# urw7rs/diffusion-models-made-easy

Measured on AMD Instinct MI355X. Metric: denoising steps/sec + training images/sec, DDPM UNet CIFAR10 32×32 @1/2/4/8 GPU, higher is better.
Workload: dtype bf16; 1 GPU; DDPM T=1000 sampling, CIFAR10 32x32, default UNet (32,416,643 params, random init), batch 128 per GPU, t.shape=(1,); global_batch=128, parallelism=dp1 (independent chains per GPU, no data-path collective)

## Files before the change

### diffusion-models-made-easy_amd/_lib.py

```python

from __future__ import annotations

import ctypes as C
import os
import subprocess
import threading

_HERE = os.path.dirname(os.path.abspath(__file__))
LIB_PATH = os.environ.get("DMME_LIB_PATH") or os.path.join(_HERE, "libdmme_hip.so")
CSRC = os.path.join(_HERE, "csrc")

F16R32 = 4
F32, BF16, BF16X3, F16 = 0, 1, 2, 3
CHAIN_DDPM, CHAIN_DDIM, CHAIN_IDDPM, CHAIN_DDPM_GUIDED, CHAIN_DDIM_GUIDED, CHAIN_GDDIM = 0, 1, 2, 3, 4, 5
CHAIN_DDPM_CFG, CHAIN_GDDIM_CFG = 6, 7
CHAIN_DPMPP, CHAIN_DPMPP_CFG = 8, 9
CHAIN_REPAINT = 10
CHAIN_ILVR = 11
CHAIN_DDNM = 12
PRED_EPS, PRED_X0, PRED_V = 0, 1, 2
PREDICTIONS = {"eps": PRED_EPS, "x0": PRED_X0, "v": PRED_V}
CM_METRICS = {"pseudo-huber": 0, "l2": 1}
THRESHOLD_NONE, THRESHOLD_STATIC, THRESHOLD_DYNAMIC = 0, 1, 2
THRESHOLDS = {"none": THRESHOLD_NONE, "static": THRESHOLD_STATIC, "dynamic": THRESHOLD_DYNAMIC}
# ... 14 lines not shown
        ("dropout", C.c_float),
        ("num_depths", C.c_int),
        ("channels_per_depth", C.c_int * 8),
        ("num_blocks", C.c_int),
        ("num_attention_depths", C.c_int),
        ("attention_depths", C.c_int * 8),
        ("arch", C.c_int),
        ("num_heads", C.c_int),
        ("num_classes", C.c_int),
    ]


class ConvDesc(C.Structure):
    _fields_ = [(n, C.c_int) for n in (
        "dtype", "N", "Hin", "Win", "C1", "C2", "upsample", "stride", "taps", "Cout", "pro_silu", "out_silu",
        "nt", "tproj_ld", "in_nchw", "out_nchw", "force_generic")]


BUCKET_FN = C.CFUNCTYPE(None, C.c_void_p, C.c_int, C.c_int64, C.c_int64)


class DmmeError(RuntimeError):
    pass


def build(verbose: bool = False) -> str:
    cmd = ["make", "-C", CSRC, "-j", str(min(8, os.cpu_count() or 1))]
    res = subprocess.run(cmd, stdout=subprocess.PIPE, stderr=subprocess.STDOUT, text=True)
    if verbose or res.returncode != 0:
        print(res.stdout)
    if res.returncode != 0:
        raise DmmeError("building libdmme_hip.so failed")
    return LIB_PATH


_vp, _i, _i64, _f, _u64 = C.c_void_p, C.c_int, C.c_int64, C.c_float, C.c_uint64

PROTOTYPES = {
    "dmme_last_error": (C.c_char_p, []),
    "dmme_version": (_i, []),
    "dmme_device_count": (_i, []),
    "dmme_unet_plan_create": (_i, [C.POINTER(UNetCfg), _i, _i, _i, _i, _i, C.POINTER(_vp)]),
    "dmme_unet_plan_destroy": (None, [_vp]),
    "dmme_unet_plan_num_params": (_i, [_vp]),
    "dmme_unet_plan_param_info": (_i, [_vp, _i, C.c_char_p, _i, C.POINTER(_i), C.POINTER(_i64), C.POINTER(_i64), C.POINTER(_i)]),
    "dmme_unet_plan_ref_numel": (_i64, [_vp]),
    "dmme_unet_plan_packed_bytes": (_i64, [_vp]),
    "dmme_unet_plan_workspace_bytes": (_i64, [_vp]),
    "dmme_unet_plan_dropmask_numel": (_i64, [_vp]),
    "dmme_unet_plan_out_channels": (_i, [_vp]),
    "dmme_unet_plan_num_launches": (_i, [_vp]),
    "dmme_unet_plan_num_launches_nograd": (_i, [_vp]),
    "dmme_unet_plan_num_folded": (_i, [_vp]),
    "dmme_unet_pack_params": (_i, [_vp, _vp, _vp, _vp]),
    "dmme_unet_pack_folded": (_i, [_vp, _vp, _vp]),
    "dmme_unet_forward": (_i, [_vp, _vp, _vp, _vp, _i, _vp, _vp, _vp, _vp]),
    "dmme_unet_forward_nograd": (_i, [_vp, _vp, _vp, _vp, _i, _vp, _vp, _vp, _vp]),
    "dmme_unet_forward_cond": (_i, [_vp, _vp, _vp, _vp, _i, _vp, _vp, _vp, _vp, _i, _vp, _vp]),
    "dmme_unet_backward_cond": (_i, [_vp, _vp, _vp, _vp, _vp, _i, _vp, _vp, _vp, _vp, _vp, _vp, _vp, _vp, _vp, _vp]),
    "dmme_unet_backward_input_cond": (_i, [_vp, _vp, _vp, _vp, _vp, _i, _vp, _vp, _vp, _vp, _vp, _vp, _vp]),
    "dmme_label_dropout": (_i, [_vp, _i, _i, _f, _u64, _u64, _vp, _vp, _vp]),
    "dmme_cfg_step": (_i, [_i, _vp, _vp, _vp, _f, _f, _f, _f, _i, _i, _i64, _vp]),
    "dmme_chain_update_cfg": (_i, [_i, _vp, _vp, _vp, _vp, _vp, _vp, _i, _i64, _vp]),
    "dmme_cfg_chain_step": (_i, [_vp, _vp, _vp, _vp, _vp, _vp, _vp, _i, _vp, _vp, _vp, _vp]),
    "dmme_dpmpp_step": (_i, [_vp, _vp, _vp, C.POINTER(_f), _i, _i, _i64, _i, _vp]),
    "dmme_chain_update_dpmpp": (_i, [_vp, _vp, _vp, _vp, _vp, _vp, _i, _i64, _i, _vp]),
    "dmme_dpmpp_chain_step": (_i, [_vp, _vp, _vp, _vp, _vp, _vp, _vp, _vp, _vp, _vp]),
    "dmme_cfg_dpmpp_step": (_i, [_vp, _vp, _vp, C.POINTER(_f), _i, _i, _i64, _vp]),
    "dmme_chain_update_cfg_dpmpp": (_i, [_vp, _vp, _vp, _vp, _vp, _vp, _i, _i64, _vp]),
    "dmme_cfg_dpmpp_chain_step": (_i, [_vp, _vp, _vp, _vp, _vp, _vp, _vp, _vp, _vp, _vp, _vp, _vp]),
    "dmme_repaint_step": (_i, [_vp, _vp, _vp, _vp, _vp, C.POINTER(_f), _i, _i64, _i, _vp]),
    "dmme_chain_update_repaint": (_i, [_vp, _vp, _vp, _vp, _vp, _vp, _vp, _vp, _i, _i64, _i, _vp]),
    "dmme_repaint_chain_step": (_i, [_vp, _vp, _vp, _vp, _vp, _vp, _vp, _vp, _vp, _vp, _vp]),
    "dmme_lowpass": (_i, [_vp, _vp, _i, _i, _i, _vp, _vp, _vp, _i, _vp]),
    "dmme_lowpass_lds_capacity": (_i, []),
    "dmme_lowpass_scratch_bytes": (_i64, [_i, _i, _i]),
    "dmme_ilvr_step": (_i, [_vp, _vp, _vp, _vp, C.POINTER(_f), _vp, _vp, _vp, _i, _i, _i, _i, _i, _i, _vp]),
    "dmme_chain_update_ilvr": (_i, [_vp, _vp, _vp, _vp, _vp, _vp, _vp, _vp, _vp, _vp, _i, _i, _i, _i, _i, _i, _vp]),
    "dmme_ilvr_chain_step": (_i, [_vp, _vp, _vp, _vp, _vp, _vp, _vp, _vp, _vp, _vp, _vp, _vp, _vp]),
    "dmme_ddnm_band_capacity": (_i, []),
    "dmme_ddnm_measure": (_i, [_vp, _vp, _vp, _i, _i, _i, _i, _i, _i, _vp]),
    "dmme_ddnm_step": (_i, [_vp, _vp, _vp, _vp, _vp, C.POINTER(_f), _i, _i, _i, _i, _i, _i, _i, _vp]),
    "dmme_chain_update_ddnm": (_i, [_vp, _vp, _vp, _vp, _vp, _vp, _vp, _vp, _i, _i, _i, _i, _i, _i, _i, _vp]),
    "dmme_ddnm_chain_step": (_i, [_vp, _vp, _vp, _vp, _vp, _vp, _vp, _i, _i, _vp, _vp, _vp, _vp]),
    "dmme_distill_noise": (_i, [_vp, _vp, _vp, _vp, _vp, _vp, _i, _i, _i64, _vp, _vp, _vp, _vp, _vp]),
    "dmme_distill_mid": (_i, [_i, _i, _vp, _vp, _vp, _vp, _i, _i, _i64, _vp, _vp]),
    "dmme_distill_target": (_i, [_i, _i, _vp, _vp, _vp, _vp, _vp, _vp, _i, _i, _i64, _vp, _vp]),
    "dmme_cm_target": (_i, [_i, _vp, _vp, _vp, _vp, _i, _i, _i64, _vp, _vp]),
    "dmme_cm_loss": (_i, [_i, _vp, _vp, _vp, _vp, _vp, _i, _i, _i64, _f, _vp, _vp, _vp, _f, _vp, _vp]),
    "dmme_ema_lerp": (_i, [_vp, _vp, _i64, _f, _vp]),
    "dmme_unet_plan_num_ops": (_i, [_vp]),
    "dmme_unet_plan_level_info": (_i, [_vp, C.c_char_p, _i]),
    "dmme_unet_plan_check": (_i, [_vp]),
    "dmme_debug_level_stamps": (_i, [_vp, _i, _i]),
    "dmme_unet_plan_op_info": (_i, [_vp, _i, C.c_char_p, _i, C.POINTER(C.c_double), C.POINTER(C.c_double)]),
    "dmme_unet_forward_profiled": (_i, [_vp, _vp, _vp, _vp, _i, _vp, _vp, _vp, _vp, _vp]),
    "dmme_unet_plan_packed_bwd_bytes": (_i64, [_vp]),
    "dmme_unet_plan_bwd_workspace_bytes": (_i64, [_vp]),
    "dmme_unet_pack_params_bwd": (_i, [_vp, _vp, _vp, _vp]),
    "dmme_unet_backward": (_i, [_vp, _vp, _vp, _vp, _vp, _i, _vp, _vp, _vp, _vp, _vp, _vp, _vp]),
    "dmme_unet_backward_buckets": (_i, [_vp, _vp, _vp, _vp, _vp, _i, _vp, _vp, _vp, _vp, _vp, _vp, _vp, BUCKET_FN, _vp]),
    "dmme_unet_backward_input": (_i, [_vp, _vp, _vp, _vp, _vp, _i, _vp, _vp, _vp, _vp, _vp, _vp]),
    "dmme_unet_plan_grad_buckets": (_i, [_vp, C.POINTER(_i64), C.POINTER(_i64), C.POINTER(_i), _i]),
    "dmme_unet_plan_bwd_summary": (_i, [_vp, C.c_char_p, _i]),
    "dmme_grad_norm": (_i, [_vp, _i64, _vp, _vp, _vp]),
    "dmme_adam_step": (_i, [_vp, _vp, _vp, _vp, _vp, _i64, _f, _f, _f, _f, _i, _vp, _f, _f, _f, _vp]),
    "dmme_amp_init": (_i, [_vp, _f, _vp]),
    "dmme_amp_scale": (_i, [_vp, _i64, _vp, _vp]),
    "dmme_adam_step_amp": (_i, [_vp, _vp, _vp, _vp, _vp, _i64, _f, _f, _f, _f, _vp, _f, _f, _f, _vp, _f, _f, _i, _vp]),
    "dmme_grad_pack_bf16": (_i, [_vp, _i64, _vp, _i64, _vp]),
    "dmme_shard_reduce_bf16": (_i, [_vp, _i, _i64, _f, _vp, _vp]),
    "dmme_grad_unpack_bf16": (_i, [_vp, _i64, _vp, _vp]),
    "dmme_unet_debug_read": (_i, [_vp, _vp, C.c_char_p, _vp, _i64, C.POINTER(_i64), _vp]),
    "dmme_unet_debug_read_grad": (_i, [_vp, _vp, C.c_char_p, _vp, _i64, C.POINTER(_i64), _vp]),
    "dmme_unet_debug_read_norm_stats": (_i, [_vp, _vp, C.c_char_p, _vp, _i64, C.POINTER(_i64), _vp]),
    "dmme_dropout_masks": (_i, [_vp, _u64, _u64, _vp, _vp]),
    "dmme_randn": (_i, [_vp, _i64, _u64, _u64, _vp]),
    "dmme_q_sample": (_i, [_vp, _vp, _vp, _vp, _vp, _i, _i64, _vp, _vp, _vp]),
    "dmme_ddpm_step": (_i, [_vp, _vp, _vp, _f, _f, _f, _i, _i64, _vp]),
    "dmme_ddim_step": (_i, [_vp, _vp, _f, _f, _i64, _vp]),
    "dmme_gddim_step": (_i, [_vp, _vp, _vp, _f, _f, _f, _i64, _vp]),
    "dmme_slerp": (_i, [_vp, _vp, _vp, _i, _i, _i64, _vp, _vp]),
    "dmme_chain_set": (_i, [_vp, _i64, _vp, _u64, _u64, _vp]),
    "dmme_chain_update": (_i, [_i, _vp, _vp, _vp, _vp, _vp, _i, _i64, _vp]),
    "dmme_chain_step": (_i, [_vp, _vp, _vp, _vp, _vp, _i, _vp, _vp, _vp, _vp]),
    "dmme_chain_update_gddim": (_i, [_vp, _vp, _vp, _vp, _vp, _vp, _i, _i64, _vp]),
    "dmme_log_softmax_grad": (_i, [_vp, _vp, _i, _i, _i, _f, _vp, _vp, _vp, _vp]),
    "dmme_chain_update_guided": (_i, [_i, _vp, _vp, _vp, _vp, _vp, _vp, _vp, _i, _i64, _vp]),
    "dmme_guided_chain_step": (_i, [_vp, _vp, _vp, _vp, _vp, _vp, _vp, _vp, _vp, _vp, _vp, _vp, _vp, _vp, _vp, _i, _vp, _vp, _vp, _vp]),
    "dmme_mse_loss": (_i, [_vp, _vp, _i64, _vp, _vp, _f, _vp, _vp]),
    "dmme_pred_to_eps": (_i, [_i, _vp, _vp, _vp, _i, _vp, _i, _i, _i64, _vp]),
    "dmme_unet_plan_set_prediction": (_i, [_vp, _i, _vp, _i]),
    "dmme_x0_threshold": (_i, [_i, _vp, _vp, _vp, _i, _vp, _i, _i, _i64, _i, _i, _f, _i, _f, _vp, _vp]),
    "dmme_x0_threshold_scratch_bytes": (_i64, [_i, _i64]),
    "dmme_x0_threshold_lds_capacity": (_i, []),
    "dmme_unet_plan_set_threshold": (_i, [_vp, _i, _vp, _i, _i, _f, _vp]),
    "dmme_q_sample_pred": (_i, [_i, _vp, _vp, _vp, _vp, _vp, _i, _i64, _vp, _vp, _vp]),
    "dmme_mse_loss_rows": (_i, [_vp, _vp, _vp, _vp, _i, _i64, _vp, _vp, _f, _vp, _vp]),
    "dmme_image_batch": (_i, [_vp, _i64, _vp, _vp, _i, _i, _i, _i, _vp, _vp]),
    "dmme_grid_tile": (_i, [_vp, _i, _i, _i, _i, _i, _i, _i, _i, _i, _i, _i, _vp, _vp]),
    "dmme_iddpm_step": (_i, [_vp, _vp, _vp, _f, _f, _f, _f, _i, _i, _i64, _vp]),
    "dmme_iddpm_loss": (_i, [_vp, _vp, _vp, _vp, _vp, _vp, _i, _i64, _f, _f, _vp, _vp, _f, _vp, _vp]),
    "dmme_iddpm_loss_rows": (_i, [_vp, _vp, _vp, _vp, _vp, _vp, _i, _vp, _i, _i64, _f, _f, _vp, _vp, _vp, _f, _vp, _vp, _vp]),
    "dmme_iddpm_prior_rows": (_i, [_vp, _i, _i64, _f, _vp, _vp]),
    "dmme_tsampler_draw": (_i, [_vp, _vp, _i, _i, _f, _u64, _u64, _i, _vp, _vp, _vp, _vp]),
    "dmme_tsampler_update": (_i, [_vp, _vp, _i, _i, _vp, _vp, _i, _vp, _vp]),
    "dmme_conv2d": (_i, [C.POINTER(ConvDesc), _vp, _vp, _vp, _vp, _vp, _vp, _vp, _vp, _vp, _vp, _i, _vp, _vp]),
    "dmme_conv2d_res": (_i, [C.POINTER(ConvDesc), _vp, _vp, _vp, _vp, _vp, _vp, _vp, _vp, _vp, _i, _i, _vp, _vp, _vp, _vp]),
    "dmme_groupnorm_scale_shift": (_i, [_i, _vp, _vp, _i, _i, _i, _i, _i, _vp, _vp, _f, _vp, _vp, _vp, _i, _vp]),
    "dmme_attention": (_i, [_i, _vp, _i, _i, _i, _vp, _i, _vp]),
    "dmme_attention_proj": (_i, [_i, _vp, _i, _i, _i, _vp, _vp, _vp, _vp, _vp, _vp, _i, _vp]),
    "dmme_attention_fold": (_i, [_i, _i, _vp, _vp, _vp, _vp, _vp, _vp, _vp, _vp, _vp]),
    "dmme_attention_block": (_i, [_i, _vp, _i, _i, _i, _vp, _i, _i, _i, _vp, _vp, _f, _vp, _vp, _vp, _vp, _vp, _vp, _vp, _vp, _vp, _i, _vp]),
    "dmme_attention_heads": (_i, [_i, _vp, _i, _i, _i, _i, _vp, _i, _vp]),
    "dmme_nchw_to_nhwc": (_i, [_i, _vp, _i, _i, _i, _vp, _vp]),
    "dmme_nhwc_to_nchw": (_i, [_i, _vp, _i, _i, _i, _vp, _vp]),
    "dmme_pack_weight": (_i, [_i, _vp, _i, _i, _i, _vp, _vp]),
    "dmme_event_create": (_i, [C.POINTER(_vp)]),
    "dmme_event_record": (_i, [_vp, _vp]),
    "dmme_event_elapsed_ms": (_i, [_vp, _vp, C.POINTER(_f)]),
    "dmme_event_destroy": (_i, [_vp]),
    "dmme_debug_set_stamps": (_i, [_vp]),
    "dmme_debug_mfma_valu": (_i, [_i, _i, _i, _vp, _vp]),
    "dmme_debug_issue_probe": (_i, [_i, _i, _i, _i, _i, _vp, _vp, _vp]),
    "dmme_debug_l2_stream": (_i, [_vp, _i64, _i, _i, _i, _i, _vp, _vp]),
}


def lib():
    global _lib
    if _lib is not None:
        return _lib
    with _lock:
        if _lib is not None:
            return _lib
        if not os.path.exists(LIB_PATH):
            raise DmmeError(
                f"{LIB_PATH} is missing: the HIP extension is not built. Run `python -c 'import __graft_entry__ as g; g.build()'` "
                "(or `make -C diffusion-models-made-easy_amd/csrc`). There is no CPU fallback for the product path."
            )
        h = C.CDLL(LIB_PATH)
        for name, (res, args) in PROTOTYPES.items():
            fn = getattr(h, name)
            fn.restype = res
            fn.argtypes = args
        _lib = h
    return _lib


def check(rc: int, what: str = ""):
    if rc != 0:
        msg = lib().dmme_last_error().decode("utf-8", "replace")
        if rc == -2:
            raise NotImplementedError(f"{what}: {msg}")
        if rc == -1:
            raise ValueError(f"{what}: {msg}")
        raise DmmeError(f"{what} failed (status {rc}): {msg}")


def require_gpu():
    if lib().dmme_device_count() <= 0:
        raise DmmeError("libdmme_hip.so loaded but no HIP device is visible; the denoiser path only runs on an MI355X")


def dtype_code(precision) -> int:
# ... 29 lines not shown
```

### diffusion-models-made-easy_amd/csrc/common.h

```cpp
#pragma once

#include <hip/hip_runtime.h>
#include <stdint.h>

#include "dmme_hip.h"

namespace dmme {

void set_error(const char* fmt, ...) __attribute__((format(printf, 1, 2)));

int debug_route(const char* key, int dflt = 0);

#define DMME_CHECK_HIP(expr)                                                                          \
    do {                                                                                              \
        hipError_t e_ = (expr);                                                                       \
        if (e_ != hipSuccess) {                                                                       \
            ::dmme::set_error("%s failed: %s (%s:%d)", #expr, hipGetErrorString(e_), __FILE__, __LINE__); \
            return DMME_ERR_HIP;                                                                      \
        }                                                                                             \
    } while (0)

#define DMME_REQUIRE(cond, code, ...)        \
    do {                                     \
        if (!(cond)) {                       \
// ... 128 lines not shown
    const float* p2;
    int t1, cnt1, C1, t2, cnt2, C2, groups;
    const float* gamma;
    const float* beta;
    float eps;
    float* mean_rstd;
    const float* t_shift;
    const float* t_scale;
    int t_ld, nt;
};

struct ConvArgs {
    const void* src1;
    const void* src2;
    const void* w;
    const float* bias;
    const float* scale;
    const float* shift;
    const float* dmask;
    const float* tproj;
    const void* res1;
    const void* res2;
    void* dst;
    int N, Hin, Win, C1, C2;
    int up, stride, taps;
    int Hout, Wout, Cout;
    int pro_silu, out_silu;
    int nt, tproj_ld, R1;
    int in_nchw, out_nchw;
    float* gn_part;
    int gn_cg, gn_tiles;
    int gn_raw_moments;
    long long* stamps;
    float* splitk;
    int64_t splitk_cap;
    int x3;
    int mix;
    int mix2;
    int f16;
    int dma_b;
    GnOut gno[2];
    int n_gno;
    float gn_eps;
    void* act;
    int act_k, act_silu;
    const float* act_dmask;
    GnIn gni;
    int has_gni;
    const void* r_src1;
    const void* r_src2;
    const void* r_w;
    const float* r_bias;
    int r_C1, r_C2;
};

int launch_mfma_valu(int mode, int iters, int blocks, float* sink, hipStream_t s);
int launch_issue_probe(int kind, int n_inner, int iters, int flags, int blocks, long long* sink, const void* src, hipStream_t s);
int launch_l2_stream(const void* buf, int64_t bytes, int iters, int mode, int depth, int blocks, unsigned* sink, hipStream_t s);

struct ConvTile {
    int TW, TH, TN;
    int HH, HWd;
    int tiles_x, tiles_y;
    int tiles_m, tiles_n;
    int a_rows;
    unsigned magic_px, magic_w;
};
enum ConvFamily {
    CONV_GENERIC = 0,
    CONV_MFMA,
    CONV_THIN,
    CONV1X1_SPLIT,
    CONV1X1_AS,
    CONV1X1_TILED,
    CONV3X3_SPLIT,
    CONV3X3_WS,
    CONV3X3_KW,
    CONV3X3_PIPE,
};
struct ConvRoute {
    int family;
    ConvTile tile;
    int BM, BN;
    int cand;
    int GT, UA;
    int NI, ring;
    int ksplit;
    int rseg;
    int vec;
    int stat_bn;
    int stat_px;
    int stat_tiles;
};
inline ConvRoute make_route(int family, int BM = 0, int BN = 0, int vec = 0) {
    ConvRoute r{};
    r.family = family;
    r.BM = r.stat_px = BM;
    r.BN = r.stat_bn = BN;
    r.vec = vec;
    return r;
}
ConvRoute conv_route(int dtype, const ConvArgs& a);
bool conv_thin_route(int dtype, const ConvArgs& a, ConvRoute& r);
bool conv1x1_split_route(int dtype, const ConvArgs& a, ConvRoute& r);
bool conv1x1_domain(int dtype, const ConvArgs& a);
bool conv1x1_as_route(int dtype, const ConvArgs& a, ConvRoute& r);
bool conv1x1_tiled_route(int dtype, const ConvArgs& a, ConvRoute& r);
bool conv3x3_split_route(int dtype, const ConvArgs& a, ConvRoute& r);
bool conv3x3_pipe_route(int dtype, const ConvArgs& a, ConvRoute& r);
bool conv3x3_ws_route(int dtype, const ConvArgs& a, ConvRoute& r);
bool conv3x3_kw_route(int dtype, const ConvArgs& a, ConvRoute& r);
bool conv_mfma_route(int dtype, const ConvArgs& a, ConvRoute& r);
void conv_generic_route(const ConvArgs& a, ConvRoute& r);
bool conv_mfma_supported(int dtype, const ConvArgs& a);
int launch_conv_generic(int dtype, const ConvArgs& a, hipStream_t s);
const char* conv_generic_kernel_name(const ConvArgs& a);
int launch_conv_mfma(const ConvRoute& r, int dtype, const ConvArgs& a, hipStream_t s);
int launch_conv_out_thin(const ConvArgs& a, hipStream_t s);
int launch_conv1x1(const ConvRoute& r, int dtype, const ConvArgs& a, hipStream_t s);
int launch_conv1x1_as(const ConvArgs& a, hipStream_t s);
int launch_conv3x3(const ConvRoute& r, int dtype, const ConvArgs& a, hipStream_t s);
int launch_conv_kw(int dtype, const ConvArgs& a, const ConvTile& g, int NI, int ring, int BM, int ksplit, hipStream_t s);
int launch_conv(int dtype, const ConvArgs& a, hipStream_t s, int force = 0);
int launch_conv(const ConvRoute& r, int dtype, const ConvArgs& a, hipStream_t s);
void conv_label(const ConvRoute& r, int dtype, const ConvArgs& a, char* buf, int cap);
bool conv_stats_query(int dtype, const ConvArgs& a, int cg, int* tiles, int* px);
bool conv_gn_in_query(int dtype, const ConvArgs& a);
bool conv1x1_tiled_gn_in_ok(const ConvArgs& a, const ConvRoute& r);
bool conv3x3_pipe_gn_in_ok(int dtype, const ConvArgs& a, const ConvRoute& r);
int conv_gn_direct_query(int dtype, const ConvArgs& a, const int* cg, int n);
int launch_gn_finalize_parts(const float* part1, int tiles1, int cnt1, int C1, const float* part2, int tiles2, int cnt2, int C2, int N, int groups,
                             const float* gamma, const float* beta, float eps, float* scale, float* shift, float* mean_rstd, const float* t_shift,
                             const float* t_scale, int t_ld, int nt, hipStream_t s);

int launch_gn_generic(int dtype, const void* src1, const void* src2, int N, int HW, int C1, int C2, int groups,
                      const float* gamma, const float* beta, float eps, float* scale, float* shift, float* mean_rstd,
                      hipStream_t s);
bool gn_fast_supported(int dtype, int N, int HW, int C1, int C2, int groups);
size_t gn_fast_scratch_floats(int N, int HW, int C, int groups);
int launch_gn_fast(int dtype, const void* src1, const void* src2, int N, int HW, int C1, int C2, int groups,
                   const float* gamma, const float* beta, float eps, float* scale, float* shift, float* mean_rstd,
                   float* partial, hipStream_t s, void* act = nullptr, int act_silu = 0, const float* dmask = nullptr);
bool gn_small_act_supported(int dtype, int HW, int C1, int C2, int groups);

int launch_attn_generic(int dtype, const void* qkv, int N, int S, int C, void* out, hipStream_t s);
int launch_attn_heads(int dtype, const void* qkv, int N, int S, int C, int heads, void* out, hipStream_t s);
int launch_attn_heads_bwd(int dtype, const void* qkv, const void* dO, int N, int S, int C, int heads, float* P, float* dS, void* dqkv, hipStream_t s);
int launch_gn_modulate(float* scale, float* shift, const float* t_shift, const float* t_scale, int ld, int nt, int N, int C, hipStream_t s);
bool attn_x3_supported(int N, int S, int C, int heads);
int launch_attn_x3(const void* qkv, int N, int S, int C, int heads, void* out, hipStream_t s);
bool attn_mfma_supported(int dtype, int N, int S, int C);
bool attn_full_takes(int S, int D);
int launch_attn_mfma(int dtype, const void* qkv, int N, int S, int C, void* out, float* lse, hipStream_t s);
bool attn_proj_fusable(int dtype, int N, int S, int C, int gn_cg, int gn_tiles);
int launch_attn_proj(int dtype, const void* qkv, int N, int S, int C, void* ctx, float* lse, const void* w, const float* bias, const void* res, void* dst,
                     float* gn_part, int gn_tiles, int gn_cg, hipStream_t s, long long* stamps = nullptr);
struct AttnFoldJob {
    int64_t wq, bq, wp, bp;
    int64_t M, c, wpv, bias2;
    int32_t C, pad;
};
bool attn_fold_shape_ok(int dtype, int N, int S, int C, int gn_cg, int gn_tiles);
int launch_attn_fold(int dtype, const void* x, int N, int S, int C, const GnIn* gni, const float* scale, const float* shift, const void* M, const float* c,
                     const void* wpv, const float* bias2, const void* res, void* dst, float* gn_part, int gn_tiles, int gn_cg, hipStream_t s,
                     long long* stamps = nullptr);
int launch_attn_fold_weights(int dtype, const AttnFoldJob* jobs_dev, int n_jobs, int maxC, void* packed, hipStream_t s, const AttnFoldJob* one = nullptr);
bool attn_heads_mfma_supported(int dtype, int N, int S, int C, int heads);
int launch_attn_heads_mfma(int dtype, const void* qkv, int N, int S, int C, int heads, void* out, float* lse, hipStream_t s);
int launch_attn_heads_bwd_mfma(int dtype, const void* qkv, const void* O, const void* dO, const float* lse, int N, int S, int C, int heads, void* P,
                               void* dS, void* dqkv, hipStream_t s);
bool attn_bwd_mfma_supported(int dtype, int N, int S, int C);
int launch_attn_bwd_mfma(int dtype, const void* qkv, const void* O, const void* dO, const float* lse, int N, int S, int C, void* P, void* dS,
                         void* dqkv, hipStream_t s);

constexpr unsigned kFwdMarkKeep = 0x4B454550u, kFwdMarkNograd = 0x4E4F4752u;
constexpr unsigned kErrNogradBackward = 0x80000000u;
int launch_time_sinusoid(const int64_t* t, int nt, const float* freqs, int half, float* out, hipStream_t s, unsigned* mark = nullptr,
                         unsigned mark_val = 0);
int launch_linear_wave(int dtype, const float* in, int nt, int K, const void* W, const float* bias, int Nout,
                       int out_silu, float* out, hipStream_t s);
int launch_label_cond(const float* z2, int nt, const float* E, const int64_t* labels, int B, int K, int emb, float* temb, float* zsave, int* status,
                      hipStream_t s);
int launch_label_grad(const float* dz2, const int64_t* labels, int B, int K, int emb, float* dE, hipStream_t s);

int launch_nchw_to_nhwc(int dtype, const float* src, int N, int C, int HW, void* dst, hipStream_t s, const unsigned* mark = nullptr,
                        unsigned* err = nullptr);
int launch_nhwc_to_nchw(int dtype, const void* src, int N, int C, int HW, float* dst, hipStream_t s);
int launch_pack_weight(int dtype, const float* src, int Cout, int Cin, int taps, void* dst, hipStream_t s);
int launch_cast_f32_to_16(int dtype, const float* src, int64_t numel, void* dst, hipStream_t s);

struct PackItem {
    int64_t src_off;
    int64_t dst_off;
    int32_t cout, cin, taps;
    int32_t row0, rows;
    int32_t ci0, nci;
    int32_t as_f32;
};
int launch_pack_table(int dtype, const PackItem* items_dev, int n_items, const float* ref_flat, void* packed,
                      hipStream_t s);

int launch_randn(float* out, int64_t numel, uint64_t seed, uint64_t offset, hipStream_t s);
int launch_dropmask(float* out, int64_t numel, float p, uint64_t seed, uint64_t offset, hipStream_t s);
int launch_q_sample(const float* x0, const float* z, const float* sqrt_abar, const float* sqrt_1m_abar,
                    const int64_t* t, int B, int64_t chw, float* x_t, float* target, hipStream_t s);
int launch_pred_to_eps(int pred, float* model_out, const float* x, const float* ab, int T, const int64_t* t, int t_len, int B, int64_t chw,
                       hipStream_t s);
int launch_x0_threshold(int mode, float* out, const float* x, const float* table, int T, const int64_t* t, int t_len, int B, int64_t chw, int planes,
                        int halves, float sg, const float* sg_coef, int sg_row, int sg_col, const int64_t* sg_state, int k, float frac, void* scratch,
                        hipStream_t s);
int slerp_parts(int64_t chw);
int launch_slerp(const float* xa, const float* xb, const float* w, int n, int B, int64_t chw, float* out, float* scratch, hipStream_t s);
int launch_chain_set(void* state, int64_t i, const int64_t* t_table, uint64_t seed, uint64_t offset, hipStream_t s);

// ... 183 lines not shown
```

### diffusion-models-made-easy_amd/csrc/conv_pipe.hip

```cpp
#include <stdio.h>

#include "conv_common.h"

namespace dmme {



template <typename T, int BM, int BN, int GT, int PIPE_UA, bool ACC3 = false>
__global__ void __launch_bounds__(256, GT == 9 ? 1 : 2) conv3x3_pipe_kernel(ConvArgs a, ConvTile g, int shTW, int shTH, int ksplit) {
    constexpr int KC = Frag<T>::KC, EPV = Frag<T>::EPV;
    constexpr int MI = BM / 64, NI = BN / 64;
    constexpr int UB = BN / 32;
    extern __shared__ __attribute__((aligned(16))) char lds[];
#define PIPE_STAMP(K) do { if (a.stamps && blockIdx.x < 2 && blockIdx.y == 0 && threadIdx.x == 0) a.stamps[blockIdx.x * 8 + (K)] = (long long)wall_clock64(); } while (0)
    PIPE_STAMP(0);
    char* ldsA = lds;
    char* ldsB = lds + (size_t)g.a_rows * ROW_DATA;
    constexpr bool DMAB_OK = sizeof(T) == 2 && GT == 3 && BN == 64;
    constexpr int B_BYTES = GT * BN * ROW_DATA;
    const bool dmab = DMAB_OK && a.dma_b;
    int cur = 0;
    float* gni_par = reinterpret_cast<float*>(ldsB + (size_t)B_BYTES * (dmab ? 2 : 1));

    const int tid = threadIdx.x, lane = tid & 63, wave = tid >> 6;
// ... 269 lines not shown
        }
        float f[4] = {v.x, v.y, v.z, v.w};
        const int n = (int)(p / hw);
#pragma unroll
        for (int j = 0; j < 4; ++j) {
            float fold = a.bias ? a.bias[c + j] : 0.f;
            if (a.tproj) fold += a.tproj[(int64_t)(a.nt == 1 ? 0 : n) * a.tproj_ld + c + j];
            f[j] += fold;
            if (a.res1) f[j] += to_f(((const T*)a.res1)[p * a.Cout + c + j]);
            ((T*)a.dst)[p * a.Cout + c + j] = from_f<T>(f[j]);
        }
    }
}
static int pipe_ksplit(const ConvArgs& a, const ConvTile& g, int pick, int KC) {
    if (a.has_gni) return 1;
    const bool off = (debug_route("no_splitk") != 0);
    if (off || !a.splitk || pick != 3 || a.stride != 1 || a.gn_part || a.n_gno || a.out_silu || a.out_nchw || a.res2 || a.Cout % 4) return 1;
    const int64_t wgs = (int64_t)g.tiles_m * g.tiles_n;
    if (wgs > 128) return 1;
    int ks = (a.C1 + a.C2) / KC;
    const int room = (int)(256 / wgs);
    if (ks > room) ks = room;
    if (ks > 4) ks = 4;
    const int64_t out = (int64_t)a.N * a.Hout * a.Wout * a.Cout;
    while (ks > 1 && ks * out > a.splitk_cap) --ks;
    return ks < 1 ? 1 : ks;
}

#ifndef WS_CDMA
#define WS_CDMA 1
#endif
#ifndef WS_HYB
#define WS_HYB 0
#endif
#ifndef WS_SCHED2
#define WS_SCHED2 1
#endif
#ifndef WS_TP_UNROLL
#define WS_TP_UNROLL 9
#endif
template <typename T, int BN, int MI, int NI>
__device__ __forceinline__ void ws_stage16(const f32x16 (&acc)[MI][NI], T* row) {
    typedef T tx2 __attribute__((ext_vector_type(2)));
#pragma unroll
    for (int mi = 0; mi < MI; ++mi)
#pragma unroll
        for (int ni = 0; ni < NI; ++ni)
#pragma unroll
            for (int q = 0; q < 4; ++q) {
                const tx2 lo = {(T)acc[mi][ni][4 * q], (T)acc[mi][ni][4 * q + 1]}, hi = {(T)acc[mi][ni][4 * q + 2], (T)acc[mi][ni][4 * q + 3]};
                *reinterpret_cast<uint2*>(row + mi * 64 * (BN + kStage16Pad) + 32 * ni + 8 * q) = make_uint2(__builtin_bit_cast(unsigned, lo), __builtin_bit_cast(unsigned, hi));
            }
}
struct WsTile { int n0, oy0, ox0, co0, ts; };
__device__ __forceinline__ WsTile ws_tile_of(const ConvTile& g, int shTW, int shTH, int kt, int bn) {
    const int t = (int)blockIdx.x + kt * (int)gridDim.x;
    const int tile_n = t % g.tiles_n, tile_m = t / g.tiles_n;
    const int tiles_img = g.tiles_x * g.tiles_y;
    WsTile r;
    const int sp = tile_m % tiles_img;
    r.n0 = tile_m / tiles_img;
    r.oy0 = (sp / g.tiles_x) << shTH;
    r.ox0 = (sp % g.tiles_x) << shTW;
    r.co0 = tile_n * bn;
    r.ts = sp;
    return r;
}

__host__ __device__ inline int ws2_stage_pad(int a_bytes) { return a_bytes + 2 * 128 * ROW_DATA >= 64 * 1024 ? 0 : 64 * 1024 - 2 * 128 * ROW_DATA - a_bytes; }

__device__ __forceinline__ void ws_fill_par_gni(const ConvArgs& a, int n, bool writer, float* par, int Cin, int tid, int nthr) {
    for (int c = tid; c < Cin; c += nthr) {
        float sc, sh;
        const float dmk = a.dmask ? a.dmask[n * Cin + c] : 1.f;
        gn_in_scale_shift(a, n, c, Cin, writer, sc, sh);
        par[c] = sc * dmk;
        par[Cin + c] = sh * dmk;
        par[2 * Cin + c] = a.pro_silu ? -1.4426950408889634f * sc : 0.f;
        par[3 * Cin + c] = a.pro_silu ? -1.4426950408889634f * sh : -126.f;
    }
}

template <typename T, int SPLIT>
struct WsSplit {
    typedef T ts;
};
template <typename T>
struct WsSplit<T, 1> {
    typedef float ts;
};
template <typename T>
struct WsSplit<T, 2> {
    typedef float ts;
};
template <int PIPE_UA, typename T = bf16, int BM = 256, int SPLIT = 0, bool RSEG = false, bool E16 = false>
__global__ void __launch_bounds__(512, 1) conv3x3_ws2_kernel(ConvArgs a, ConvTile g, int shTW, int shTH, int ntiles) {
    constexpr int KC = 64, EPV = 8, BN = 128, MI = BM / 64, NI = 2, UB = BN / 32;
    constexpr bool CDMA = WS_CDMA != 0;
    constexpr bool SCHED2 = WS_SCHED2 != 0 && CDMA && SPLIT == 0;
    static_assert(!(SCHED2 && WS_HYB != 0), "the hybrid tap ownership counts the halo loads of the two-unit schedule");
    static_assert(!E16 || (SPLIT == 0 && BM == 256 && sizeof(T) == 2), "16-bit staging: 16-bit tensors, 256-pixel tiles");
    static_assert(!RSEG || (SPLIT == 0 && sizeof(T) == 2), "residual segment: 16-bit tensors");
    constexpr int KCR = SPLIT ? 32 : KC;
    constexpr int EPR = SPLIT ? 4 : EPV;
    typedef typename WsSplit<T, SPLIT>::ts TS;
    static_assert(SPLIT == 0 || (BM == 256 && dtype_of<T>::value == DMME_F16), "split passes: fp16 hi / lo on the 256-pixel tile");
    constexpr int R_BYTES = BN * ROW_DATA;
    constexpr int A_PITCH = ROW_DATA + 16;
    static_assert((BM == 256 && PIPE_UA == 11) || (BM == 128 && PIPE_UA == 7), "unit schedules below: 11 units over 9 stages, or 7 units over the first 7");
    typedef unsigned u32x4 __attribute__((ext_vector_type(4)));
    extern __shared__ __attribute__((aligned(16))) char lds[];
    const int a_bytes = g.a_rows * A_PITCH;
    const int Cin = a.C1 + a.C2;
    const int offA1 = a_bytes + 3 * R_BYTES, offR = a_bytes;
    float* par_base = reinterpret_cast<float*>(lds + 2 * a_bytes + 3 * R_BYTES + ws2_stage_pad(a_bytes));
    float* fold_base = par_base + 2 * 4 * Cin;
#define WS_FILL_FOLD(KT)                                                                              \
    if constexpr (E16) {                                                                              \
        if (tid < BN) {                                                                               \
            const TileXY ff_ = WS_TILE(KT);                                                           \
            const int co_ = ff_.co0 + tid;                                                            \
            float f_ = 0.f;                                                                           \
            if (co_ < a.Cout) {                                                                       \
                f_ = a.bias ? a.bias[co_] : 0.f;                                                      \
                if (a.r_bias) f_ += a.r_bias[co_];                                                    \
                if (a.tproj) f_ += a.tproj[(a.nt == 1 ? 0 : ff_.n0) * a.tproj_ld + co_];              \
            }                                                                                         \
            fold_base[((KT) & 1) * BN + tid] = f_;                                                    \
        }                                                                                             \
    }
#define WS_BUFA(p) (lds + (((p) & 1) ? offA1 : 0))
#define WS_RING(slot) (lds + offR + (slot) * R_BYTES)
#define WS_PAR(kt) (par_base + ((kt) & 1) * 4 * Cin)
#define WS_TILE(kt) ws_tile_of(g, shTW, shTH, (kt), BN)
    typedef WsTile TileXY;
    const int tid = threadIdx.x, lane = tid & 63, wave = tid >> 6;
    const bool producer = wave >= 4;
    const int nchunks = Cin / KCR;
    const int CinW = SPLIT ? 2 * Cin : Cin;
    const int Cres = RSEG ? a.r_C1 + a.r_C2 : 0;
    const int HS = Cres / 32;
    constexpr int RSL = 5;
    const int RT = HS + ((RSEG && (HS - 1) % RSL < 2) ? 1 : 0);
#define WS_RSA(k) ((k) < 2 ? lds + (k) * (BM * 64) : (k) == 2 ? lds + offR + 2 * R_BYTES : lds + offA1 + ((k) - 3) * (BM * 64))
#define WS_RSW(k) ((k) < 4 ? lds + offR + (k) * 8192 : lds + offA1 + 2 * (BM * 64))
    const int K = (ntiles - (int)blockIdx.x + (int)gridDim.x - 1) / (int)gridDim.x;
    const bool has_pro = a.scale || a.pro_silu || a.dmask;
#define WS_FILL_PAR_N(KT, NTHR)                                           \
    {                                                                     \
        float* par = WS_PAR(KT);                                          \
        const TileXY ft_ = WS_TILE(KT);                                   \
        if (a.has_gni) {                                                  \
            ws_fill_par_gni(a, ft_.n0, ft_.ts == 0 && ft_.co0 == 0, par, Cin, tid, NTHR); \
        } else {                                                          \
            const int pn0 = ft_.n0;                                       \
            for (int c = tid; c < Cin; c += (NTHR)) {                     \
                const int so = pn0 * Cin + c;                             \
                const float sc_ = a.scale ? a.scale[so] : 1.f, sh_ = a.scale ? a.shift[so] : 0.f, dm_ = a.dmask ? a.dmask[so] : 1.f; \
                par[c] = sc_ * dm_;                                       \
                par[Cin + c] = sh_ * dm_;                                 \
                par[2 * Cin + c] = a.pro_silu ? -1.4426950408889634f * sc_ : 0.f;    \
                par[3 * Cin + c] = a.pro_silu ? -1.4426950408889634f * sh_ : -126.f; \
            }                                                             \
        }                                                                 \
    }
#define WS_FILL_PAR(KT) WS_FILL_PAR_N(KT, 512)
    const int mTW = (1 << shTW) - 1, mTH = (1 << shTH) - 1;
    float gn_carry[2] = {0.f, 0.f};
    const bool estamp = tid == 0 && blockIdx.x == 0;
    int e_i = 0;
#define WS_ESTAMP() { if (estamp && a.stamps && e_i < 24) a.stamps[64 + e_i++] = (long long)clock64(); }
#define WS2_PASS(TT, P, STAGE_STMT)                                                                                                \
    {                                                                                                                              \
        constexpr int p = (P);                                                                                                     \
        auto pix_of = [&](int m) -> int {                                                                                          \
            const int mm = m + 128 * p;                                                                                            \
            const int tx = mm & mTW, ty = (mm >> shTW) & mTH;                                                                      \
            return ((TT).n0 * a.Hout + (TT).oy0 + ty) * a.Wout + (TT).ox0 + tx;                                                    \
        };                                                                                                                         \
        uint4 rpre[128 * (BN / (16 / (int)sizeof(TS))) / 512];                                                                     \
        if constexpr (!E16) conv_epilogue_res_prefetch<TS, 128, BN, 512>(a, (TT).co0, pix_of, rpre);  \
        WS_ESTAMP()                                                                                                                \
        STAGE_STMT                                                                                                                 \
        WS_ESTAMP()                                                                                                                \
        lds_barrier();                                                                                                             \
        WS_ESTAMP()                                                                                                                \
        conv_epilogue_store<TS, 128, BN, 512, E16>(a, (TT).co0, (TT).n0, pix_of, stage, (BM / 128) * (TT).ts + p, E16 ? nullptr : rpre, a.n_gno ? p : -1, gn_carry); \
        WS_ESTAMP()                                                                                                                \
        lds_barrier();                 \
    }
#define WS2_EPILOGUE(TT, KT, STAGE0, STAGE1)                                                                                       \
    {                                                                                                                              \
        float* stage = reinterpret_cast<float*>(WS_RING(1));                                                                       \
        WS2_PASS(TT, 0, STAGE0)                                                                                                    \
        if constexpr (BM == 256) { WS2_PASS(TT, 1, STAGE1) }                                                                       \
        if ((KT) + 2 < K) WS_FILL_PAR((KT) + 2)                                                                                    \
    }
#define WS2_EPILOGUE16(TT, KT, STAGE_ALL)                                                                                          \
    {                                                                                                                              \
        T* st16 = reinterpret_cast<T*>(WS_RING(1));                                                                                \
        if ((KT) + 1 < K) WS_FILL_FOLD((KT) + 1)                                                                                   \
        WS_ESTAMP()                                                                                                                \
        STAGE_ALL                                                                                                                  \
        WS_ESTAMP()                                                                                                                \
        lds_barrier();                                                                                                             \
        WS_ESTAMP()                                                                                                                \
        _Pragma("unroll") for (int p = 0; p < 2; ++p) {                                                                            \
            auto pix_of = [&](int m) -> int {                                                                                      \
                const int mm = m + 128 * p;                                                                                        \
                const int tx = mm & mTW, ty = (mm >> shTW) & mTH;                                                                  \
                return ((TT).n0 * a.Hout + (TT).oy0 + ty) * a.Wout + (TT).ox0 + tx;                                                \
            };                                                                                                                     \
            conv_epilogue_store<TS, 128, BN, 512, true>(a, (TT).co0, (TT).n0, pix_of, reinterpret_cast<float*>(st16 + p * 128 * (BN + kStage16Pad)), \
                                                        2 * (TT).ts + p, nullptr, a.n_gno ? p : -1, gn_carry);                     \
            WS_ESTAMP()                                                                                                            \
        }                                                                                                                          \
        lds_barrier();                                                                 \
        if ((KT) + 2 < K) WS_FILL_PAR((KT) + 2)                                                                                    \
    }
    if (producer) {
        const int ptid = tid & 255, cu = ptid & 7, urow = ptid >> 3, pw = ptid >> 6;
        const int Hv = a.up ? 2 * a.Hin : a.Hin, Wv = a.up ? 2 * a.Win : a.Win;
        int a_pix[PIPE_UA], a_sw[PIPE_UA];
        unsigned b_vo[UB];
#pragma unroll
        for (int i = 0; i < PIPE_UA; ++i) a_sw[i] = (urow + 32 * i) * A_PITCH + cu * (SPLIT ? 8 : 16);
#pragma unroll
        for (int k4 = 0; k4 < UB; ++k4) b_vo[k4] = (unsigned)(((urow + 32 * k4) * 9 * CinW + (cu ^ ((urow >> 1) & 7)) * EPV) * 2);
        auto pix_unit = [&](int i, const TileXY& t) __attribute__((always_inline)) -> int {
            const int row = urow + 32 * i;
            const int hy = (int)__umulhi((unsigned)row, g.magic_w), hx = row - hy * g.HWd;
            const int iy = t.oy0 - 1 + hy, ix = t.ox0 - 1 + hx;
            const bool in = iy >= 0 && iy < Hv && ix >= 0 && ix < Wv && !(a.up == 2 && ((iy | ix) & 1));
            const int sy = a.up ? (iy >> 1) : iy, sx = a.up ? (ix >> 1) : ix;
#ifdef WS_SAME_IMAGE
            return row >= g.a_rows ? -2 : in ? ((t.n0 & 7) * a.Hin + sy) * a.Win + sx : -1;
#else
            return row >= g.a_rows ? -2 : in ? (t.n0 * a.Hin + sy) * a.Win + sx : -1;
#endif
        };
        auto set_pix = [&](int i, const TileXY& t) __attribute__((always_inline)) { a_pix[i] = pix_unit(i, t); };
        const char* wbase = (const char*)a.w;
        u32x4 areg[PIPE_UA];
        f32x2 pS[4], pH[4], pS2[4], pH2[4];
        auto load_par = [&](const float* par, int c0) __attribute__((always_inline)) {
            const float* p = par + c0 + cu * EPR;
#pragma unroll
            for (int d = 0; d < EPR / 2; ++d) {
                pS[d] = *reinterpret_cast<const f32x2*>(p + 2 * d);
                pH[d] = *reinterpret_cast<const f32x2*>(p + Cin + 2 * d);
                pS2[d] = *reinterpret_cast<const f32x2*>(p + 2 * Cin + 2 * d);
                pH2[d] = *reinterpret_cast<const f32x2*>(p + 3 * Cin + 2 * d);
            }
        };
        auto load_A = [&](int i, int ch) __attribute__((always_inline)) {
            constexpr int SB = SPLIT == 1 ? 4 : 2;
            const int c0 = ch * KCR;
            const bool second = c0 >= a.C1;
            const char* sbase = (const char*)(second ? a.src2 : a.src1) + (size_t)((second ? c0 - a.C1 : c0) * SB);
            const int Cs = second ? a.C2 : a.C1;
            const int px = a_pix[i] < 0 ? 0 : a_pix[i];
            const char* gp = sbase + (size_t)((unsigned)(px * Cs + cu * EPR) * (unsigned)SB);
            if constexpr (SPLIT == 2) {
                const uint2 v2 = *reinterpret_cast<const uint2*>(gp);
                areg[i] = u32x4{v2.x, v2.y, 0u, 0u};
            } else {
                areg[i] = *reinterpret_cast<const u32x4*>(gp);
            }
        };
        auto store_A = [&](int i, char* dstA, int mode = 0) __attribute__((always_inline)) {
            const int pix = a_pix[i], sw = a_sw[i];
            u32x4 val = areg[i];
            if constexpr (SPLIT != 0) {
                f32x2 y[2];
                if constexpr (SPLIT == 1) {
                    y[0] = f32x2{__uint_as_float(val[0]), __uint_as_float(val[1])};
                    y[1] = f32x2{__uint_as_float(val[2]), __uint_as_float(val[3])};
                } else {
                    typedef T tx4 __attribute__((ext_vector_type(4)));
                    const tx4 x = __builtin_bit_cast(tx4, make_uint2(val[0], val[1]));
                    y[0] = f32x2{(float)x[0], (float)x[1]};
// ... 12 lines not shown
#pragma unroll
                for (int d = 0; d < 2; ++d)
#pragma unroll
                    for (int k = 0; k < 2; ++k) {
                        const f16 hv = (f16)y[d][k];
                        hi[2 * d + k] = hv;
                        lo[2 * d + k] = (f16)sub_plain(y[d][k], (float)hv);
                    }
                uint2 hw = __builtin_bit_cast(uint2, hi), lw = __builtin_bit_cast(uint2, lo);
                if (pix < 0) hw = lw = make_uint2(0u, 0u);
                if (pix != -2) {
                    *reinterpret_cast<uint2*>(dstA + sw) = hw;
                    *reinterpret_cast<uint2*>(dstA + sw + 64) = lw;
                }
                return;
            }
            if (has_pro && mode != 2) {
                typedef typename Vec8<T>::type tx8;
                const tx8 x = __builtin_bit_cast(tx8, val);
                tx8 o;
#pragma unroll
                for (int d = 0; d < 4; ++d) {
                    float xv[2], yv[2];
                    if constexpr (sizeof(T) == 2 && dtype_of<T>::value == DMME_BF16) {
                        xv[0] = __uint_as_float(val[d] << 16);
                        xv[1] = __uint_as_float(val[d] & 0xffff0000u);
                    } else {
                        xv[0] = (float)x[2 * d];
                        xv[1] = (float)x[2 * d + 1];
                    }
                    pro_pair_plain(xv[0], xv[1], pS[d], pH[d], pS2[d], pH2[d], yv[0], yv[1]);
                    o[2 * d] = (T)yv[0];
                    o[2 * d + 1] = (T)yv[1];
                }
                val = __builtin_bit_cast(u32x4, o);
            }
            if (mode == 1) {
                areg[i] = val;
                return;
            }
            const u32x4 zero = {0u, 0u, 0u, 0u};
            if (pix < 0) val = zero;
            if (pix != -2) *reinterpret_cast<u32x4*>(dstA + sw) = val;
        };
        auto dma_tap = [&](char* dstR, int co0, int c, int t) __attribute__((always_inline)) {
#if defined(WS_X_NO_DMA)
            {
                const char* ub1 = wbase + ((size_t)co0 * 9 * CinW + (size_t)t * CinW + (size_t)c * KC) * 2;
                _Pragma("unroll") for (int k4 = 0; k4 < UB; ++k4) glds16_hidden(ub1 + (lane & 7) * 16, (unsigned)__builtin_amdgcn_readfirstlane((int)((unsigned)(size_t)(lds_c*)dstR + (unsigned)(pw * 8 * ROW_DATA) + (unsigned)(32 * k4 * ROW_DATA))));
                return;
            }
#endif
            const unsigned lbase = (unsigned)(size_t)(lds_c*)dstR + (unsigned)(pw * 8 * ROW_DATA);
            const char* ub = wbase + ((size_t)co0 * 9 * CinW + (size_t)t * CinW + (size_t)c * KC) * 2;
#pragma unroll
            for (int k4 = 0; k4 < UB; ++k4) {
                const unsigned l = (unsigned)__builtin_amdgcn_readfirstlane((int)(lbase + (unsigned)(32 * k4 * ROW_DATA)));
                glds16_hidden(ub + b_vo[k4], l);
            }
        };
        constexpr int RA = BM / 64, RD = RA + 2;
        auto dma_rseg_A = [&](int k, const TileXY& t, int j) __attribute__((always_inline)) {
            int ln = lane;
            asm volatile("" : "+v"(ln));
            const int c0 = j * 32;
            const bool second = c0 >= a.r_C1;
            const int Cs = second ? a.r_C2 : a.r_C1;
            const int tile_pix0 = (t.n0 * a.Hin + t.oy0) * a.Win + t.ox0;
            const char* sb = (const char*)(second ? a.r_src2 : a.r_src1) + ((size_t)tile_pix0 * Cs + (second ? c0 - a.r_C1 : c0)) * 2;
            const unsigned la = (unsigned)(size_t)(lds_c*)WS_RSA(k) + (unsigned)(pw * (BM / 4) * 64);
            const int piece = ((ln & 3) ^ ((ln >> 4) & 3)) * 16;
#pragma unroll
            for (int q = 0; q < RA; ++q) {
                const int m = (BM / 4) * pw + 16 * q + (ln >> 2);
                const int rel = (m >> shTW) * a.Win + (m & mTW);
                const unsigned l = (unsigned)__builtin_amdgcn_readfirstlane((int)(la + (unsigned)(q * 1024)));
                glds16_hidden_s(sb, (unsigned)(rel * Cs * 2 + piece), l);
            }
        };
        auto dma_rseg_W = [&](int k, const TileXY& t, int j) __attribute__((always_inline)) {
            int ln = lane;
            asm volatile("" : "+v"(ln));
            const char* wb = (const char*)a.r_w + ((size_t)t.co0 * Cres + j * 32) * 2;
            const unsigned lw = (unsigned)(size_t)(lds_c*)WS_RSW(k) + (unsigned)(pw * 2048);
            const int piece = ((ln & 3) ^ ((ln >> 4) & 3)) * 16;
#pragma unroll
            for (int q = 0; q < 2; ++q) {
                const unsigned l = (unsigned)__builtin_amdgcn_readfirstlane((int)(lw + (unsigned)(q * 1024)));
                glds16_hidden_s(wb, (unsigned)((32 * pw + 16 * q + (ln >> 2)) * Cres * 2 + piece), l);
            }
        };
        TileXY tcur = WS_TILE(0), tnext = WS_TILE(K > 1 ? 1 : 0);
        {
#pragma unroll
            for (int i = 0; i < PIPE_UA; ++i) {
                set_pix(i, tcur);
                load_A(i, 0);
            }
            dma_tap(WS_RING(0), tcur.co0, 0, 0);
            dma_tap(WS_RING(1), tcur.co0, 0, 1);
            WS_FILL_PAR(0)
            __syncthreads();
            load_par(WS_PAR(0), 0);
#pragma unroll
            for (int i = 0; i < PIPE_UA; ++i) store_A(i, WS_BUFA(0));
#pragma unroll
            for (int i = 0; i < PIPE_UA; ++i) load_A(i, 1);
            wait_vm_keep<PIPE_UA>();
        }
        __syncthreads();
        int kt = 0, cc = 0, cg = 0;
        int p_i = 0;
        (void)p_i;
#define WS_A_UNIT(i)                                                        \
    {                                                                       \
        if (RSEG && last_c) {  \
            if (do_store) store_A((i), dstA, 1);                            \
        } else {                                                            \
            if (do_store) store_A((i), dstA);                               \
            WS_PSTT(1)                                                      \
            if (new_tile) set_pix((i), tnn);                                \
            WS_PSTT(2)                                                      \
            load_A((i), lc);                                                \
            WS_PSTT(3)                                                      \
        }                                                                   \
    }
#define WS_A_MATH(i) { if (do_store) store_A((i), dstA, 1); }
#define WS_A_WRITE(i)                                                        \
    {                                                                       \
        if (RSEG && last_c) {  } \
        else {                                                              \
            if (do_store) store_A((i), dstA, 2);                            \
            WS_PSTT(1)                                                      \
            if (new_tile) set_pix((i), tnn);                                \
            load_A((i), lc);                                                \
        }                                                                   \
    }
#define WS_A_ARRIVED(i) { asm volatile("" : "+v"(areg[i][0]), "+v"(areg[i][1]), "+v"(areg[i][2]), "+v"(areg[i][3])); }
#ifdef WS_PSTAMPS
        long long* pst_lds = reinterpret_cast<long long*>(reinterpret_cast<char*>(par_base) + 2 * 4 * Cin * 4 + 1024);
#define WS_PSTT(TAG) { if (a.stamps && ptid == 0 && blockIdx.x == 0 && p_i < 500) pst_lds[p_i++] = (long long)clock64() | ((long long)(TAG) << 56); }
#else
#define WS_PSTT(TAG)
#endif
#define WS_PST() WS_PSTT(0)
#define WS_L(TP) (PIPE_UA == 11 ? (((TP) == 0 || (TP) == 8) ? 2 : 1) : ((TP) < 7 ? 1 : 0))
#define WS_RD(TP) ((TP) <= 4 ? UB : (TP) <= 6 ? UB + RA : 0)
#define WS_RX(TP) (((TP) == 5 || (TP) == 6) ? RA : 0)
#define WS_PSTAGE(TP)                                                                                                   \
    {                                                                                                                   \
        WS_PST()                                                                                                        \
        const bool last_c = cc + 1 == nchunks;                                                                          \
        const bool have_n = !(last_c && kt + 1 == K);                                                                   \
// ... 77 lines not shown
            else wait_lgkm_all();                                                                                       \
        }                                                                                                               \
        else if (RSEG && last_c) {                                                                                      \
             \
            if ((TP) == 0) wait_vm_keep<WS_L(8) + UB>();                                                                \
            else if ((TP) <= 6) wait_vm_keep<WS_RX(((TP) + 8) % 9) + WS_RD(TP)>();                                      \
            else if ((TP) == 7) wait_vm_keep<WS_RX(6) + 4>();   \
            else wait_vm_keep<2>();                                                                                     \
        }                                                                                                               \
        else if (sent_next) wait_vm_keep<UB + WS_L(TP)>();                                                              \
        else if (sent) wait_vm_keep<WS_L(((TP) + 8) % 9) + UB + WS_L(TP)>();                                            \
        else wait_vm_keep<WS_L(((TP) + 8) % 9) + WS_L(TP)>();                                                           \
        WS_PST()                                                                                                        \
        __builtin_amdgcn_s_barrier();                                                                                   \
        if ((TP) == 8) {                                                                                                \
            ++cg;                                                                                                       \
            if (++cc == nchunks) {         \
                if constexpr (RSEG) {                                                                                   \
                     \
                    int sl = 2;                                                                                         \
                    for (int j = 0; j < RT; ++j) {                                                                      \
                        const bool fin = j + 1 == RT && kt + 1 < K;                                                     \
                        for (int h_ = (j == 0 ? 2 : j + 4); h_ <= j + 4 && h_ < HS; ++h_) {                             \
                            dma_rseg_A(sl, tcur, h_);                                                                   \
                            dma_rseg_W(sl, tcur, h_);                                                                   \
                            sl = sl == RSL - 1 ? 0 : sl + 1;                                                            \
                        }                                                                                               \
                        if (fin) {  \
                            _Pragma("unroll") for (int i = 0; i < PIPE_UA; ++i) store_A(i, WS_BUFA(cg), 2);             \
                            dma_tap(WS_RING(0), tnext.co0, 0, 0);                                                       \
                            _Pragma("unroll") for (int i = 0; i < PIPE_UA; ++i) load_A(i, 1);                           \
                        }                                                                                               \
                        __builtin_amdgcn_sched_barrier(0);                                                              \
                        const int hmax = j + 4 < HS - 1 ? j + 4 : HS - 1;     \
                        const int ahead = hmax - (j + 1);                    \
                        if (fin) wait_vm_keep<UB + PIPE_UA>();                                                          \
                        else if (ahead >= 3) wait_vm_keep<3 * RD>();                                                    \
                        else if (ahead == 2) wait_vm_keep<2 * RD>();                                                    \
                        else if (ahead == 1) wait_vm_keep<RD>();                                                        \
                        else wait_vm_keep<0>();                                                                         \
                        __builtin_amdgcn_s_barrier();                                                                   \
                    }                                                                                                   \
                }                                                                                                       \
                if constexpr (E16) { WS2_EPILOGUE16(tcur, kt, ;) } else { WS2_EPILOGUE(tcur, kt, ;, ;) }                         \
                                       \
                        \
                cc = 0;                                                                                                 \
                ++kt;                                                                                                   \
                tcur = tnext;                                                                                           \
                tnext = WS_TILE(kt + 1 < K ? kt + 1 : kt);                                                              \
            }                                                                                                           \
        }                                                                                                               \
    }
        const int GCH = K * nchunks;
        for (int ch = 0; ch < GCH; ++ch) {
            WS_PSTAGE(0) WS_PSTAGE(1) WS_PSTAGE(2) WS_PSTAGE(3) WS_PSTAGE(4) WS_PSTAGE(5) WS_PSTAGE(6) WS_PSTAGE(7) WS_PSTAGE(8)
        }
#ifdef WS_PSTAMPS
        if (a.stamps && ptid == 0 && blockIdx.x == 0)
            for (int i = 0; i < p_i; ++i) a.stamps[128 + i] = pst_lds[i];
#endif
#undef WS_PSTAGE
#undef WS_RD
#undef WS_RX
#undef WS_L
#undef WS_PST
#undef WS_PSTT
#undef WS_A_UNIT
#undef WS_A_MATH
#undef WS_A_WRITE
#undef WS_A_ARRIVED
        return;
    }

    WS_FILL_PAR(0)
    WS_FILL_FOLD(0)
    __syncthreads();
    if (K > 1) WS_FILL_PAR_N(1, 256)
    __builtin_amdgcn_s_setprio(3);
    const int wrow = wave >> 1, wn0 = (wave & 1) * 64;
    const int r = lane & 31, h = lane >> 5;
    int a_row[MI];
#pragma unroll
    for (int mi = 0; mi < MI; ++mi) {
        const int m = (2 * mi + wrow) * 32 + r;
        const int tx = m & mTW, ty = (m >> shTW) & mTH;
        a_row[mi] = (ty * g.HWd + tx) * A_PITCH + h * 16;
    }
    int b_off[NI][4];
#pragma unroll
    for (int ni = 0; ni < NI; ++ni) {
        const int row = wn0 + ni * 32 + r;
#pragma unroll
        for (int kg = 0; kg < 4; ++kg) b_off[ni][kg] = row * ROW_DATA + (((kg * 2 + h) ^ ((row >> 1) & 7)) << 4);
    }
    unsigned cb_vo[UB];
#pragma unroll
    for (int k4 = 0; k4 < UB; ++k4) {
        const int urow_ = wave * 8 + (lane >> 3);
        cb_vo[k4] = (unsigned)(((urow_ + 32 * k4) * 9 * CinW + ((lane & 7) ^ ((urow_ >> 1) & 7)) * EPV) * 2);
    }
    auto cdma = [&](int slot, int co0, int c, int t) __attribute__((always_inline)) {
        const char* ub = (const char*)a.w + ((size_t)co0 * 9 * CinW + (size_t)t * CinW + (size_t)c * KC) * 2;
        const unsigned lbase = (unsigned)(size_t)(lds_c*)WS_RING(slot) + (unsigned)(wave * 8 * ROW_DATA);
#pragma unroll
        for (int k4 = 0; k4 < UB; ++k4)
            glds16_hidden_s(ub, cb_vo[k4], (unsigned)__builtin_amdgcn_readfirstlane((int)(lbase + (unsigned)(32 * k4 * ROW_DATA))));
    };
    int stamp_i = 0;
    const bool stamping = a.stamps && tid == 0 && blockIdx.x == 0;
#define WS_STAMP() { if (stamping && stamp_i < 64) a.stamps[stamp_i++] = (long long)clock64(); }
    WS_STAMP()
    __syncthreads();
    WS_STAMP()
    int cg = 0;
    for (int kt = 0; kt < K; ++kt) {
        const TileXY t = WS_TILE(kt);
        f32x16 acc[MI][NI];
        if constexpr (E16) {
            const float* fb = fold_base + (kt & 1) * BN + wn0 + 4 * h;
#pragma unroll
            for (int ni = 0; ni < NI; ++ni)
#pragma unroll
                for (int q = 0; q < 4; ++q) {
                    const f32x4 f4 = *reinterpret_cast<const f32x4*>(fb + 32 * ni + 8 * q);
#pragma unroll
                    for (int mi = 0; mi < MI; ++mi)
#pragma unroll
                        for (int k = 0; k < 4; ++k) acc[mi][ni][4 * q + k] = f4[k];
                }
        } else {
#pragma unroll
        for (int mi = 0; mi < MI; ++mi)
#pragma unroll
            for (int ni = 0; ni < NI; ++ni)
#pragma unroll
                for (int j = 0; j < 16; ++j) acc[mi][ni][j] = 0.f;
        }
#if defined(WS_X_NO_FRAGS)
#define WS_FRAGS(SET, KG)                                                                                                         \
    {                                                                                                                             \
        _Pragma("unroll") for (int mi = 0; mi < MI; ++mi) { u32x4 t_; asm volatile("" : "=v"(t_)); af[SET][mi] = __builtin_bit_cast(uint4, t_); }   \
        _Pragma("unroll") for (int ni = 0; ni < NI; ++ni) { u32x4 t_; asm volatile("" : "=v"(t_)); bfr[SET][ni] = __builtin_bit_cast(uint4, t_); }  \
        __builtin_amdgcn_sched_barrier(0);                                                                                        \
    }
#else
#define WS_FRAGS(SET, KG)                                                                                                         \
    {                                                                                                                             \
        _Pragma("unroll") for (int mi = 0; mi < MI; ++mi) af[SET][mi] = *reinterpret_cast<const uint4*>(pa[mi] + (KG) * 32);      \
        _Pragma("unroll") for (int ni = 0; ni < NI; ++ni) bfr[SET][ni] = *reinterpret_cast<const uint4*>(ldsR + b_off[ni][KG]);   \
        __builtin_amdgcn_sched_barrier(0);                                                                                        \
    }
#endif
#if defined(WS_X_NO_MFMA)
#define WS_MMAS(SET)                                                                                  \
    {                                                                                                 \
        _Pragma("unroll") for (int mi = 0; mi < MI; ++mi) asm volatile("" ::"v"(__builtin_bit_cast(u32x4, af[SET][mi])));   \
        _Pragma("unroll") for (int ni = 0; ni < NI; ++ni) asm volatile("" ::"v"(__builtin_bit_cast(u32x4, bfr[SET][ni])));  \
        __builtin_amdgcn_sched_barrier(0);                                                            \
    }
#else
#define WS_MMAS(SET)                                                                                  \
    {                                                                                                 \
        _Pragma("unroll") for (int mi = 0; mi < MI; ++mi)                                             \
            _Pragma("unroll") for (int ni = 0; ni < NI; ++ni) {                                       \
                if constexpr (E16) mma_group(bfr[SET][ni], af[SET][mi], acc[mi][ni], (T*)nullptr);    \
                else mma_group(af[SET][mi], bfr[SET][ni], acc[mi][ni], (T*)nullptr);                  \
            }                                                                                         \
        __builtin_amdgcn_sched_barrier(0);                                                            \
    }
#endif
#define WS_FA(SET, KG) { _Pragma("unroll") for (int mi = 0; mi < MI; ++mi) af[SET][mi] = *reinterpret_cast<const uint4*>(pa[mi] + (KG) * 32); }
#define WS_FB(SET, KG) { _Pragma("unroll") for (int ni = 0; ni < NI; ++ni) bfr[SET][ni] = *reinterpret_cast<const uint4*>(ldsR + b_off[ni][KG]); }
#define WS_SB() __builtin_amdgcn_sched_barrier(0);
#define WS_MM(SA, SB_)                                                                                \
    {                                                                                                 \
        _Pragma("unroll") for (int mi = 0; mi < MI; ++mi)                                             \
            _Pragma("unroll") for (int ni = 0; ni < NI; ++ni) mma_group(af[SA][mi], bfr[SB_][ni], acc[mi][ni], (T*)nullptr); \
        __builtin_amdgcn_sched_barrier(0);                                                            \
    }
        const TileXY tn = WS_TILE(kt + 1 < K ? kt + 1 : kt);
        const bool three = !a.mix2;
        for (int c = 0; c < nchunks; ++c, ++cg) {
            const char* ldsA = WS_BUFA(cg);
            const bool last_c = c + 1 == nchunks;
#pragma unroll WS_TP_UNROLL
            for (int tp = 0; tp < 9; ++tp) {
                const char* ldsR = WS_RING(tp % 3);
                const int tap_b = ((tp / 3) * g.HWd + (tp % 3)) * A_PITCH;
                const char* pa[MI];
#pragma unroll
                for (int mi = 0; mi < MI; ++mi) pa[mi] = ldsA + a_row[mi] + tap_b;
                uint4 af[2][MI], bfr[2][NI];
                bool sent = false;
#define WS_CDMA_ISSUE()                                                                                               \
    if constexpr (CDMA) {                                                                                             \
        if (tp == 0 && c == 0 && kt > 0) cdma(1, t.co0, 0, 1);                                                        \
        if (tp <= 6) { if (WS_HYB == 0 || tp == 0 || tp == 6) { cdma((tp + 2) % 3, t.co0, c, tp + 2); sent = true; } } \
        else if (RSEG && last_c) { }                                                                                  \
        else if (tp == 7) { if (!(last_c && kt + 1 == K)) { cdma(0, last_c ? tn.co0 : t.co0, last_c ? 0 : c + 1, 0); sent = true; } } \
        else if (!last_c) { cdma(1, t.co0, c + 1, 1); sent = true; }                                                  \
        __builtin_amdgcn_sched_barrier(0);                                                                            \
    }
                if constexpr (SPLIT != 0) {
                    WS_FA(0, 0) WS_FB(0, 0) WS_FB(1, 2) WS_SB()
                    WS_CDMA_ISSUE()
                    WS_MM(0, 0)
                    WS_FA(1, 2) WS_SB()
                    if (three) { WS_MM(0, 1) }
                    WS_FA(0, 1) WS_FB(1, 1) WS_SB()
                    WS_MM(1, 0)
                    WS_FB(0, 3) WS_FA(1, 3) WS_SB()
                    WS_MM(0, 1)
                    if (three) { WS_MM(0, 0) }
                    WS_MM(1, 1)
                } else {
                    WS_FRAGS(0, 0) WS_FRAGS(1, 1) WS_CDMA_ISSUE() WS_MMAS(0) WS_FRAGS(0, 2) WS_MMAS(1) WS_FRAGS(1, 3) WS_MMAS(0) WS_MMAS(1)
                }
#undef WS_CDMA_ISSUE
                WS_STAMP()
                if constexpr (CDMA) {
                    if (sent) wait_vm_keep<UB>();
                    else wait_vm_keep<0>();
                }
                __syncthreads();
                WS_STAMP()
            }
        }
        if constexpr (RSEG) {
            const int rsw = (r >> 2) & 3;
            const int rA = (wrow * 32 + r) * 64, rB = (wn0 + r) * 64;
            const int pk0 = (h ^ rsw) << 4, pk1 = ((2 + h) ^ rsw) << 4;
            int slot = 0;
            for (int j = 0; j < HS; ++j) {
                const char* sa = WS_RSA(slot) + rA;
                const char* sw = WS_RSW(slot) + rB;
                slot = slot == RSL - 1 ? 0 : slot + 1;
                uint4 af[2][MI], bfr[2][NI];
#pragma unroll
                for (int mi = 0; mi < MI; ++mi) af[0][mi] = *reinterpret_cast<const uint4*>(sa + mi * 4096 + pk0);
#pragma unroll
                for (int ni = 0; ni < NI; ++ni) bfr[0][ni] = *reinterpret_cast<const uint4*>(sw + ni * 2048 + pk0);
                __builtin_amdgcn_sched_barrier(0);
#pragma unroll
                for (int mi = 0; mi < MI; ++mi) af[1][mi] = *reinterpret_cast<const uint4*>(sa + mi * 4096 + pk1);
#pragma unroll
                for (int ni = 0; ni < NI; ++ni) bfr[1][ni] = *reinterpret_cast<const uint4*>(sw + ni * 2048 + pk1);
                __builtin_amdgcn_sched_barrier(0);
                WS_MMAS(0) WS_MMAS(1)
                WS_STAMP()
                __syncthreads();
                WS_STAMP()
            }
            for (int j = HS; j < RT; ++j) __syncthreads();
        }
#undef WS_FA
#undef WS_FB
#undef WS_SB
#undef WS_MM
#undef WS_FRAGS
#undef WS_MMAS
        if constexpr (E16) {
            WS2_EPILOGUE16(t, kt, (ws_stage16<T, BN, MI, NI>(acc, st16 + (wrow * 32 + r) * (BN + kStage16Pad) + wn0 + 4 * h));)
        } else {
        WS2_EPILOGUE(t, kt, (conv_epilogue_stage<T, BN, 2, NI, 64>(a, reinterpret_cast<f32x16(&)[2][NI]>(acc[0]), t.co0, wn0, r, h, wrow * 32, t.n0, stage));,
                     (conv_epilogue_stage<T, BN, 2, NI, 64>(a, reinterpret_cast<f32x16(&)[2][NI]>(acc[2]), t.co0, wn0, r, h, wrow * 32, t.n0, stage));)
        }
        WS_STAMP()
    }
#undef WS_STAMP
#undef WS2_EPILOGUE
#undef WS2_EPILOGUE16
#undef WS_FILL_FOLD
#undef WS2_PASS
#undef WS_FILL_PAR
#undef WS_FILL_PAR_N
#undef WS_ESTAMP
#undef WS_BUFA
#undef WS_RING
#undef WS_RSA
#undef WS_RSW
#undef WS_PAR
#undef WS_TILE
}

static size_t ws2_lds(const ConvArgs& a, const ConvTile& g) {
    const size_t a_bytes = (size_t)g.a_rows * (ROW_DATA + 16);
    size_t extra = 0;
#ifdef WS_PSTAMPS
    extra = 4096;
#endif
    return 2 * a_bytes + 3 * (size_t)128 * ROW_DATA + (size_t)ws2_stage_pad((int)a_bytes) + (size_t)2 * 4 * (a.C1 + a.C2) * 4 + 1024  + extra;
}

static int ws_pick(const ConvArgs& a, ConvTile& g) {
    constexpr int ws_min_tiles = 256;
    const int Cin = a.C1 + a.C2, nch = Cin / 64;
    if (a.taps != 9 || a.stride != 1 || Cin % 64 || a.C1 % 64 || nch < 2 || nch % 2 || Cin > 512 || a.out_silu || a.out_nchw || a.in_nchw || a.Cout % 128) return 0;
    ConvTile t;
    if (make_tile(a, 256, 128, t) && t.TN == 1 && t.a_rows <= 352 && ws2_lds(a, t) <= 160 * 1024 && (size_t)t.a_rows * ROW_DATA + 2 * 128 * ROW_DATA >= 64 * 1024 &&
        t.tiles_m * t.tiles_n >= ws_min_tiles) {
        g = t;
        return 3;
    }
    ConvTile u;
    if (!debug_route("no_ws128") && make_tile(a, 128, 128, u) && u.TN == 1 && u.a_rows <= 224 && ws2_lds(a, u) <= 160 * 1024 && u.tiles_m * u.tiles_n >= ws_min_tiles) {
        g = u;
        return 4;
    }
    return 0;
}

static bool ws2s_pick(const ConvArgs& a, ConvTile& g) {
    const int Cin = a.C1 + a.C2;
    if ((a.mix != 1 && a.mix != 2) || a.taps != 9 || a.stride != 1 || a.up == 2 || Cin % 64 || a.C1 % 32 || Cin < 64 || Cin > 512 || a.out_silu || a.out_nchw || a.in_nchw ||
        a.Cout % 128 || a.res2 || a.n_gno || (a.tproj && a.nt != 1 && a.nt != a.N))
// ... 49 lines not shown
        if (pipe_fits(a, 4, t) && (int64_t)t.tiles_m * t.tiles_n >= 2 * 256) {
            pick = 4;
            g = t;
        }
    }
    return pick;
}

static bool rseg_shape_ok(const ConvArgs& a) {
    const int Cres = a.r_C1 + a.r_C2;
    return a.r_src1 && a.r_bias && a.r_C1 > 0 && a.r_C1 % 64 == 0 && a.r_C2 >= 0 && (a.r_C2 == 0 || a.r_src2) && Cres % 128 == 0 && Cres <= 512 && !a.up && !a.res1 &&
           !a.res2 && (int64_t)a.Cout * Cres < (1ll << 30) && (int64_t)a.N * a.Hin * a.Win * Cres < (1ll << 30);
}

bool conv3x3_split_route(int dtype, const ConvArgs& a, ConvRoute& r) {
    ConvTile g{};
    if (dtype != DMME_F16 || a.taps != 9 || !ws2s_pick(a, g)) return false;
    r = make_route(CONV3X3_SPLIT, 256, 128, 4);
    r.tile = g;
    r.stat_px = 128;
    r.stat_tiles = g.tiles_x * g.tiles_y * 2;
    return true;
}

bool conv3x3_pipe_route(int dtype, const ConvArgs& a, ConvRoute& r) {
    if (!conv_mfma_supported(dtype, a)) return false;
    if (a.taps != 9 || (a.stride != 1 && a.stride != 2)) return false;
    if ((int64_t)a.Cout * 9 * (a.C1 + a.C2) >= (1ll << 31)) return false;
    if ((int64_t)a.N * a.Hin * a.Win >= (1ll << 31)) return false;
    ConvTile g{};
    const int pick = pipe_pick(a, g);
    if (pick < 0) return false;
    r = make_route(CONV3X3_PIPE, kPipeCand[pick][0], kPipeCand[pick][1], is16(dtype) ? 8 : 4);
    r.tile = g;
    r.cand = pick;
    r.GT = kPipeCand[pick][2];
    r.UA = kPipeUA[pick];
    r.ksplit = pipe_ksplit(a, g, pick, is16(dtype) ? 64 : 32);
    r.stat_tiles = g.TN == 1 ? g.tiles_x * g.tiles_y : 0;
    return true;
}

bool conv3x3_ws_route(int dtype, const ConvArgs& a, ConvRoute& r) {
    ConvTile g{};
    if (!is16(dtype) || getenv("DMME_NO_WS") || !ws_pick(a, g)) return false;
    r = make_route(CONV3X3_WS, g.TH * g.TW, 128, 8);
    r.tile = g;
    r.rseg = a.r_w && rseg_shape_ok(a);
    r.stat_px = 128;
    r.stat_tiles = g.tiles_x * g.tiles_y * (r.BM / 128);
    return true;
}

static size_t pipe_launch_lds(int dtype, const ConvArgs& a, const ConvRoute& r, bool* dma) {
    size_t lds = pipe_lds(r.tile, r.BN, r.GT);
    *dma = pipe_dma_ok(dtype, r.tile, r.BN, r.GT);
    if (*dma) lds += (size_t)r.GT * r.BN * ROW_DATA;
    if (a.has_gni) lds += (size_t)2 * (a.C1 + a.C2) * 4;
    if (a.n_gno && lds < (size_t)kDirectLds) lds = kDirectLds;
    return lds;
}

bool conv3x3_pipe_gn_in_ok(int dtype, const ConvArgs& a, const ConvRoute& r) {
    if (debug_route("no_gn_in_pipe") || r.tile.TN != 1) return false;
    ConvArgs b = a;
    b.has_gni = 1;
    bool dma = false;
    return pipe_launch_lds(dtype, b, r, &dma) <= (size_t)(r.GT == 9 ? 128 : 80) * 1024;
}

template <typename K>
static int set_lds_limit(K kernel, size_t bytes) {
    DMME_CHECK_HIP(hipFuncSetAttribute(reinterpret_cast<const void*>(kernel), hipFuncAttributeMaxDynamicSharedMemorySize, (int)bytes));
    return DMME_OK;
}

static int launch_ws2_split(const ConvRoute& r, const ConvArgs& a, hipStream_t s) {
    const ConvTile& gw = r.tile;
    static bool attr = false;
    if (!attr) {
        int rc0 = set_lds_limit(conv3x3_ws2_kernel<11, f16, 256, 1>, 160 * 1024);
        if (rc0 == DMME_OK) rc0 = set_lds_limit(conv3x3_ws2_kernel<11, f16, 256, 2>, 160 * 1024);
        if (rc0 != DMME_OK) return rc0;
        attr = true;
    }
    const int ntiles = gw.tiles_m * gw.tiles_n;
    const dim3 wgrid((unsigned)(ntiles < 256 ? ntiles : 256));
    if (a.mix == 2)
        hipLaunchKernelGGL((conv3x3_ws2_kernel<11, f16, 256, 2>), wgrid, dim3(512), ws2_lds(a, gw), s, a, gw, ilog2(gw.TW), ilog2(gw.TH), ntiles);
    else
        hipLaunchKernelGGL((conv3x3_ws2_kernel<11, f16, 256, 1>), wgrid, dim3(512), ws2_lds(a, gw), s, a, gw, ilog2(gw.TW), ilog2(gw.TH), ntiles);
    DMME_CHECK_LAUNCH();
    return DMME_OK;
}

template <typename T>
static int launch_ws_t(const ConvRoute& r, const ConvArgs& a, hipStream_t s) {
    const ConvTile& gw = r.tile;
    static bool ws_attr = false;
    if (!ws_attr) {
        int rc0 = set_lds_limit(conv3x3_ws2_kernel<11, T, 256>, 160 * 1024);
        if (rc0 == DMME_OK) rc0 = set_lds_limit(conv3x3_ws2_kernel<7, T, 128>, 160 * 1024);
        if (rc0 == DMME_OK) rc0 = set_lds_limit(conv3x3_ws2_kernel<11, T, 256, 0, true>, 160 * 1024);
        if (rc0 == DMME_OK) rc0 = set_lds_limit(conv3x3_ws2_kernel<7, T, 128, 0, true>, 160 * 1024);
        if (rc0 == DMME_OK) rc0 = set_lds_limit(conv3x3_ws2_kernel<11, T, 256, 0, false, true>, 160 * 1024);
        if (rc0 == DMME_OK) rc0 = set_lds_limit(conv3x3_ws2_kernel<11, T, 256, 0, true, true>, 160 * 1024);
        if (rc0 != DMME_OK) return rc0;
        ws_attr = true;
    }
    const int ntiles = gw.tiles_m * gw.tiles_n;
    const dim3 wgrid((unsigned)(ntiles < 256 ? ntiles : 256));
    const bool e16 = !a.res1 && !a.res2 && !debug_route("no_ws_e16");
    if (a.r_w) {
        if (r.BM == 128)
            hipLaunchKernelGGL((conv3x3_ws2_kernel<7, T, 128, 0, true>), wgrid, dim3(512), ws2_lds(a, gw), s, a, gw, ilog2(gw.TW), ilog2(gw.TH), ntiles);
        else if (e16)
            hipLaunchKernelGGL((conv3x3_ws2_kernel<11, T, 256, 0, true, true>), wgrid, dim3(512), ws2_lds(a, gw), s, a, gw, ilog2(gw.TW), ilog2(gw.TH), ntiles);
        else
            hipLaunchKernelGGL((conv3x3_ws2_kernel<11, T, 256, 0, true>), wgrid, dim3(512), ws2_lds(a, gw), s, a, gw, ilog2(gw.TW), ilog2(gw.TH), ntiles);
    } else if (r.BM == 128)
        hipLaunchKernelGGL((conv3x3_ws2_kernel<7, T, 128>), wgrid, dim3(512), ws2_lds(a, gw), s, a, gw, ilog2(gw.TW), ilog2(gw.TH), ntiles);
    else if (e16)
        hipLaunchKernelGGL((conv3x3_ws2_kernel<11, T, 256, 0, false, true>), wgrid, dim3(512), ws2_lds(a, gw), s, a, gw, ilog2(gw.TW), ilog2(gw.TH), ntiles);
    else
        hipLaunchKernelGGL((conv3x3_ws2_kernel<11, T, 256>), wgrid, dim3(512), ws2_lds(a, gw), s, a, gw, ilog2(gw.TW), ilog2(gw.TH), ntiles);
    DMME_CHECK_LAUNCH();
    return DMME_OK;
}

template <typename T, bool ACC3 = false>
static int launch_pipe_t(const ConvRoute& r, int dtype, const ConvArgs& a, hipStream_t s) {
    const ConvTile& g = r.tile;
    const int ksplit = r.ksplit;
    const dim3 grid((unsigned)(g.tiles_m * g.tiles_n), (unsigned)ksplit);
    ConvArgs ad = a;
    bool dma = false;
    const size_t lds = pipe_launch_lds(dtype, a, r, &dma);
    ad.dma_b = dma ? 1 : 0;
    const int shTW = ilog2(g.TW), shTH = ilog2(g.TH);
    static bool attr_done[5] = {false, false, false, false, false};
    int rc = DMME_OK;
#define DMME_PIPE_CASE(IDX, BM_, BN_, GT_, UA_, LIM)                                                                          \
    case IDX:                                                                                                                 \
        if (!attr_done[IDX]) {                                                                                                \
            rc = set_lds_limit(conv3x3_pipe_kernel<T, BM_, BN_, GT_, UA_, ACC3>, (LIM) * 1024);                               \
            attr_done[IDX] = rc == DMME_OK;                                                                                   \
        }                                                                                                                     \
        if (rc == DMME_OK) hipLaunchKernelGGL((conv3x3_pipe_kernel<T, BM_, BN_, GT_, UA_, ACC3>), grid, dim3(256), lds, s, ad, g, shTW, shTH, ksplit); \
        break;
    switch (r.cand) {
        DMME_PIPE_CASE(0, 128, 128, 3, 8, 80)
        DMME_PIPE_CASE(1, 128, 64, 3, 8, 80)
        DMME_PIPE_CASE(2, 64, 64, 3, 8, 80)
        DMME_PIPE_CASE(3, 64, 64, 9, 11, 128)
        DMME_PIPE_CASE(4, 64, 64, 3, 10, 80)
    }
#undef DMME_PIPE_CASE
    if (rc != DMME_OK) return rc;
    DMME_CHECK_LAUNCH();
    if (ksplit > 1) {
        const int64_t total4 = (int64_t)a.N * a.Hout * a.Wout * (a.Cout / 4);
        hipLaunchKernelGGL(conv_splitk_finish_kernel<T>, dim3((unsigned)((total4 + 255) / 256)), dim3(256), 0, s, a, ksplit, total4);
        DMME_CHECK_LAUNCH();
    }
    return DMME_OK;
}

int launch_conv3x3(const ConvRoute& r, int dtype, const ConvArgs& a, hipStream_t s) {
    switch (r.family) {
        case CONV3X3_SPLIT: return launch_ws2_split(r, a, s);
        case CONV3X3_WS: return dtype == DMME_F16 ? launch_ws_t<f16>(r, a, s) : launch_ws_t<bf16>(r, a, s);
        case CONV3X3_KW: return launch_conv_kw(dtype, a, r.tile, r.NI, r.ring, r.BM, r.ksplit, s);
        default: break;
    }
    if (dtype == DMME_BF16) return launch_pipe_t<bf16>(r, dtype, a, s);
    if (dtype == DMME_F16) return launch_pipe_t<f16>(r, dtype, a, s);
    return a.x3 ? launch_pipe_t<float, true>(r, dtype, a, s) : launch_pipe_t<float>(r, dtype, a, s);
}

}
```

### diffusion-models-made-easy_amd/csrc/conv_route.hip

```cpp
#include <stdio.h>
#include <stdlib.h>

#include "conv_common.h"

namespace dmme {

ConvRoute conv_route(int dtype, const ConvArgs& a) {
    ConvRoute r{};
    if (conv_thin_route(dtype, a, r)) return r;
    if (conv1x1_split_route(dtype, a, r)) return r;
    if (conv1x1_domain(dtype, a) && (conv1x1_as_route(dtype, a, r) || conv1x1_tiled_route(dtype, a, r))) return r;
    if (conv3x3_split_route(dtype, a, r)) return r;
    if (conv3x3_pipe_route(dtype, a, r)) {
        if (!conv3x3_ws_route(dtype, a, r)) conv3x3_kw_route(dtype, a, r);
        return r;
    }
    if (conv_mfma_route(dtype, a, r)) return r;
    conv_generic_route(a, r);
    return r;
}

int launch_conv(const ConvRoute& r, int dtype, const ConvArgs& a, hipStream_t s) {
    DMME_REQUIRE(!a.r_w || r.rseg, DMME_ERR_UNSUPPORTED,
                 "conv with a residual segment: only the wave-specialised 3x3 kernel takes it, with raw channel counts inside its domain");
    switch (r.family) {
        case CONV_THIN: return launch_conv_out_thin(a, s);
        case CONV1X1_AS: return launch_conv1x1_as(a, s);
        case CONV1X1_SPLIT:
        case CONV1X1_TILED: return launch_conv1x1(r, dtype, a, s);
        case CONV3X3_SPLIT:
        case CONV3X3_WS:
        case CONV3X3_KW:
        case CONV3X3_PIPE: return launch_conv3x3(r, dtype, a, s);
        case CONV_MFMA: return launch_conv_mfma(r, dtype, a, s);
        default: return launch_conv_generic(dtype, a, s);
    }
}

int launch_conv(int dtype, const ConvArgs& a, hipStream_t s, int force) {
    ConvRoute r{};
    if (force == 0)
        r = conv_route(dtype, a);
    else if (force == 2)
        conv_mfma_route(dtype, a, r);
    return launch_conv(r, dtype, a, s);
}

void conv_label(const ConvRoute& r, int dtype, const ConvArgs& a, char* buf, int cap) {
    const char* tn = dtype == DMME_BF16 ? "bf16" : dtype == DMME_F16 ? "f16" : a.x3 ? "float:bf16x3" : "float";
    switch (r.family) {
        case CONV_THIN: snprintf(buf, (size_t)cap, a.mix == 3 ? "conv_out_thin_kernel<%d,f16x3>" : "conv_out_thin_kernel<%d>", a.Cout * 9 <= 32 ? 1 : 2); break;
        case CONV1X1_SPLIT: snprintf(buf, (size_t)cap, "conv1x1_split_kernel<128,128>"); break;
        case CONV1X1_AS: snprintf(buf, (size_t)cap, "conv1x1_as_kernel<%d>", (a.C1 + a.C2) / 64); break;
        case CONV1X1_TILED: snprintf(buf, (size_t)cap, "conv1x1_pipe_kernel<%s,%d,%d>", tn, r.BM, r.BN); break;
        case CONV3X3_SPLIT: snprintf(buf, (size_t)cap, a.mix == 2 ? "conv3x3_ws2_kernel<11,f16x3,src16>" : "conv3x3_ws2_kernel<11,f16x3>"); break;
        case CONV3X3_WS: snprintf(buf, (size_t)cap, r.BM == 128 ? (a.r_w ? "conv3x3_ws2_kernel<7,128,res>" : "conv3x3_ws2_kernel<7,128>") : a.r_w ? "conv3x3_ws2_kernel<11,res>" : "conv3x3_ws2_kernel<11>"); break;
        case CONV3X3_KW: snprintf(buf, (size_t)cap, "conv3x3_kw_kernel<%d,%d,%d>", r.NI, r.ring, r.BM); break;
        case CONV3X3_PIPE: snprintf(buf, (size_t)cap, "conv3x3_pipe_kernel<%s,%d,%d,%d,%d>", tn, r.BM, r.BN, r.GT, r.UA); break;
        case CONV_MFMA: snprintf(buf, (size_t)cap, "conv_mfma_kernel<%s,%d,%d,%d>", tn, a.taps, r.BM, r.BN); break;
        default: snprintf(buf, (size_t)cap, "%s<%s>", conv_generic_kernel_name(a), dtype == DMME_BF16 ? "bf16" : dtype == DMME_F16 ? "f16" : "float"); break;
    }
}

bool conv_stats_query(int dtype, const ConvArgs& a, int cg, int* tiles, int* px) {
    ConvArgs b = a;
    b.gn_part = nullptr;
    const ConvRoute r = conv_route(dtype, b);
    if (!r.stat_tiles || !stats_cols_ok(a, r.stat_bn, cg, r.vec)) return false;
    *tiles = r.stat_tiles;
    *px = r.stat_px;
    return true;
}

bool conv_gn_in_query(int dtype, const ConvArgs& a) {
    if (getenv("DMME_NO_GN_IN") || !is16(dtype)) return false;
    const ConvRoute r = conv_route(dtype, a);
    switch (r.family) {
        case CONV_THIN: return true;
        case CONV3X3_SPLIT:
        case CONV3X3_WS: return true;
        case CONV1X1_AS: return true;
        case CONV1X1_TILED: return conv1x1_tiled_gn_in_ok(a, r);
        case CONV3X3_KW: return !debug_route("no_gn_in_kw") && r.tile.TN == 1;
        case CONV3X3_PIPE: return conv3x3_pipe_gn_in_ok(dtype, a, r);
        default: return false;
    }
}

int conv_gn_direct_query(int dtype, const ConvArgs& a, const int* cg, int n) {
    if (a.mix || n < 1 || n > 2) return 0;
    const ConvRoute r = conv_route(dtype, a);
    const ConvTile& g = r.tile;
    if (r.family == CONV3X3_WS) {
        if (debug_route("no_gn_direct_ws") || g.TH != a.Hout || g.TW != a.Wout || r.BM != 256) return 0;
        const int cgs = a.gn_cg;
        if (cgs < 8 || cgs % 8 || 128 % cgs || !stats_cols_ok(a, 128, cgs, 8)) return 0;
        for (int k = 0; k < n; ++k) {
            const int f = cg[k] / cgs;
            if (cg[k] % cgs || (f != 1 && f != 2 && f != 4) || 128 % cg[k]) return 0;
        }
        return 2;
    }
    if (r.family != CONV3X3_KW && r.family != CONV3X3_PIPE) return 0;
    const int HW = a.Hout * a.Wout;
    if (a.out_silu || a.out_nchw || a.res2 || a.Cout % r.vec || HW > 64 || (HW & (HW - 1))) return 0;
    if (r.family == CONV3X3_KW) {
        if (a.up) return 0;
    } else {
        ConvArgs b = a;
// ... 15 lines not shown
```

### diffusion-models-made-easy_amd/csrc/kernels_generic.hip

```cpp
#include <stdlib.h>

#include <algorithm>

#include "common.h"

namespace dmme {

template <typename T>
__global__ void __launch_bounds__(256) conv_generic_kernel(ConvArgs a) {
    const int64_t total = (int64_t)a.N * a.Hout * a.Wout * a.Cout;
    const int Cin = a.C1 + a.C2;
    const int Hv = a.up ? 2 * a.Hin : a.Hin, Wv = a.up ? 2 * a.Win : a.Win;
    const int k = a.taps == 9 ? 3 : 1, pad = a.taps == 9 ? 1 : 0;
    for (int64_t idx = blockIdx.x * (int64_t)blockDim.x + threadIdx.x; idx < total;
         idx += (int64_t)gridDim.x * blockDim.x) {
        const int co = (int)(idx % a.Cout);
        int64_t p = idx / a.Cout;
        const int ow = (int)(p % a.Wout);
        p /= a.Wout;
        const int oh = (int)(p % a.Hout);
        const int n = (int)(p / a.Hout);
        const T* w = (const T*)a.w + (int64_t)co * a.taps * Cin;
        const float* sc = a.scale ? a.scale + (int64_t)n * Cin : nullptr;
        const float* sh = a.scale ? a.shift + (int64_t)n * Cin : nullptr;
// ... 809 lines not shown
        hipLaunchKernelGGL(pack_table_kernel<bf16>, dim3(n_items), dim3(256), 0, s, items_dev, ref_flat, (char*)packed);
    else if (dtype == DMME_F16)
        hipLaunchKernelGGL(pack_table_kernel<f16>, dim3(n_items), dim3(256), 0, s, items_dev, ref_flat, (char*)packed);
    else
        hipLaunchKernelGGL(pack_table_kernel<float>, dim3(n_items), dim3(256), 0, s, items_dev, ref_flat, (char*)packed);
    DMME_CHECK_LAUNCH();
    return DMME_OK;
}

template <typename T>
__global__ void __launch_bounds__(256) attn_fold_weights_kernel(const AttnFoldJob* __restrict__ jobs, AttnFoldJob one, char* __restrict__ packed) {
    const AttnFoldJob jb = jobs ? jobs[blockIdx.x] : one;
    const int C = jb.C, i = blockIdx.y, j = threadIdx.x;
    if (i >= C) return;
    const T* wq = (const T*)(packed + jb.wq);
    const T* wk = wq + (int64_t)C * C;
    const T* wv = wk + (int64_t)C * C;
    const T* wp = (const T*)(packed + jb.wp);
    const float* bq = (const float*)(packed + jb.bq);
    const float* bv = bq + 2 * C;
    const float s = 1.0f / sqrtf((float)C);
    if (j < C) {
        float m = 0.f, pv = 0.f;
        for (int o = 0; o < C; ++o) {
            m = fmaf((float)wk[(int64_t)o * C + i], (float)wq[(int64_t)o * C + j], m);
            pv = fmaf((float)wp[(int64_t)i * C + o], (float)wv[(int64_t)o * C + j], pv);
        }
        ((T*)(packed + jb.M))[(int64_t)i * C + j] = from_f<T>(m * s);
        ((T*)(packed + jb.wpv))[(int64_t)i * C + j] = from_f<T>(pv);
    }
    if (j == 0) {
        float c = 0.f, b2 = 0.f;
        for (int o = 0; o < C; ++o) {
            c = fmaf((float)wk[(int64_t)o * C + i], bq[o], c);
            b2 = fmaf((float)wp[(int64_t)i * C + o], bv[o], b2);
        }
        ((float*)(packed + jb.c))[i] = c * s;
        ((float*)(packed + jb.bias2))[i] = b2 + ((const float*)(packed + jb.bp))[i];
    }
}
int launch_attn_fold_weights(int dtype, const AttnFoldJob* jobs_dev, int n_jobs, int maxC, void* packed, hipStream_t s, const AttnFoldJob* one) {
    if (n_jobs == 0) return DMME_OK;
    DMME_REQUIRE((jobs_dev != nullptr) != (one != nullptr) && (!one || n_jobs == 1), DMME_ERR_INVALID, "attn_fold_weights: a device table, or one job by value");
    const AttnFoldJob j1 = one ? *one : AttnFoldJob{};
    DMME_REQUIRE(is16(dtype) && maxC >= 1 && maxC <= 256, DMME_ERR_UNSUPPORTED, "attn_fold_weights: 16-bit plans, blocks of at most 256 channels (got %d)", maxC);
    if (dtype == DMME_F16)
        hipLaunchKernelGGL(attn_fold_weights_kernel<f16>, dim3((unsigned)n_jobs, (unsigned)maxC), dim3(256), 0, s, jobs_dev, j1, (char*)packed);
    else
        hipLaunchKernelGGL(attn_fold_weights_kernel<bf16>, dim3((unsigned)n_jobs, (unsigned)maxC), dim3(256), 0, s, jobs_dev, j1, (char*)packed);
    DMME_CHECK_LAUNCH();
    return DMME_OK;
}

template <int DEPTH>
__global__ void __launch_bounds__(256) l2_stream_kernel(const uint4* __restrict__ buf, int nvec, int iters, unsigned* __restrict__ sink) {
    unsigned acc = 0;
    const int tid = threadIdx.x;
    for (int it = 0; it < iters; ++it) {
        for (int base = 0; base + DEPTH * 256 <= nvec; base += DEPTH * 256) {
            uint4 v[DEPTH];
#pragma unroll
            for (int d = 0; d < DEPTH; ++d) v[d] = buf[base + d * 256 + tid];
#pragma unroll
            for (int d = 0; d < DEPTH; ++d) acc ^= v[d].x ^ v[d].y ^ v[d].z ^ v[d].w;
        }
    }
    if (acc == 0x12345u) sink[blockIdx.x] = acc;
}
typedef __attribute__((address_space(3))) char l2s_lds_c;
template <int DEPTH>
__global__ void __launch_bounds__(256) l2_stream_dma_kernel(const uint4* __restrict__ buf, int nvec, int iters, unsigned* __restrict__ sink, int row_stride) {
    extern __shared__ __attribute__((aligned(16))) char lds[];
    const int tid = threadIdx.x, wave = tid >> 6;
    (void)wave;
    unsigned acc = 0;
    for (int it = 0; it < iters; ++it) {
        int gbase = 0;
        for (int base = 0; base + DEPTH * 256 <= nvec; base += DEPTH * 256) {
            if (row_stride) {
                gbase += DEPTH * 32 * row_stride;
                if (gbase + (DEPTH * 32 + 32) * row_stride >= nvec) gbase = 0;
            }
#pragma unroll
            for (int d = 0; d < DEPTH; ++d) {
#if defined(__HIP_DEVICE_COMPILE__)
                const unsigned l = (unsigned)__builtin_amdgcn_readfirstlane((int)((unsigned)(size_t)(l2s_lds_c*)lds + (unsigned)((d * 4 + wave) * 1024)));
                const int idx = row_stride ? gbase + (d * 32 + (tid >> 3)) * row_stride + (tid & 7) : base + d * 256 + tid;
                __builtin_amdgcn_global_load_lds(buf + idx, (l2s_lds_c*)(size_t)l, 16, 0, 0);
#endif
            }
#if defined(__HIP_DEVICE_COMPILE__)
            asm volatile("s_waitcnt vmcnt(0)" ::: "memory");
#endif
        }
        acc ^= reinterpret_cast<unsigned*>(lds)[tid];
    }
    if (acc == 0x12345u) sink[blockIdx.x] = acc;
}
typedef float f32x16_d __attribute__((ext_vector_type(16)));
typedef __bf16 bf16x8_d __attribute__((ext_vector_type(8)));
__global__ void __launch_bounds__(512, 1) mfma_valu_kernel(int mode, int iters, float* __restrict__ sink) {
    const int wave = threadIdx.x >> 6;
    float out = 0.f;
    if (wave < 4) {
        if (!(mode & 1)) return;
        bf16x8_d a, b;
// ... 215 lines not shown
```

### diffusion-models-made-easy_amd/csrc/plan.h

```cpp
#pragma once
#include <stdarg.h>
#include <stdlib.h>
#include <stdio.h>
#include <string.h>

#include <algorithm>
#include <memory>
#include <string>
#include <unordered_map>
#include <vector>

#include "common.h"
#include "lvl.h"

namespace dmme {

static inline int64_t align_up(int64_t v, int64_t a) { return (v + a - 1) / a * a; }

template <typename T>
class DevTable {
    T* p_ = nullptr;

public:
    DevTable() = default;
// ... 47 lines not shown
    int cout = 1, cin = 1, taps = 1;
    int64_t numel() const { return shape[0] * shape[1] * shape[2] * shape[3]; }
};

struct Tensor {
    int64_t off = 0;
    int C = 0, H = 0, W = 0;
    int f32 = 0;
    int64_t stats_off = -1;
    int stats_tiles = 0, stats_cnt = 0;
};

enum OpKind { OP_SINUS, OP_LINEAR, OP_GN, OP_CONV, OP_ATTN, OP_CAST, OP_LABEL };

struct Op {
    OpKind kind;
    int64_t lin_in = 0, lin_out = 0;
    int lin_K = 0, lin_N = 0, lin_w = -1, lin_b = -1, lin_silu = 0;
    int64_t lin_pre = -1;
    int gn_src1 = -1, gn_src2 = -1, gn_gamma = -1, gn_beta = -1;
    int64_t b_rowsum = 0, b_ab = 0;
    int64_t b_gnrows = -1;
    int gn_rows_deferred = 0;
    int64_t gn_scale = 0, gn_shift = 0, gn_mr = 0;
    int gn_mod_col = -1, gn_mod_C = 0;
    int64_t gn_act = -1;
    int gn_force_small = 0;
    int gn_consumer = -1;
    int gn_direct = 0;
    int gn_in_consumer = 0;
    int src1 = -1, src2 = -1;
    int w = -1, b = -1;
    int gn = -1;
    int pro_silu = 0, out_silu = 0;
    int64_t dmask_off = -1;
    int tproj_col = -1;
    int res1 = -1, res2 = -1;
    int dst = -1;
    int up = 0, stride = 1, taps = 9;
    int use_act = 0;
    int gd_n = 0, gd_gn[2] = {-1, -1}, gd_coff[2] = {0, 0};
    int gd_act = -1;
    int res_alias = 0;
    int rseg = -1, fused_away = 0;
    int wg_layer = -1;
    int64_t wg_act = -1;
    int bias_deferred = 0;
    int at_qkv = -1, at_out = -1, at_heads = 1;
    int64_t at_lse = 0;
    int at_proj = -1;
    int at_fold_qkv = -1;
    int folded_into = -1;
    int64_t fold_M = -1, fold_c = -1, fold_wpv = -1, fold_b2 = -1;
    int mix = 0, route_f32 = 0;
    int mix2 = 0;
    int cast_src = -1, cast_dst = -1;
    int lvl = -1, lvl_first = 0;
};

struct LvlRun {
    int op_first = 0, op_last = 0;
    int sh = 0, NG = 0, NGS = 0, GB = 1, NJ = 1;
    std::vector<LvlOp> ops;
    std::vector<std::pair<int, int>> made;
    DevTable<LvlOp> ops_dev;
    std::vector<LvlOp> ops_nograd;
    DevTable<LvlOp> ops_nograd_dev;
    int raw_skipped = 0;
    DevTable<unsigned> sync_dev;
    double flops = 0, bytes = 0;
};

}

using namespace dmme;

struct dmme_plan {
    dmme_unet_cfg cfg;
    int B, H, W, dtype, device;
    int x3 = 0;
    int mix = 0;
    int out_channels = 0;
    int head_src = -1, p_hgw = -1, p_hgb = -1, p_hw = -1, p_hb = -1;
    int64_t bws_hpool = 0, bws_hrows = 0;
    int cond = 0, p_lemb = -1, label_op = -1;
    std::vector<Param> params;
    std::vector<Tensor> tensors;
    std::vector<Op> ops;
    std::unordered_map<std::string, int> named;
    int64_t ref_numel = 0, packed_bytes = 0, ws_bytes = 0, dropmask_numel = 0;
    int64_t ws_tsin = 0, ws_th1 = 0, ws_temb = 0, ws_tproj = 0, ws_gnpart = 0;
    int64_t ws_mark = 0;
    int64_t ws_tz1 = -1, ws_tz2 = -1;
    int64_t ws_splitk = 0, splitk_floats = 0;
    int tproj_cols = 0;
    int64_t tproj_w_off = 0, tproj_b_off = 0;
    int freqs_param = -1;
    DevTable<PackItem> items_dev;
    int n_items = 0;
    int n_launches = 0;
    struct TBlock { int tw, tb, col, cout; };
    std::vector<TBlock> tblocks;
    int p_l1w = -1, p_l1b = -1, p_l2w = -1, p_l2b = -1;
    int64_t packed_bwd_bytes = 0, bws_bytes = 0;
    std::vector<int64_t> gt_off;
    int64_t bws_zero = 0, bws_zero_bytes = 0, bws_wimage = 0, bws_gnS = 0, bws_zpage = 0;
    DevTable<PackItem> items_unpack_dev;
    int n_items_unpack = 0;
    int64_t bws_sink = 0, sink_half = 0;
    int64_t bws_tmp = 0, bws_dy = 0, bws_rowsum = 0, bws_dtproj = 0, bws_dtemb = 0, bws_dh1 = 0, bws_z = 0, bws_wT = 0, bws_attP = 0,
            bws_attdS = 0;
    DevTable<PackItem> items_bwd_dev;
    int n_items_bwd = 0;
    struct WgGroup {
        int taps = 0;
        std::vector<WgLayer> layers;
        std::vector<WgJob> jobs;
        DevTable<WgLayer> layers_dev;
        DevTable<WgJob> jobs_dev;
        int dma = 0;
        int stride = 1;
    } wg[3];
    struct GradBucket {
        int op_lo = 0, op_hi = 0;
        WgGroup wg[3];
        int col0 = 0, col1 = 0, bias0 = 0, bias1 = 0;
        std::vector<std::pair<int, int>> unpack, tcols;
        std::vector<std::pair<int64_t, int64_t>> ranges;
    };
    std::vector<GradBucket> gb;
    std::vector<int64_t> tp_tiles;
    DevTable<int64_t> tp_tiles_dev;
    int tp_n64 = 0;
    std::vector<BiasJob> bias_jobs;
    DevTable<BiasJob> bias_jobs_dev;
    std::vector<ColJob> col_jobs;
    DevTable<ColJob> col_jobs_dev;
    std::vector<LvlRun> lvl_runs;
    int lvl_max_wg = LVL_MAX_WG;
    PinnedWord err_host;
    mutable const void* nograd_ws = nullptr;
    std::vector<AttnFoldJob> fold_jobs;
    DevTable<AttnFoldJob> fold_jobs_dev;
    int fold_maxC = 0, n_launches_nograd = 0;
    mutable const void* fold_packed = nullptr;
    int pred = DMME_PRED_EPS, pred_T = 0;
    const float* pred_ab = nullptr;
    int thr_mode = DMME_THRESHOLD_NONE, thr_T = 0, thr_k = 0;
    float thr_frac = 0.f;
    const float* thr_table = nullptr;
    void* thr_scratch = nullptr;
};

namespace dmme {

constexpr int kR32TwoPassDefault = 0;
static inline int conv_dt(const dmme_plan* P, const Op& o) { return o.route_f32 ? DMME_F32 : P->dtype; }
static inline int wg_index(const Op& o) { return o.taps == 1 ? 1 : o.stride == 2 ? 2 : 0; }

void fill_conv(const dmme_plan* P, const Op& o, const char* packed, const float* x, float* y, char* ws, const float* drop_masks, int nt, ConvArgs& a,
               bool fwd = false);
bool gn_from_parts(const dmme_plan* P, const Op& o);
void assign_levels(dmme_plan* P);
void assign_rseg(dmme_plan* P);
int run_level(const dmme_plan* P, const LvlRun& R, const char* pk, char* ws, int nt, const float* drop_masks, hipStream_t s, bool keep_ctx = true);
void assign_lvl_nograd(dmme_plan* P);
void assign_attn_fold(dmme_plan* P);
int lvl_check(const dmme_plan* P, const char* where, hipStream_t stream = nullptr, bool have_stream = false);
void build_unpack_items(const dmme_plan* P, std::vector<PackItem>& items);
void plan_backward(dmme_plan* P);

}
```

### diffusion-models-made-easy_amd/csrc/plan.hip

```cpp
#include "plan.h"

#include <functional>
#include <map>
#include <mutex>

namespace dmme {

static thread_local char g_err[512] = "";
void set_error(const char* fmt, ...) {
    va_list ap;
    va_start(ap, fmt);
    vsnprintf(g_err, sizeof(g_err), fmt, ap);
    va_end(ap);
}

int debug_route(const char* key, int dflt) {
    const char* e = getenv("DMME_DEBUG_ROUTE");
    if (!e || !*e) return dflt;
    const size_t kl = strlen(key);
    for (const char* p = e; *p;) {
        const char* end = strchr(p, ',');
        const size_t len = end ? (size_t)(end - p) : strlen(p);
        if (len >= kl && !strncmp(p, key, kl) && (len == kl || p[kl] == '=')) return len == kl ? 1 : atoi(p + kl + 1);
        if (!end) break;
// ... 921 lines not shown
    for (int ai = 1; ai < (int)P->ops.size(); ++ai) {
        Op& at = P->ops[ai];
        if (at.kind != OP_ATTN || at.at_proj < 0 || at.at_heads != 1 || at.lvl >= 0) continue;
        Op& qc = P->ops[ai - 1];
        const Op& pr = P->ops[at.at_proj];
        if (qc.kind != OP_CONV || qc.dst != at.at_qkv || qc.taps != 1 || qc.src1 < 0 || qc.src2 >= 0 || qc.gn < 0 || qc.pro_silu || qc.out_silu || qc.dmask_off >= 0 ||
            qc.tproj_col >= 0 || qc.res1 >= 0 || qc.res2 >= 0 || qc.up || qc.stride != 1 || qc.gd_n > 0 || qc.mix || qc.route_f32 || qc.fused_away || qc.rseg >= 0 ||
            qc.use_act || qc.lvl >= 0 || pr.res1 != qc.src1)
            continue;
        const Op& gn = P->ops[qc.gn];
        const Tensor& tx = P->tensors[qc.src1];
        const int C = tx.C, groups = P->cfg.num_groups;
        if (gn.kind != OP_GN || gn.gn_src1 != qc.src1 || gn.gn_src2 >= 0 || gn.gn_mod_col >= 0 || gn.gn_act >= 0 || tx.f32 ||
            (gn.gn_in_consumer && (tx.stats_off < 0 || tx.stats_tiles > 32)) || P->tensors[at.at_qkv].C != 3 * C || P->params[qc.w].pack_code >= 0 || P->params[pr.w].pack_code >= 0)
            continue;
        bool only_here = true;
        for (int oi = 0; oi < (int)P->ops.size() && only_here; ++oi) {
            const Op& o = P->ops[oi];
            if (oi == ai) continue;
            if (o.kind == OP_CONV && (o.src1 == at.at_qkv || o.src2 == at.at_qkv || o.res1 == at.at_qkv || o.res2 == at.at_qkv)) only_here = false;
            if (o.kind == OP_GN && (o.gn_src1 == at.at_qkv || o.gn_src2 == at.at_qkv)) only_here = false;
            if (o.kind == OP_ATTN && o.at_qkv == at.at_qkv) only_here = false;
            if (o.kind == OP_CAST && o.cast_src == at.at_qkv) only_here = false;
        }
        const Tensor& td = P->tensors[pr.dst];
        const bool stats = td.stats_off >= 0;
        if (!only_here || !attn_fold_shape_ok(P->dtype, P->B, tx.H * tx.W, C, stats ? C / groups : 0, stats ? td.stats_tiles : 0)) continue;
        at.at_fold_qkv = ai - 1;
        qc.folded_into = ai;
        at.fold_M = cur;
        cur = align_up(cur + (int64_t)C * C * es, 256);
        at.fold_wpv = cur;
        cur = align_up(cur + (int64_t)C * C * es, 256);
        at.fold_c = cur;
        cur = align_up(cur + (int64_t)C * 4, 256);
        at.fold_b2 = cur;
        cur = align_up(cur + (int64_t)C * 4, 256);
        AttnFoldJob jb{};
        jb.wq = P->params[qc.w].packed_off;
        jb.bq = P->params[qc.b].packed_off;
        jb.wp = P->params[pr.w].packed_off;
        jb.bp = P->params[pr.b].packed_off;
        jb.M = at.fold_M;
        jb.c = at.fold_c;
        jb.wpv = at.fold_wpv;
        jb.bias2 = at.fold_b2;
        jb.C = C;
        P->fold_jobs.push_back(jb);
        if (C > P->fold_maxC) P->fold_maxC = C;
    }
    P->packed_bytes = cur;
}

int run_gn(const dmme_plan* P, const Op& o, const char* pk, char* ws, int nt, const float* drop_masks, hipStream_t s) {
    if (o.gn_direct || o.gn_in_consumer) return DMME_OK;
    const float* tsh = o.gn_mod_col >= 0 ? (const float*)(ws + P->ws_tproj) + o.gn_mod_col : nullptr;
    const float* tsc = tsh ? tsh + o.gn_mod_C : nullptr;
    int rc;
    const Tensor& t1 = P->tensors[o.gn_src1];
    const void* s1 = ws + t1.off;
    const void* s2 = o.gn_src2 >= 0 ? ws + P->tensors[o.gn_src2].off : nullptr;
    const int C2 = o.gn_src2 >= 0 ? P->tensors[o.gn_src2].C : 0;
    const float* gam = (const float*)(pk + P->params[o.gn_gamma].packed_off);
    const float* bet = (const float*)(pk + P->params[o.gn_beta].packed_off);
    float* sc = (float*)(ws + o.gn_scale);
    float* sh = (float*)(ws + o.gn_shift);
    if (gn_from_parts(P, o)) {
        const Tensor* t2 = o.gn_src2 >= 0 ? &P->tensors[o.gn_src2] : nullptr;
        return launch_gn_finalize_parts((const float*)(ws + t1.stats_off), t1.stats_tiles, t1.stats_cnt, t1.C,
                                        t2 ? (const float*)(ws + t2->stats_off) : nullptr, t2 ? t2->stats_tiles : 0,
                                        t2 ? t2->stats_cnt : 0, C2, P->B, P->cfg.num_groups, gam, bet, 1e-5f, sc, sh,
                                        (float*)(ws + o.gn_mr), tsh, tsc, P->tproj_cols, nt, s);
    }
    const int gdt = t1.f32 ? DMME_F32 : P->dtype;
    if (gn_fast_supported(gdt, P->B, t1.H * t1.W, t1.C, C2, P->cfg.num_groups)) {
        void* act = nullptr;
        int act_silu = 0;
        const float* dm = nullptr;
        if (o.gn_act >= 0) {
            const Op& cv = P->ops[o.gn_consumer];
            act = ws + o.gn_act;
            act_silu = cv.pro_silu;
            if (cv.dmask_off >= 0 && drop_masks) dm = drop_masks + cv.dmask_off;
        }
        rc = launch_gn_fast(gdt, s1, s2, P->B, t1.H * t1.W, t1.C, C2, P->cfg.num_groups, gam, bet, 1e-5f, sc, sh,
                            (float*)(ws + o.gn_mr), (float*)(ws + P->ws_gnpart), s, act, act_silu, dm);
    }
    else
        rc = launch_gn_generic(gdt, s1, s2, P->B, t1.H * t1.W, t1.C, C2, P->cfg.num_groups, gam, bet, 1e-5f, sc, sh,
                               (float*)(ws + o.gn_mr), s);
    if (rc != DMME_OK || !tsh) return rc;
    return launch_gn_modulate(sc, sh, tsh, tsc, P->tproj_cols, nt, P->B, o.gn_mod_C, s);
}

int run_op(const dmme_plan* P, const Op& o, const char* pk, const float* x, const int64_t* t, int nt, float* y,
           char* ws, const float* drop_masks, hipStream_t s, bool keep_ctx, const int64_t* labels = nullptr, int* status = nullptr) {
    if (o.lvl >= 0) return o.lvl_first ? run_level(P, P->lvl_runs[o.lvl], pk, ws, nt, drop_masks, s, keep_ctx) : DMME_OK;
    if (o.fused_away) return DMME_OK;
    const bool fold = !keep_ctx && P->fold_packed == (const void*)pk;
    if (fold && o.kind == OP_CONV && o.folded_into >= 0) return DMME_OK;
    switch (o.kind) {
        case OP_SINUS:
            return launch_time_sinusoid(t, nt, (const float*)(pk + P->params[P->freqs_param].packed_off),
                                        P->cfg.pos_dim / 2, (float*)(ws + P->ws_tsin), s, (unsigned*)(ws + P->ws_mark),
                                        keep_ctx ? kFwdMarkKeep : kFwdMarkNograd);
        case OP_LINEAR: {
            const char* w = o.lin_w >= 0 ? pk + P->params[o.lin_w].packed_off : pk + P->tproj_w_off;
            const float* b = (const float*)(o.lin_b >= 0 ? pk + P->params[o.lin_b].packed_off : pk + P->tproj_b_off);
            if (nt > 4)
                return launch_small_gemm(P->dtype, 0, (const float*)(ws + o.lin_in), o.lin_K, w, o.lin_K, nt, o.lin_N, o.lin_K, b, o.lin_silu,
                                         (float*)(ws + o.lin_out), o.lin_N, s, o.lin_pre >= 0 ? (float*)(ws + o.lin_pre) : nullptr);
            return launch_linear_wave(P->dtype, (const float*)(ws + o.lin_in), nt, o.lin_K, w, b, o.lin_N, o.lin_silu,
                                      (float*)(ws + o.lin_out), s);
        }
        case OP_LABEL: {
            float* z2 = (float*)(ws + P->ws_tz2);
            return launch_label_cond(z2, nt, (const float*)(pk + P->params[P->p_lemb].packed_off), labels, P->B, P->cfg.num_classes, P->cfg.emb_dim,
                                     (float*)(ws + P->ws_temb), nt == P->B ? z2 : nullptr, status, s);
        }
        case OP_GN:
            return run_gn(P, o, pk, ws, nt, drop_masks, s);
        case OP_CONV: {
            ConvArgs a{};
            fill_conv(P, o, pk, x, y, ws, drop_masks, nt, a, true);
            return launch_conv(conv_dt(P, o), a, s);
        }
        case OP_CAST: {
            const Tensor& ts = P->tensors[o.cast_src];
            return launch_cast_f32_to_16(P->dtype, (const float*)(ws + ts.off), (int64_t)P->B * ts.H * ts.W * ts.C, ws + P->tensors[o.cast_dst].off, s);
        }
        case OP_ATTN: {
            const Tensor& q = P->tensors[o.at_qkv];
            const int S = q.H * q.W, C = q.C / 3;
            if (fold && o.at_fold_qkv >= 0) {
                ConvArgs a{}, qa{};
                fill_conv(P, P->ops[o.at_proj], pk, x, y, ws, drop_masks, nt, a, true);
                fill_conv(P, P->ops[o.at_fold_qkv], pk, x, y, ws, drop_masks, nt, qa, true);
                return launch_attn_fold(P->dtype, qa.src1, P->B, S, C, qa.has_gni ? &qa.gni : nullptr, qa.scale, qa.shift, pk + o.fold_M, (const float*)(pk + o.fold_c), pk + o.fold_wpv,
                                        (const float*)(pk + o.fold_b2), a.res1, a.dst, a.gn_part, a.gn_tiles, a.gn_cg, s);
            }
            if (o.at_proj >= 0) {
                ConvArgs a{};
                fill_conv(P, P->ops[o.at_proj], pk, x, y, ws, drop_masks, nt, a, true);
                return launch_attn_proj(P->dtype, ws + q.off, P->B, S, C, keep_ctx ? ws + P->tensors[o.at_out].off : nullptr, (float*)(ws + o.at_lse), a.w, a.bias,
                                        a.res1, a.dst, a.gn_part, a.gn_tiles, a.gn_cg, s);
            }
            if (P->x3 && attn_x3_supported(P->B, S, C, o.at_heads))
                return launch_attn_x3(ws + q.off, P->B, S, C, o.at_heads, ws + P->tensors[o.at_out].off, s);
            if (o.at_heads > 1) {
                if (attn_heads_mfma_supported(P->dtype, P->B, S, C, o.at_heads))
                    return launch_attn_heads_mfma(P->dtype, ws + q.off, P->B, S, C, o.at_heads, ws + P->tensors[o.at_out].off, (float*)(ws + o.at_lse), s);
                return launch_attn_heads(P->dtype, ws + q.off, P->B, S, C, o.at_heads, ws + P->tensors[o.at_out].off, s);
            }
            if (attn_mfma_supported(P->dtype, P->B, S, C))
                return launch_attn_mfma(P->dtype, ws + q.off, P->B, S, C, ws + P->tensors[o.at_out].off, (float*)(ws + o.at_lse), s);
            return launch_attn_generic(P->dtype, ws + q.off, P->B, S, C, ws + P->tensors[o.at_out].off, s);
        }
    }
    return DMME_OK;
}
void op_account(const dmme_plan* P, const Op& o, char* label, int cap, double* flops, double* bytes) {
    const double es = (double)dtype_size(P->dtype);
    const char* tn = P->dtype == DMME_BF16 ? "bf16" : P->dtype == DMME_F16 ? "f16" : "float";
    const double B = P->B;
    *flops = 0;
    *bytes = 0;
    if (o.lvl >= 0) {
        const LvlRun& R = P->lvl_runs[o.lvl];
        if (o.lvl_first) {
            snprintf(label, cap, "lvl_engine_kernel<%dx%d>", 1 << R.sh, 1 << R.sh);
            *flops = R.flops;
            *bytes = R.bytes;
        } else {
            snprintf(label, cap, "(level engine)");
        }
        return;
    }
// ... 103 lines not shown
                     DMME_ERR_INVALID, "channels_per_depth[%d]=%d not divisible by num_groups=%d", d,
                     cfg->channels_per_depth[d], cfg->num_groups);
    return DMME_OK;
}

static int check_mix_kernels(const dmme_plan* P) {
    if (!P->mix) return DMME_OK;
    for (const Op& o : P->ops) {
        if (o.kind != OP_CONV || !(o.mix || o.route_f32)) continue;
        ConvArgs a{};
        fill_conv(P, o, (const char*)4096, (const float*)4096, (float*)4096, (char*)4096, nullptr, 1, a);
        const bool ok = !o.mix || conv_route(P->dtype, a).family == (o.mix == 3 ? CONV_THIN : o.mix == 4 ? CONV1X1_SPLIT : CONV3X3_SPLIT);
        DMME_REQUIRE(ok, DMME_ERR_UNSUPPORTED, "plan_create: precision fp16r32 has no kernel for the %dx%d conv %d+%d -> %d channels on the %dx%d level (B = %d)",
                     o.taps == 9 ? 3 : 1, o.taps == 9 ? 3 : 1, a.C1, a.C2, a.Cout, a.Hout, a.Wout, P->B);
    }
    return DMME_OK;
}

static int count_launches(const dmme_plan* P, bool nograd = false) {
    int n = 0;
    for (const Op& o : P->ops) {
        if (o.fused_away || (nograd && o.folded_into >= 0)) continue;
        if (o.lvl >= 0)
            n += o.lvl_first;
        else if (o.kind == OP_GN)
            n += !(o.gn_direct || o.gn_in_consumer);
        else
            ++n;
    }
    return n;
}

#define DMME_TRY(expr)                 \
    do {                               \
        if (int rc_ = (expr)) return rc_; \
    } while (0)

static int upload_tables(dmme_plan* P) {
    DMME_CHECK_HIP(hipSetDevice(P->device));
    std::vector<PackItem> items, bitems, uitems;
    build_pack_items(P, items);
    build_pack_items_bwd(P, bitems);
    build_unpack_items(P, uitems);
    P->n_items = (int)items.size();
    P->n_items_bwd = (int)bitems.size();
    P->n_items_unpack = (int)uitems.size();
    DMME_TRY(P->items_dev.upload(items));
    DMME_TRY(P->items_bwd_dev.upload(bitems));
    DMME_TRY(P->items_unpack_dev.upload(uitems));
    DMME_TRY(P->tp_tiles_dev.upload(P->tp_tiles));
    DMME_TRY(P->col_jobs_dev.upload(P->col_jobs));
    DMME_TRY(P->bias_jobs_dev.upload(P->bias_jobs));
    if (!P->fold_jobs.empty()) DMME_TRY(P->fold_jobs_dev.upload(P->fold_jobs));
    std::vector<dmme_plan::WgGroup*> all_groups{&P->wg[0], &P->wg[1], &P->wg[2]};
    for (auto& B_ : P->gb)
        for (int k = 0; k < 3; ++k) all_groups.push_back(&B_.wg[k]);
    for (dmme_plan::WgGroup* G : all_groups) {
        if (G->jobs.empty()) continue;
        DMME_TRY(G->layers_dev.upload(G->layers));
        DMME_TRY(G->jobs_dev.upload(G->jobs));
    }
    DMME_TRY(P->err_host.alloc());
    for (LvlRun& R : P->lvl_runs) {
        DMME_TRY(R.ops_dev.upload(R.ops));
        if (R.raw_skipped > 0) DMME_TRY(R.ops_nograd_dev.upload(R.ops_nograd));
        DMME_TRY(R.sync_dev.zeroed(16 + R.ops.size() * 2 * (size_t)R.NG * LVL_NS));
    }
    return DMME_OK;
}

}

extern "C" {

DMME_API const char* dmme_last_error(void) { return g_err; }
DMME_API int dmme_version(void) { return 119; }
DMME_API int dmme_device_count(void) {
    int n = 0;
    if (hipGetDeviceCount(&n) != hipSuccess) return 0;
    return n;
}

DMME_API int dmme_unet_plan_create(const dmme_unet_cfg* cfg, int B, int H, int W, int dtype, int device, dmme_plan** out) {
    DMME_REQUIRE(cfg && out, DMME_ERR_INVALID, "plan_create: null argument");
    DMME_TRY(check_cfg(cfg, B, H, W, dtype));
    std::unique_ptr<dmme_plan> owned(new dmme_plan());
    dmme_plan* P = owned.get();
    P->cfg = *cfg;
    if (cfg->arch == DMME_ARCH_DDPM_COND) {
        P->cond = 1;
        P->cfg.arch = DMME_ARCH_DDPM;
    }
    P->B = B;
    P->H = H;
    P->W = W;
    P->x3 = dtype == DMME_BF16X3;
    P->mix = dtype == DMME_F16R32;
    P->dtype = P->x3 ? DMME_F32 : P->mix ? DMME_F16 : dtype;
    P->device = device;
    DMME_TRY(build_plan(P));
    DMME_TRY(check_mix_kernels(P));
    assign_levels(P);
    const bool fused_gn = !getenv("DMME_NO_FUSED_GN");
    if (fused_gn) assign_stats(P);
    if (fused_gn && !getenv("DMME_NO_GN_DIRECT")) assign_direct(P);
    if (!getenv("DMME_NO_PREACT")) assign_preact(P);
    if (fused_gn) assign_gn_in(P);
    assign_rseg(P);
    assign_attn_proj(P);
    assign_lvl_nograd(P);
    assign_attn_fold(P);
    P->n_launches = count_launches(P);
    P->n_launches_nograd = count_launches(P, true);
    plan_backward(P);
    if (device >= 0) DMME_TRY(upload_tables(P));
    *out = owned.release();
    return DMME_OK;
}

DMME_API void dmme_unet_plan_destroy(dmme_plan* plan) { delete plan; }

DMME_API int dmme_unet_plan_num_params(const dmme_plan* plan) { return plan ? (int)plan->params.size() : 0; }

DMME_API int dmme_unet_plan_param_info(const dmme_plan* plan, int index, char* name, int name_cap, int* ndim,
                              int64_t shape[4], int64_t* ref_offset, int* is_buffer) {
    DMME_REQUIRE(plan && index >= 0 && index < (int)plan->params.size(), DMME_ERR_INVALID, "param_info: bad index %d", index);
    const Param& p = plan->params[index];
    if (name && name_cap > 0) {
        strncpy(name, p.name.c_str(), (size_t)name_cap - 1);
        name[name_cap - 1] = 0;
    }
    if (ndim) *ndim = p.ndim;
    if (shape)
        for (int i = 0; i < 4; ++i) shape[i] = p.shape[i];
    if (ref_offset) *ref_offset = p.ref_off;
    if (is_buffer) *is_buffer = p.is_buffer ? 1 : 0;
    return DMME_OK;
}

DMME_API int64_t dmme_unet_plan_ref_numel(const dmme_plan* plan) { return plan ? plan->ref_numel : 0; }
DMME_API int64_t dmme_unet_plan_packed_bytes(const dmme_plan* plan) { return plan ? plan->packed_bytes : 0; }
DMME_API int64_t dmme_unet_plan_workspace_bytes(const dmme_plan* plan) { return plan ? plan->ws_bytes : 0; }
DMME_API int64_t dmme_unet_plan_dropmask_numel(const dmme_plan* plan) { return plan ? plan->dropmask_numel : 0; }
DMME_API int dmme_unet_plan_out_channels(const dmme_plan* plan) { return plan ? plan->out_channels : 0; }
DMME_API int dmme_unet_plan_num_launches(const dmme_plan* plan) { return plan ? plan->n_launches : 0; }
DMME_API int dmme_unet_plan_num_launches_nograd(const dmme_plan* plan) { return plan ? plan->n_launches_nograd : 0; }
DMME_API int dmme_unet_plan_num_folded(const dmme_plan* plan) { return plan ? (int)plan->fold_jobs.size() : 0; }

DMME_API int dmme_unet_pack_params(const dmme_plan* plan, const float* ref_flat, void* packed, void* stream) {
    DMME_REQUIRE(plan && ref_flat && packed, DMME_ERR_INVALID, "pack_params: null argument");
    DMME_REQUIRE(plan->items_dev, DMME_ERR_INVALID, "pack_params: plan was created without a device");
    if (plan->fold_packed == packed) plan->fold_packed = nullptr;
    return launch_pack_table(plan->dtype, plan->items_dev.get(), plan->n_items, ref_flat, packed, (hipStream_t)stream);
}

DMME_API int dmme_unet_pack_folded(const dmme_plan* plan, void* packed, void* stream) {
    DMME_REQUIRE(plan && packed, DMME_ERR_INVALID, "pack_folded: null argument");
    DMME_REQUIRE(plan->items_dev, DMME_ERR_INVALID, "pack_folded: plan was created without a device");
    if (plan->fold_jobs.empty()) return DMME_OK;
    const int rc = launch_attn_fold_weights(plan->dtype, plan->fold_jobs_dev.get(), (int)plan->fold_jobs.size(), plan->fold_maxC, packed, (hipStream_t)stream);
    if (rc == DMME_OK) plan->fold_packed = packed;
    return rc;
}

static int unet_forward_impl(const dmme_plan* plan, const void* packed, const float* x, const int64_t* t, int t_len,
                      float* y, void* workspace, const float* drop_masks, void* stream, bool keep_ctx, const int64_t* labels = nullptr,
                      int* status = nullptr) {
    DMME_REQUIRE(plan && packed && x && t && y && workspace, DMME_ERR_INVALID, "unet_forward: null argument");
    DMME_REQUIRE((plan->cond != 0) == (labels != nullptr), DMME_ERR_INVALID,
                 plan->cond ? "unet_forward: a class-conditional plan (DMME_ARCH_DDPM_COND) takes labels: call dmme_unet_forward_cond / dmme_cfg_chain_step"
                            : "unet_forward_cond: the plan is not class-conditional (DMME_ARCH_DDPM_COND)");
    DMME_REQUIRE(t_len == 1 || t_len == plan->B, DMME_ERR_INVALID,
                 "unet_forward: timestep tensor of length %d does not broadcast against batch %d", t_len, plan->B);
    {
        const int rc = lvl_check(plan, "unet_forward", (hipStream_t)stream, true);
        if (rc != DMME_OK) return rc;
    }
    hipStream_t s = (hipStream_t)stream;
    const dmme_plan* P = plan;
    const char* pk = (const char*)packed;
    char* ws = (char*)workspace;
    const int nt = t_len;
    if (keep_ctx) {
        if (plan->nograd_ws == workspace) plan->nograd_ws = nullptr;
    } else {
        plan->nograd_ws = workspace;
    }
    for (int oi = 0; oi < (int)P->ops.size(); ++oi) {
        const int rc = run_op(P, P->ops[oi], pk, x, t, P->cond && oi > P->label_op ? P->B : nt, y, ws, drop_masks, s, keep_ctx, labels, status);
        if (rc != DMME_OK) return rc;
    }
    if (P->head_src >= 0) {
        const Tensor& tt = P->tensors[P->head_src];
        return launch_cls_head_fwd(P->dtype, ws + tt.off, P->B, tt.H * tt.W, tt.C, P->cfg.num_groups, (const float*)(pk + P->params[P->p_hgw].packed_off),
                                   (const float*)(pk + P->params[P->p_hgb].packed_off), (const float*)(pk + P->params[P->p_hw].packed_off),
                                   (const float*)(pk + P->params[P->p_hb].packed_off), P->out_channels, y, s);
    }
    return DMME_OK;
}
DMME_API int dmme_unet_forward(const dmme_plan* plan, const void* packed, const float* x, const int64_t* t, int t_len,
                      float* y, void* workspace, const float* drop_masks, void* stream) {
    return unet_forward_impl(plan, packed, x, t, t_len, y, workspace, drop_masks, stream, true);
}
DMME_API int dmme_unet_forward_nograd(const dmme_plan* plan, const void* packed, const float* x, const int64_t* t, int t_len,
                      float* y, void* workspace, const float* drop_masks, void* stream) {
    return unet_forward_impl(plan, packed, x, t, t_len, y, workspace, drop_masks, stream, false);
}

DMME_API int dmme_unet_forward_cond(const dmme_plan* plan, const void* packed, const float* x, const int64_t* t, int t_len, const int64_t* labels,
                                    float* y, void* workspace, const float* drop_masks, int keep_ctx, int* status, void* stream) {
    DMME_REQUIRE(labels, DMME_ERR_INVALID, "unet_forward_cond: null argument (labels)");
    return unet_forward_impl(plan, packed, x, t, t_len, y, workspace, drop_masks, stream, keep_ctx != 0, labels, status);
}
// ... 552 lines not shown
                             (hipStream_t)stream);
}

DMME_API int dmme_attention(int dtype, const void* qkv, int N, int S, int C, void* out, int force_generic, void* stream) {
    DMME_REQUIRE(qkv && out && N > 0 && S > 0 && C > 0, DMME_ERR_INVALID, "attention: bad argument");
    if (dtype == DMME_BF16X3) {
        if (!force_generic && attn_x3_supported(N, S, C, 1)) return launch_attn_x3(qkv, N, S, C, 1, out, (hipStream_t)stream);
        dtype = DMME_F32;
    }
    if (!force_generic && attn_mfma_supported(dtype, N, S, C)) return launch_attn_mfma(dtype, qkv, N, S, C, out, nullptr, (hipStream_t)stream);
    return launch_attn_generic(dtype, qkv, N, S, C, out, (hipStream_t)stream);
}

DMME_API int dmme_attention_proj(int dtype, const void* qkv, int N, int S, int C, const void* w, const float* bias, const void* res, void* dst, void* ctx,
                                 float* gn_part, int gn_cg, void* stream) {
    DMME_REQUIRE(qkv && w && bias && res && dst && N > 0 && S > 0 && C > 0, DMME_ERR_INVALID, "attention_proj: bad argument");
    return launch_attn_proj(dtype, qkv, N, S, C, ctx, nullptr, w, bias, res, dst, gn_part, S / 32, gn_cg, (hipStream_t)stream, g_stamps);
}

DMME_API int dmme_attention_fold(int dtype, int C, const void* wqkv, const float* bqkv, const void* wp, const float* bp, void* M, float* c, void* wpv, float* bias2,
                                 void* stream) {
    DMME_REQUIRE(wqkv && bqkv && wp && bp && M && c && wpv && bias2 && C > 0, DMME_ERR_INVALID, "attention_fold: bad argument");
    AttnFoldJob jb{};
    jb.wq = (int64_t)(intptr_t)wqkv;
    jb.bq = (int64_t)(intptr_t)bqkv;
    jb.wp = (int64_t)(intptr_t)wp;
    jb.bp = (int64_t)(intptr_t)bp;
    jb.M = (int64_t)(intptr_t)M;
    jb.c = (int64_t)(intptr_t)c;
    jb.wpv = (int64_t)(intptr_t)wpv;
    jb.bias2 = (int64_t)(intptr_t)bias2;
    jb.C = C;
    return launch_attn_fold_weights(dtype, nullptr, 1, C, nullptr, (hipStream_t)stream, &jb);
}
DMME_API int dmme_attention_block(int dtype, const void* x, int N, int S, int C, const float* parts, int part_tiles, int part_cnt, int groups, const float* gamma,
                                  const float* beta, float eps, float* scale, float* shift, const void* M, const float* c, const void* wpv, const float* bias2,
                                  const void* res, void* dst, float* gn_part, int gn_cg, void* stream) {
    DMME_REQUIRE(x && M && c && wpv && bias2 && res && dst && N > 0 && S > 0 && C > 0, DMME_ERR_INVALID, "attention_block: bad argument");
    GnIn gni{};
    if (parts) {
        DMME_REQUIRE(gamma && beta && groups > 0 && part_tiles > 0 && part_cnt > 0, DMME_ERR_INVALID, "attention_block: partials without gamma / beta / geometry");
        gni.p1 = parts;
        gni.t1 = part_tiles;
        gni.cnt1 = part_cnt;
        gni.C1 = C;
        gni.groups = groups;
        gni.gamma = gamma;
        gni.beta = beta;
        gni.eps = eps;
    }
    return launch_attn_fold(dtype, x, N, S, C, parts ? &gni : nullptr, scale, shift, M, c, wpv, bias2, res, dst, gn_part, S / 32, gn_cg, (hipStream_t)stream, g_stamps);
}

DMME_API int dmme_attention_heads(int dtype, const void* qkv, int N, int S, int C, int heads, void* out, int force_generic, void* stream) {
    DMME_REQUIRE(qkv && out && N > 0 && S > 0 && C > 0 && heads > 0 && C % heads == 0, DMME_ERR_INVALID, "attention_heads: bad argument");
    if (dtype == DMME_BF16X3) {
        if (!force_generic && attn_x3_supported(N, S, C, heads)) return launch_attn_x3(qkv, N, S, C, heads, out, (hipStream_t)stream);
        dtype = DMME_F32;
    }
    if (!force_generic && attn_heads_mfma_supported(dtype, N, S, C, heads))
        return launch_attn_heads_mfma(dtype, qkv, N, S, C, heads, out, nullptr, (hipStream_t)stream);
    return launch_attn_heads(dtype, qkv, N, S, C, heads, out, (hipStream_t)stream);
}

DMME_API int dmme_nchw_to_nhwc(int dtype, const float* src, int N, int C, int HW, void* dst, void* stream) {
    DMME_REQUIRE(src && dst, DMME_ERR_INVALID, "nchw_to_nhwc: null argument");
    return launch_nchw_to_nhwc(dtype, src, N, C, HW, dst, (hipStream_t)stream);
}
DMME_API int dmme_nhwc_to_nchw(int dtype, const void* src, int N, int C, int HW, float* dst, void* stream) {
    DMME_REQUIRE(src && dst, DMME_ERR_INVALID, "nhwc_to_nchw: null argument");
    return launch_nhwc_to_nchw(dtype, src, N, C, HW, dst, (hipStream_t)stream);
}
DMME_API int dmme_pack_weight(int dtype, const float* src, int Cout, int Cin, int taps, void* dst, void* stream) {
    DMME_REQUIRE(src && dst, DMME_ERR_INVALID, "pack_weight: null argument");
    return launch_pack_weight(dtype, src, Cout, Cin, taps, dst, (hipStream_t)stream);
}

DMME_API int dmme_event_create(void** ev) {
    DMME_REQUIRE(ev, DMME_ERR_INVALID, "event_create: null");
    hipEvent_t e;
    DMME_CHECK_HIP(hipEventCreate(&e));
    *ev = (void*)e;
    return DMME_OK;
}
DMME_API int dmme_event_record(void* ev, void* stream) {
    DMME_CHECK_HIP(hipEventRecord((hipEvent_t)ev, (hipStream_t)stream));
    return DMME_OK;
}
DMME_API int dmme_event_elapsed_ms(void* start, void* stop, float* ms) {
    DMME_CHECK_HIP(hipEventSynchronize((hipEvent_t)stop));
    DMME_CHECK_HIP(hipEventElapsedTime(ms, (hipEvent_t)start, (hipEvent_t)stop));
    return DMME_OK;
}
DMME_API int dmme_event_destroy(void* ev) {
    DMME_CHECK_HIP(hipEventDestroy((hipEvent_t)ev));
    return DMME_OK;
}

}
```

### include/dmme_hip.h

```cpp
#ifndef DMME_HIP_H
#define DMME_HIP_H

#include <stddef.h>
#include <stdint.h>

#if defined(DMME_BUILD)
#define DMME_API __attribute__((visibility("default")))
#else
#define DMME_API
#endif

#ifdef __cplusplus
extern "C" {
#endif

typedef enum {
    DMME_OK = 0,
    DMME_ERR_INVALID = -1,
    DMME_ERR_UNSUPPORTED = -2,
    DMME_ERR_HIP = -3,
    DMME_ERR_NOMEM = -4
} dmme_status;

typedef enum { DMME_F32 = 0, DMME_BF16 = 1, DMME_BF16X3 = 2, DMME_F16 = 3, DMME_F16R32 = 4 } dmme_dtype;

typedef enum {
    DMME_ARCH_DDPM = 0,
    DMME_ARCH_IDDPM = 1,
    DMME_ARCH_CLASSIFIER = 2,
    DMME_ARCH_DDPM_COND = 3
} dmme_unet_arch;

typedef struct {
    int in_channels;
    int pos_dim;
    int emb_dim;
    int num_groups;
    float dropout;
    int num_depths;
    int channels_per_depth[8];
    int num_blocks;
    int num_attention_depths;
    int attention_depths[8];
    int arch;
    int num_heads;
    int num_classes;
} dmme_unet_cfg;

typedef struct dmme_plan dmme_plan;

DMME_API const char* dmme_last_error(void);
DMME_API int dmme_version(void);
DMME_API int dmme_device_count(void);

DMME_API int dmme_unet_plan_create(const dmme_unet_cfg* cfg, int B, int H, int W, int dtype, int device, dmme_plan** out);
DMME_API void dmme_unet_plan_destroy(dmme_plan* plan);

DMME_API int dmme_unet_plan_num_params(const dmme_plan* plan);
DMME_API int dmme_unet_plan_param_info(const dmme_plan* plan, int index, char* name, int name_cap, int* ndim,
                              int64_t shape[4], int64_t* ref_offset, int* is_buffer);
DMME_API int64_t dmme_unet_plan_ref_numel(const dmme_plan* plan);
DMME_API int64_t dmme_unet_plan_packed_bytes(const dmme_plan* plan);
DMME_API int64_t dmme_unet_plan_workspace_bytes(const dmme_plan* plan);
DMME_API int64_t dmme_unet_plan_dropmask_numel(const dmme_plan* plan);
DMME_API int dmme_unet_plan_out_channels(const dmme_plan* plan);
DMME_API int dmme_unet_plan_num_launches(const dmme_plan* plan);
DMME_API int dmme_unet_plan_num_launches_nograd(const dmme_plan* plan);
DMME_API int dmme_unet_plan_num_folded(const dmme_plan* plan);

DMME_API int dmme_unet_pack_params(const dmme_plan* plan, const float* ref_flat, void* packed, void* stream);
DMME_API int dmme_unet_pack_folded(const dmme_plan* plan, void* packed, void* stream);

DMME_API int dmme_unet_forward(const dmme_plan* plan, const void* packed, const float* x, const int64_t* t, int t_len,
                      float* y, void* workspace, const float* drop_masks, void* stream);
DMME_API int dmme_unet_forward_nograd(const dmme_plan* plan, const void* packed, const float* x, const int64_t* t, int t_len,
                      float* y, void* workspace, const float* drop_masks, void* stream);

DMME_API int dmme_unet_forward_cond(const dmme_plan* plan, const void* packed, const float* x, const int64_t* t, int t_len, const int64_t* labels,
                                    float* y, void* workspace, const float* drop_masks, int keep_ctx, int* status, void* stream);

DMME_API int dmme_unet_plan_num_ops(const dmme_plan* plan);
DMME_API int dmme_unet_plan_level_info(const dmme_plan* plan, char* buf, int cap);
DMME_API int dmme_unet_plan_check(const dmme_plan* plan);
DMME_API int dmme_unet_plan_op_info(const dmme_plan* plan, int index, char* label, int label_cap, double* flops,
                           double* bytes);
DMME_API int dmme_unet_forward_profiled(const dmme_plan* plan, const void* packed, const float* x, const int64_t* t,
                               int t_len, float* y, void* workspace, const float* drop_masks, void* stream,
                               float* op_ms);

DMME_API int64_t dmme_unet_plan_packed_bwd_bytes(const dmme_plan* plan);
DMME_API int64_t dmme_unet_plan_bwd_workspace_bytes(const dmme_plan* plan);
DMME_API int dmme_unet_pack_params_bwd(const dmme_plan* plan, const float* ref_flat, void* packed_bwd, void* stream);
DMME_API int dmme_unet_backward(const dmme_plan* plan, const void* packed, const void* packed_bwd, const float* x,
                       const int64_t* t, int t_len, const float* d_y, void* workspace, void* bwd_workspace,
                       const float* drop_masks, float* grad_flat, float* d_x, void* stream);
typedef void (*dmme_bucket_fn)(void* user, int bucket, int64_t offset, int64_t numel);
DMME_API int dmme_unet_backward_buckets(const dmme_plan* plan, const void* packed, const void* packed_bwd, const float* x,
                               const int64_t* t, int t_len, const float* d_y, void* workspace, void* bwd_workspace,
                               const float* drop_masks, float* grad_flat, float* d_x, void* stream, dmme_bucket_fn ready, void* user);
DMME_API int dmme_unet_backward_input(const dmme_plan* plan, const void* packed, const void* packed_bwd, const float* x, const int64_t* t,
                                      int t_len, const float* d_y, void* workspace, void* bwd_workspace, const float* drop_masks, float* d_x,
                                      void* stream);
DMME_API int dmme_unet_plan_grad_buckets(const dmme_plan* plan, int64_t* offsets, int64_t* numels, int* bucket_of, int cap);
DMME_API int dmme_unet_backward_cond(const dmme_plan* plan, const void* packed, const void* packed_bwd, const float* x, const int64_t* t, int t_len,
                                     const int64_t* labels, const float* d_y, void* workspace, void* bwd_workspace, const float* drop_masks,
                                     float* grad_flat, float* d_x, void* stream, dmme_bucket_fn ready, void* user);
DMME_API int dmme_unet_backward_input_cond(const dmme_plan* plan, const void* packed, const void* packed_bwd, const float* x, const int64_t* t,
                                           int t_len, const int64_t* labels, const float* d_y, void* workspace, void* bwd_workspace,
                                           const float* drop_masks, float* d_x, void* stream);
DMME_API int dmme_unet_plan_bwd_summary(const dmme_plan* plan, char* buf, int cap);
DMME_API int dmme_debug_level_stamps(void* buf, int run, int workgroup);
DMME_API int dmme_debug_mfma_valu(int mode, int iters, int blocks, void* sink, void* stream);
DMME_API int dmme_debug_issue_probe(int kind, int n_inner, int iters, int flags, int blocks, void* sink, const void* src, void* stream);
DMME_API int dmme_debug_l2_stream(const void* buf, int64_t bytes, int iters, int mode, int depth, int blocks, void* sink, void* stream);
DMME_API int dmme_grad_norm(const float* grad, int64_t numel, float* norm_out, float* scratch, void* stream);
DMME_API int dmme_adam_step(float* param, const float* grad, float* exp_avg, float* exp_avg_sq, float* ema, int64_t numel,
                            float lr, float beta1, float beta2, float eps, int step, const float* grad_norm, float max_norm,
                            float ema_decay, float grad_scale, void* stream);
DMME_API int dmme_amp_init(float* amp_state, float init_scale, void* stream);
DMME_API int dmme_amp_scale(float* grad, int64_t numel, const float* amp_state, void* stream);
DMME_API int dmme_adam_step_amp(float* param, const float* grad, float* exp_avg, float* exp_avg_sq, float* ema, int64_t numel, float lr, float beta1,
// ... 153 lines not shown
                    const float* coef, int B, int64_t chw, float w_simple, float w_vlb, float* loss, float* d_out,
                    float grad_scale, float* scratch, void* stream);


DMME_API int dmme_iddpm_loss_rows(const float* model_out, const float* x_t, const float* x_0, const float* target, const int64_t* t,
                                  const float* coef, int T, const float* weight, int B, int64_t chw, float w_simple, float w_vlb, float* loss,
                                  float* rows, float* d_out, float grad_scale, int* status, float* scratch, void* stream);

DMME_API int dmme_iddpm_prior_rows(const float* x_0, int B, int64_t chw, float alpha_bar_T, float* prior, void* stream);

DMME_API int dmme_tsampler_draw(const float* hist, const int* count, int T, int H, float uniform_prob, uint64_t philox_seed,
                                uint64_t philox_offset, int B, int64_t* t, float* weight, float* p, void* stream);

DMME_API int dmme_tsampler_update(float* hist, int* count, int T, int H, const int64_t* t, const float* L, int B, int* status, void* stream);

typedef struct {
    int dtype;
    int N, Hin, Win;
    int C1, C2;
    int upsample;
    int stride;
    int taps;
    int Cout;
    int pro_silu;
    int out_silu;
    int nt;
    int tproj_ld;
    int in_nchw;
    int out_nchw;
    int force_generic;
} dmme_conv_desc;

DMME_API int dmme_conv2d(const dmme_conv_desc* d, const void* src1, const void* src2, const void* weight,
                const float* bias, const float* scale, const float* shift, const float* dmask,
                const float* tproj, const void* res1, const void* res2, int R1, void* dst, void* stream);

DMME_API int dmme_conv2d_res(const dmme_conv_desc* d, const void* src1, const void* src2, const void* weight, const float* bias,
                const float* scale, const float* shift, const float* dmask, const void* r_src1, const void* r_src2, int r_C1,
                int r_C2, const void* r_weight, const float* r_bias, void* dst, void* stream);

DMME_API int dmme_groupnorm_scale_shift(int dtype, const void* src1, const void* src2, int N, int HW, int C1, int C2,
                               int groups, const float* gamma, const float* beta, float eps, float* scale,
                               float* shift, float* partial_scratch, int force_generic, void* stream);

DMME_API int dmme_attention(int dtype, const void* qkv, int N, int S, int C, void* out, int force_generic, void* stream);
DMME_API int dmme_attention_proj(int dtype, const void* qkv, int N, int S, int C, const void* w, const float* bias, const void* res,
                                 void* dst, void* ctx, float* gn_part, int gn_cg, void* stream);
DMME_API int dmme_attention_fold(int dtype, int C, const void* wqkv, const float* bqkv, const void* wp, const float* bp, void* M, float* c, void* wpv,
                                 float* bias2, void* stream);
DMME_API int dmme_attention_block(int dtype, const void* x, int N, int S, int C, const float* parts, int part_tiles, int part_cnt, int groups,
                                  const float* gamma, const float* beta, float eps, float* scale, float* shift, const void* M, const float* c,
                                  const void* wpv, const float* bias2, const void* res, void* dst, float* gn_part, int gn_cg, void* stream);

DMME_API int dmme_attention_heads(int dtype, const void* qkv, int N, int S, int C, int heads, void* out, int force_generic, void* stream);

DMME_API int dmme_nchw_to_nhwc(int dtype, const float* src, int N, int C, int HW, void* dst, void* stream);
DMME_API int dmme_nhwc_to_nchw(int dtype, const void* src, int N, int C, int HW, float* dst, void* stream);
DMME_API int dmme_pack_weight(int dtype, const float* src, int Cout, int Cin, int taps, void* dst, void* stream);

DMME_API int dmme_debug_set_stamps(void* buf);

DMME_API int dmme_event_create(void** ev);
DMME_API int dmme_event_record(void* ev, void* stream);
DMME_API int dmme_event_elapsed_ms(void* start, void* stop, float* ms);
DMME_API int dmme_event_destroy(void* ev);

#ifdef __cplusplus
}
#endif
#endif
```

Before: 477.2 denoising steps/s (one step = UNet forward + DDPM update on a batch of 128), summed over GPUs.

## Fold nearest-upsample into 3x3 conv as four-phase 2x2 convolutions

Nearest-neighbour 2x upsampling followed by a 3x3 conv is rewritten as four sub-pixel phases, each a 2x2 conv on the low-resolution input. The per-phase weights are precomputed at pack time. A folded variant of the warp-specialised conv kernel reads 4 taps instead of 9 and scatters outputs to interleaved pixels. This cuts upsample-conv MACs and input reads by more than half, at the cost of extra packed weight storage and a more complex pipeline schedule.

```diff
diff --git a/diffusion-models-made-easy_amd/_lib.py b/diffusion-models-made-easy_amd/_lib.py
--- a/diffusion-models-made-easy_amd/_lib.py
+++ b/diffusion-models-made-easy_amd/_lib.py
@@ -90,6 +90,7 @@
     "dmme_unet_plan_num_launches": (_i, [_vp]),
     "dmme_unet_plan_num_launches_nograd": (_i, [_vp]),
     "dmme_unet_plan_num_folded": (_i, [_vp]),
+    "dmme_unet_plan_num_up_folded": (_i, [_vp]),
     "dmme_unet_pack_params": (_i, [_vp, _vp, _vp, _vp]),
     "dmme_unet_pack_folded": (_i, [_vp, _vp, _vp]),
     "dmme_unet_forward": (_i, [_vp, _vp, _vp, _vp, _i, _vp, _vp, _vp, _vp]),
@@ -189,6 +190,8 @@
     "dmme_attention": (_i, [_i, _vp, _i, _i, _i, _vp, _i, _vp]),
     "dmme_attention_proj": (_i, [_i, _vp, _i, _i, _i, _vp, _vp, _vp, _vp, _vp, _vp, _i, _vp]),
     "dmme_attention_fold": (_i, [_i, _i, _vp, _vp, _vp, _vp, _vp, _vp, _vp, _vp, _vp]),
+    "dmme_up_fold_weights": (_i, [_i, _vp, _i, _i, _vp, _vp]),
+    "dmme_conv2d_up_folded": (_i, [_i, _vp, _i, _i, _i, _i, _vp, _vp, _i, _vp, _vp, _i, C.POINTER(_i), _vp]),
     "dmme_attention_block": (_i, [_i, _vp, _i, _i, _i, _vp, _i, _i, _i, _vp, _vp, _f, _vp, _vp, _vp, _vp, _vp, _vp, _vp, _vp, _vp, _i, _vp]),
     "dmme_attention_heads": (_i, [_i, _vp, _i, _i, _i, _i, _vp, _i, _vp]),
     "dmme_nchw_to_nhwc": (_i, [_i, _vp, _i, _i, _i, _vp, _vp]),
diff --git a/diffusion-models-made-easy_amd/csrc/common.h b/diffusion-models-made-easy_amd/csrc/common.h
--- a/diffusion-models-made-easy_amd/csrc/common.h
+++ b/diffusion-models-made-easy_amd/csrc/common.h
@@ -204,6 +204,7 @@
     const void* r_w;
     const float* r_bias;
     int r_C1, r_C2;
+    int fold_up;
 };
 
 int launch_mfma_valu(int mode, int iters, int blocks, float* sink, hipStream_t s);
@@ -239,6 +240,7 @@
     int NI, ring;
     int ksplit;
     int rseg;
+    int fold;
     int vec;
     int stat_bn;
     int stat_px;
@@ -262,6 +264,7 @@
 bool conv3x3_pipe_route(int dtype, const ConvArgs& a, ConvRoute& r);
 bool conv3x3_ws_route(int dtype, const ConvArgs& a, ConvRoute& r);
 bool conv3x3_kw_route(int dtype, const ConvArgs& a, ConvRoute& r);
+bool conv3x3_ws_fold_route(int dtype, const ConvArgs& a, ConvRoute& r);
 bool conv_mfma_route(int dtype, const ConvArgs& a, ConvRoute& r);
 void conv_generic_route(const ConvArgs& a, ConvRoute& r);
 bool conv_mfma_supported(int dtype, const ConvArgs& a);
@@ -312,6 +315,11 @@
     int64_t M, c, wpv, bias2;
     int32_t C, pad;
 };
+struct UpFoldJob {
+    int64_t w, dst;
+    int32_t Cout, Cin;
+};
+int launch_up_fold_weights(int dtype, const UpFoldJob* jobs_dev, int n_jobs, int max_rows, void* packed, hipStream_t s, const UpFoldJob* one = nullptr);
 bool attn_fold_shape_ok(int dtype, int N, int S, int C, int gn_cg, int gn_tiles);
 int launch_attn_fold(int dtype, const void* x, int N, int S, int C, const GnIn* gni, const float* scale, const float* shift, const void* M, const float* c,
                      const void* wpv, const float* bias2, const void* res, void* dst, float* gn_part, int gn_tiles, int gn_cg, hipStream_t s,
diff --git a/diffusion-models-made-easy_amd/csrc/conv_pipe.hip b/diffusion-models-made-easy_amd/csrc/conv_pipe.hip
--- a/diffusion-models-made-easy_amd/csrc/conv_pipe.hip
+++ b/diffusion-models-made-easy_amd/csrc/conv_pipe.hip
@@ -345,8 +345,8 @@
                 *reinterpret_cast<uint2*>(row + mi * 64 * (BN + kStage16Pad) + 32 * ni + 8 * q) = make_uint2(__builtin_bit_cast(unsigned, lo), __builtin_bit_cast(unsigned, hi));
             }
 }
-struct WsTile { int n0, oy0, ox0, co0, ts; };
-__device__ __forceinline__ WsTile ws_tile_of(const ConvTile& g, int shTW, int shTH, int kt, int bn) {
+struct WsTile { int n0, oy0, ox0, co0, ts, wco, ph; };
+__device__ __forceinline__ WsTile ws_tile_of(const ConvTile& g, int shTW, int shTH, int kt, int bn, int fold_cout = 0) {
     const int t = (int)blockIdx.x + kt * (int)gridDim.x;
     const int tile_n = t % g.tiles_n, tile_m = t / g.tiles_n;
     const int tiles_img = g.tiles_x * g.tiles_y;
@@ -357,6 +357,12 @@
     r.ox0 = (sp % g.tiles_x) << shTW;
     r.co0 = tile_n * bn;
     r.ts = sp;
+    r.wco = r.co0;
+    r.ph = 0;
+    if (fold_cout) {
+        r.ph = r.co0 / fold_cout;
+        r.co0 -= r.ph * fold_cout;
+    }
     return r;
 }
 
@@ -386,7 +392,7 @@
 struct WsSplit<T, 2> {
     typedef float ts;
 };
-template <int PIPE_UA, typename T = bf16, int BM = 256, int SPLIT = 0, bool RSEG = false, bool E16 = false>
+template <int PIPE_UA, typename T = bf16, int BM = 256, int SPLIT = 0, bool RSEG = false, bool E16 = false, bool FOLD = false>
 __global__ void __launch_bounds__(512, 1) conv3x3_ws2_kernel(ConvArgs a, ConvTile g, int shTW, int shTH, int ntiles) {
     constexpr int KC = 64, EPV = 8, BN = 128, MI = BM / 64, NI = 2, UB = BN / 32;
     constexpr bool CDMA = WS_CDMA != 0;
@@ -394,6 +400,8 @@
     static_assert(!(SCHED2 && WS_HYB != 0), "the hybrid tap ownership counts the halo loads of the two-unit schedule");
     static_assert(!E16 || (SPLIT == 0 && BM == 256 && sizeof(T) == 2), "16-bit staging: 16-bit tensors, 256-pixel tiles");
     static_assert(!RSEG || (SPLIT == 0 && sizeof(T) == 2), "residual segment: 16-bit tensors");
+    static_assert(!FOLD || (E16 && !RSEG && CDMA && WS_HYB == 0), "folded up-sampling form: 16-bit staging, no residual segment, consumer-requested taps");
+    constexpr int TPW = FOLD ? 4 : 9;
     constexpr int KCR = SPLIT ? 32 : KC;
     constexpr int EPR = SPLIT ? 4 : EPV;
     typedef typename WsSplit<T, SPLIT>::ts TS;
@@ -425,7 +433,7 @@
 #define WS_BUFA(p) (lds + (((p) & 1) ? offA1 : 0))
 #define WS_RING(slot) (lds + offR + (slot) * R_BYTES)
 #define WS_PAR(kt) (par_base + ((kt) & 1) * 4 * Cin)
-#define WS_TILE(kt) ws_tile_of(g, shTW, shTH, (kt), BN)
+#define WS_TILE(kt) ws_tile_of(g, shTW, shTH, (kt), BN, FOLD ? a.Cout : 0)
     typedef WsTile TileXY;
     const int tid = threadIdx.x, lane = tid & 63, wave = tid >> 6;
     const bool producer = wave >= 4;
@@ -502,10 +510,13 @@
             auto pix_of = [&](int m) -> int {                                                                                      \
                 const int mm = m + 128 * p;                                                                                        \
                 const int tx = mm & mTW, ty = (mm >> shTW) & mTH;                                                                  \
+                  \
+                if constexpr (FOLD) return ((TT).n0 * 2 * a.Hout + 2 * ((TT).oy0 + ty) + ((TT).ph >> 1)) * 2 * a.Wout + 2 * ((TT).ox0 + tx) + ((TT).ph & 1); \
                 return ((TT).n0 * a.Hout + (TT).oy0 + ty) * a.Wout + (TT).ox0 + tx;                                                \
             };                                                                                                                     \
+             \
             conv_epilogue_store<TS, 128, BN, 512, true>(a, (TT).co0, (TT).n0, pix_of, reinterpret_cast<float*>(st16 + p * 128 * (BN + kStage16Pad)), \
-                                                        2 * (TT).ts + p, nullptr, a.n_gno ? p : -1, gn_carry);                     \
+                                                        2 * (FOLD ? (TT).ph * g.tiles_x * g.tiles_y + (TT).ts : (TT).ts) + p, nullptr, a.n_gno ? p : -1, gn_carry); \
             WS_ESTAMP()                                                                                                            \
         }                                                                                                                          \
         lds_barrier();                                                                 \
@@ -519,7 +530,7 @@
 #pragma unroll
         for (int i = 0; i < PIPE_UA; ++i) a_sw[i] = (urow + 32 * i) * A_PITCH + cu * (SPLIT ? 8 : 16);
 #pragma unroll
-        for (int k4 = 0; k4 < UB; ++k4) b_vo[k4] = (unsigned)(((urow + 32 * k4) * 9 * CinW + (cu ^ ((urow >> 1) & 7)) * EPV) * 2);
+        for (int k4 = 0; k4 < UB; ++k4) b_vo[k4] = (unsigned)(((urow + 32 * k4) * TPW * CinW + (cu ^ ((urow >> 1) & 7)) * EPV) * 2);
         auto pix_unit = [&](int i, const TileXY& t) __attribute__((always_inline)) -> int {
             const int row = urow + 32 * i;
             const int hy = (int)__umulhi((unsigned)row, g.magic_w), hx = row - hy * g.HWd;
@@ -638,7 +649,7 @@
             }
 #endif
             const unsigned lbase = (unsigned)(size_t)(lds_c*)dstR + (unsigned)(pw * 8 * ROW_DATA);
-            const char* ub = wbase + ((size_t)co0 * 9 * CinW + (size_t)t * CinW + (size_t)c * KC) * 2;
+            const char* ub = wbase + ((size_t)co0 * TPW * CinW + (size_t)t * CinW + (size_t)c * KC) * 2;
 #pragma unroll
             for (int k4 = 0; k4 < UB; ++k4) {
                 const unsigned l = (unsigned)__builtin_amdgcn_readfirstlane((int)(lbase + (unsigned)(32 * k4 * ROW_DATA)));
@@ -683,8 +694,8 @@
                 set_pix(i, tcur);
                 load_A(i, 0);
             }
-            dma_tap(WS_RING(0), tcur.co0, 0, 0);
-            dma_tap(WS_RING(1), tcur.co0, 0, 1);
+            dma_tap(WS_RING(0), tcur.wco, 0, 0);
+            dma_tap(WS_RING(1), tcur.wco, 0, 1);
             WS_FILL_PAR(0)
             __syncthreads();
             load_par(WS_PAR(0), 0);
@@ -868,10 +879,57 @@
             }                                                                                                           \
         }                                                                                                               \
     }
+#define WS_PSTAGE_F(TP)                                                                                                 \
+    {                                                                                                                   \
+        WS_PST()                                                                                                        \
+        const bool last_c = cc + 1 == nchunks;                                                                          \
+        const bool have_n = !(last_c && kt + 1 == K);                                                                   \
+        const int nk = have_n ? (last_c ? kt + 1 : kt) : kt, nc = have_n ? (last_c ? 0 : cc + 1) : cc;                  \
+        const bool last_n = nc + 1 == nchunks;                                                                          \
+        const bool have_l = have_n && !(last_n && nk + 1 == K);                                                         \
+        const int lk = have_l ? (last_n ? nk + 1 : nk) : nk, lc = have_l ? (last_n ? 0 : nc + 1) : nc;                  \
+        WS_A_ARRIVED(TP)                                                                                                \
+        WS_A_ARRIVED((TP) + 4)                                                                                          \
+        if constexpr ((TP) + 8 < PIPE_UA) { WS_A_ARRIVED((TP) + 8) }                                                    \
+        __builtin_amdgcn_sched_barrier(0);                                                                              \
+        WS_PST()                                                                                                        \
+        {                                                                                                               \
+            const bool do_store = have_n;                                                                               \
+            char* dstA = WS_BUFA(cg + 1);                                                                               \
+            const bool new_tile = have_l && lc == 0;                                                                    \
+            const TileXY tnn = lk == kt ? tcur : tnext;                                                                 \
+            if ((TP) == 0) load_par(WS_PAR(nk), nc* KCR);                                                               \
+            WS_A_UNIT(TP)                                                                                               \
+            WS_A_UNIT((TP) + 4)                                                                                         \
+            if constexpr ((TP) + 8 < PIPE_UA) { WS_A_UNIT((TP) + 8) }                                                   \
+        }                                                                                                               \
+        __builtin_amdgcn_sched_barrier(0);                                                                              \
+        WS_PST()                                                                                                        \
+        wait_lgkm_all();               \
+        WS_PST()                                                                                                        \
+        __builtin_amdgcn_s_barrier();                                                                                   \
+        if ((TP) == 3) {                                                                                                \
+            ++cg;                                                                                                       \
+            if (++cc == nchunks) {                                                                                      \
+                WS2_EPILOGUE16(tcur, kt, ;)                                                                             \
+                cc = 0;                                                                                                 \
+                ++kt;                                                                                                   \
+                tcur = tnext;                                                                                           \
+                tnext = WS_TILE(kt + 1 < K ? kt + 1 : kt);                                                              \
+            }                                                                                                           \
+        }                                                                                                               \
+    }
         const int GCH = K * nchunks;
-        for (int ch = 0; ch < GCH; ++ch) {
-            WS_PSTAGE(0) WS_PSTAGE(1) WS_PSTAGE(2) WS_PSTAGE(3) WS_PSTAGE(4) WS_PSTAGE(5) WS_PSTAGE(6) WS_PSTAGE(7) WS_PSTAGE(8)
-        }
+        if constexpr (FOLD) {
+            for (int ch = 0; ch < GCH; ++ch) {
+                WS_PSTAGE_F(0) WS_PSTAGE_F(1) WS_PSTAGE_F(2) WS_PSTAGE_F(3)
+            }
+        } else {
+            for (int ch = 0; ch < GCH; ++ch) {
+                WS_PSTAGE(0) WS_PSTAGE(1) WS_PSTAGE(2) WS_PSTAGE(3) WS_PSTAGE(4) WS_PSTAGE(5) WS_PSTAGE(6) WS_PSTAGE(7) WS_PSTAGE(8)
+            }
+        }
+#undef WS_PSTAGE_F
 #ifdef WS_PSTAMPS
         if (a.stamps && ptid == 0 && blockIdx.x == 0)
             for (int i = 0; i < p_i; ++i) a.stamps[128 + i] = pst_lds[i];
@@ -914,10 +972,10 @@
 #pragma unroll
     for (int k4 = 0; k4 < UB; ++k4) {
         const int urow_ = wave * 8 + (lane >> 3);
-        cb_vo[k4] = (unsigned)(((urow_ + 32 * k4) * 9 * CinW + ((lane & 7) ^ ((urow_ >> 1) & 7)) * EPV) * 2);
+        cb_vo[k4] = (unsigned)(((urow_ + 32 * k4) * TPW * CinW + ((lane & 7) ^ ((urow_ >> 1) & 7)) * EPV) * 2);
     }
     auto cdma = [&](int slot, int co0, int c, int t) __attribute__((always_inline)) {
-        const char* ub = (const char*)a.w + ((size_t)co0 * 9 * CinW + (size_t)t * CinW + (size_t)c * KC) * 2;
+        const char* ub = (const char*)a.w + ((size_t)co0 * TPW * CinW + (size_t)t * CinW + (size_t)c * KC) * 2;
         const unsigned lbase = (unsigned)(size_t)(lds_c*)WS_RING(slot) + (unsigned)(wave * 8 * ROW_DATA);
 #pragma unroll
         for (int k4 = 0; k4 < UB; ++k4)
@@ -997,6 +1055,38 @@
     }
         const TileXY tn = WS_TILE(kt + 1 < K ? kt + 1 : kt);
         const bool three = !a.mix2;
+        if constexpr (FOLD) {
+            const int ph_b = ((t.ph >> 1) * g.HWd + (t.ph & 1)) * A_PITCH;
+#pragma unroll
+            for (int s = 0; s < 8; ++s) {
+                const int tp = s & 3;
+                const char* ldsA = WS_BUFA(cg + (s >> 2));
+                const char* ldsR = WS_RING(s % 3);
+                const int tap_b = ph_b + ((tp >> 1) * g.HWd + (tp & 1)) * A_PITCH;
+                const char* pa[MI];
+#pragma unroll
+                for (int mi = 0; mi < MI; ++mi) pa[mi] = ldsA + a_row[mi] + tap_b;
+                uint4 af[2][MI], bfr[2][NI];
+                bool sent = false;
+                WS_FRAGS(0, 0) WS_FRAGS(1, 1)
+                if (s == 0 && kt > 0) cdma(1, t.wco, 0, 1);
+                if (s <= 5) {
+                    cdma((s + 2) % 3, t.wco, (s + 2) >> 2, (s + 2) & 3);
+                    sent = true;
+                } else if (s == 7 && kt + 1 < K) {
+                    cdma(0, tn.wco, 0, 0);
+                    sent = true;
+                }
+                __builtin_amdgcn_sched_barrier(0);
+                WS_MMAS(0) WS_FRAGS(0, 2) WS_MMAS(1) WS_FRAGS(1, 3) WS_MMAS(0) WS_MMAS(1)
+                WS_STAMP()
+                if (sent) wait_vm_keep<UB>();
+                else wait_vm_keep<0>();
+                __syncthreads();
+                WS_STAMP()
+            }
+            cg += 2;
+        } else
         for (int c = 0; c < nchunks; ++c, ++cg) {
             const char* ldsA = WS_BUFA(cg);
             const bool last_c = c + 1 == nchunks;
@@ -1077,7 +1167,7 @@
 #undef WS_FRAGS
 #undef WS_MMAS
         if constexpr (E16) {
-            WS2_EPILOGUE16(t, kt, (ws_stage16<T, BN, MI, NI>(acc, st16 + (wrow * 32 + r) * (BN + kStage16Pad) + wn0 + 4 * h));)
+            WS2_EPILOGUE16(t, kt, (ws_stage16<T, BN, MI, NI>(acc, st16 + (wrow * 32 + r) * (BN + kStage16Pad) + wn0 + 4 * h)); if constexpr (FOLD) wait_vm_keep<0>();)
         } else {
         WS2_EPILOGUE(t, kt, (conv_epilogue_stage<T, BN, 2, NI, 64>(a, reinterpret_cast<f32x16(&)[2][NI]>(acc[0]), t.co0, wn0, r, h, wrow * 32, t.n0, stage));,
                      (conv_epilogue_stage<T, BN, 2, NI, 64>(a, reinterpret_cast<f32x16(&)[2][NI]>(acc[2]), t.co0, wn0, r, h, wrow * 32, t.n0, stage));)
@@ -1233,6 +1323,37 @@
     return true;
 }
 
+static bool ws_fold_pick(const ConvArgs& a, ConvArgs& src, ConvTile& g) {
+    if (a.up != 1 || a.taps != 9 || a.stride != 1 || a.C1 != 128 || a.C2 || a.src2 || a.Cout % 128 || a.scale || a.shift || a.dmask || a.pro_silu || a.has_gni ||
+        a.out_silu || a.out_nchw || a.in_nchw || a.res1 || a.res2 || a.r_w || a.n_gno || a.mix || a.x3 || a.Hout != 2 * a.Hin || a.Wout != 2 * a.Win)
+        return false;
+    if ((int64_t)a.N * a.Hout * a.Wout * a.Cout >= (1ll << 31) || (int64_t)a.N * a.Hin * a.Win * a.C1 >= (1ll << 30)) return false;
+    src = a;
+    src.up = 0;
+    src.Hout = a.Hin;
+    src.Wout = a.Win;
+    ConvArgs t4 = src;
+    t4.Cout = 4 * a.Cout;
+    ConvTile t;
+    if (!make_tile(t4, 256, 128, t) || t.TN != 1 || t.TH * t.TW != 256 || t.a_rows > 352 || ws2_lds(src, t) > 160 * 1024 ||
+        (size_t)t.a_rows * ROW_DATA + 2 * 128 * ROW_DATA < 64 * 1024 || t.tiles_m * t.tiles_n < 256)
+        return false;
+    g = t;
+    return true;
+}
+
+bool conv3x3_ws_fold_route(int dtype, const ConvArgs& a, ConvRoute& r) {
+    ConvTile g{};
+    ConvArgs src{};
+    if (!is16(dtype) || !a.fold_up || getenv("DMME_NO_WS") || !ws_fold_pick(a, src, g)) return false;
+    r = make_route(CONV3X3_WS, 256, 128, 8);
+    r.tile = g;
+    r.fold = 1;
+    r.stat_px = 128;
+    r.stat_tiles = 4 * g.tiles_x * g.tiles_y * 2;
+    return true;
+}
+
 static size_t pipe_launch_lds(int dtype, const ConvArgs& a, const ConvRoute& r, bool* dma) {
     size_t lds = pipe_lds(r.tile, r.BN, r.GT);
     *dma = pipe_dma_ok(dtype, r.tile, r.BN, r.GT);
@@ -1271,6 +1392,26 @@
         hipLaunchKernelGGL((conv3x3_ws2_kernel<11, f16, 256, 2>), wgrid, dim3(512), ws2_lds(a, gw), s, a, gw, ilog2(gw.TW), ilog2(gw.TH), ntiles);
     else
         hipLaunchKernelGGL((conv3x3_ws2_kernel<11, f16, 256, 1>), wgrid, dim3(512), ws2_lds(a, gw), s, a, gw, ilog2(gw.TW), ilog2(gw.TH), ntiles);
+    DMME_CHECK_LAUNCH();
+    return DMME_OK;
+}
+
+template <typename T>
+static int launch_ws_fold_t(const ConvRoute& r, const ConvArgs& a, hipStream_t s) {
+    ConvTile g{};
+    ConvArgs src{};
+    DMME_REQUIRE(r.fold && ws_fold_pick(a, src, g), DMME_ERR_UNSUPPORTED, "folded up-sampling conv: outside the kernel's domain");
+    DMME_REQUIRE(!a.gn_part || (a.gn_tiles == r.stat_tiles && stats_cols_ok(a, 128, a.gn_cg, 8)), DMME_ERR_INVALID,
+                 "folded up-sampling conv: %d statistics partials per image asked for, the launch writes %d", a.gn_tiles, r.stat_tiles);
+    static bool attr = false;
+    if (!attr) {
+        const int rc0 = set_lds_limit(conv3x3_ws2_kernel<11, T, 256, 0, false, true, true>, 160 * 1024);
+        if (rc0 != DMME_OK) return rc0;
+        attr = true;
+    }
+    const int ntiles = g.tiles_m * g.tiles_n;
+    const dim3 wgrid((unsigned)(ntiles < 256 ? ntiles : 256));
+    hipLaunchKernelGGL((conv3x3_ws2_kernel<11, T, 256, 0, false, true, true>), wgrid, dim3(512), ws2_lds(src, g), s, src, g, ilog2(g.TW), ilog2(g.TH), ntiles);
     DMME_CHECK_LAUNCH();
     return DMME_OK;
 }
@@ -1350,7 +1491,9 @@
 int launch_conv3x3(const ConvRoute& r, int dtype, const ConvArgs& a, hipStream_t s) {
     switch (r.family) {
         case CONV3X3_SPLIT: return launch_ws2_split(r, a, s);
-        case CONV3X3_WS: return dtype == DMME_F16 ? launch_ws_t<f16>(r, a, s) : launch_ws_t<bf16>(r, a, s);
+        case CONV3X3_WS:
+            if (r.fold) return dtype == DMME_F16 ? launch_ws_fold_t<f16>(r, a, s) : launch_ws_fold_t<bf16>(r, a, s);
+            return dtype == DMME_F16 ? launch_ws_t<f16>(r, a, s) : launch_ws_t<bf16>(r, a, s);
         case CONV3X3_KW: return launch_conv_kw(dtype, a, r.tile, r.NI, r.ring, r.BM, r.ksplit, s);
         default: break;
     }
diff --git a/diffusion-models-made-easy_amd/csrc/conv_route.hip b/diffusion-models-made-easy_amd/csrc/conv_route.hip
--- a/diffusion-models-made-easy_amd/csrc/conv_route.hip
+++ b/diffusion-models-made-easy_amd/csrc/conv_route.hip
@@ -7,6 +7,10 @@
 
 ConvRoute conv_route(int dtype, const ConvArgs& a) {
     ConvRoute r{};
+    if (a.fold_up) {
+        if (!conv3x3_ws_fold_route(dtype, a, r)) conv_generic_route(a, r);
+        return r;
+    }
     if (conv_thin_route(dtype, a, r)) return r;
     if (conv1x1_split_route(dtype, a, r)) return r;
     if (conv1x1_domain(dtype, a) && (conv1x1_as_route(dtype, a, r) || conv1x1_tiled_route(dtype, a, r))) return r;
@@ -23,6 +27,7 @@
 int launch_conv(const ConvRoute& r, int dtype, const ConvArgs& a, hipStream_t s) {
     DMME_REQUIRE(!a.r_w || r.rseg, DMME_ERR_UNSUPPORTED,
                  "conv with a residual segment: only the wave-specialised 3x3 kernel takes it, with raw channel counts inside its domain");
+    DMME_REQUIRE(!a.fold_up || r.fold, DMME_ERR_UNSUPPORTED, "conv with a phase-folded filter: only the wave-specialised 3x3 kernel's folded form reads it");
     switch (r.family) {
         case CONV_THIN: return launch_conv_out_thin(a, s);
         case CONV1X1_AS: return launch_conv1x1_as(a, s);
@@ -54,7 +59,8 @@
         case CONV1X1_AS: snprintf(buf, (size_t)cap, "conv1x1_as_kernel<%d>", (a.C1 + a.C2) / 64); break;
         case CONV1X1_TILED: snprintf(buf, (size_t)cap, "conv1x1_pipe_kernel<%s,%d,%d>", tn, r.BM, r.BN); break;
         case CONV3X3_SPLIT: snprintf(buf, (size_t)cap, a.mix == 2 ? "conv3x3_ws2_kernel<11,f16x3,src16>" : "conv3x3_ws2_kernel<11,f16x3>"); break;
-        case CONV3X3_WS: snprintf(buf, (size_t)cap, r.BM == 128 ? (a.r_w ? "conv3x3_ws2_kernel<7,128,res>" : "conv3x3_ws2_kernel<7,128>") : a.r_w ? "conv3x3_ws2_kernel<11,res>" : "conv3x3_ws2_kernel<11>"); break;
+        case CONV3X3_WS: if (r.fold) { snprintf(buf, (size_t)cap, "conv3x3_ws2_kernel<11,fold4>"); break; }
+            snprintf(buf, (size_t)cap, r.BM == 128 ? (a.r_w ? "conv3x3_ws2_kernel<7,128,res>" : "conv3x3_ws2_kernel<7,128>") : a.r_w ? "conv3x3_ws2_kernel<11,res>" : "conv3x3_ws2_kernel<11>"); break;
         case CONV3X3_KW: snprintf(buf, (size_t)cap, "conv3x3_kw_kernel<%d,%d,%d>", r.NI, r.ring, r.BM); break;
         case CONV3X3_PIPE: snprintf(buf, (size_t)cap, "conv3x3_pipe_kernel<%s,%d,%d,%d,%d>", tn, r.BM, r.BN, r.GT, r.UA); break;
         case CONV_MFMA: snprintf(buf, (size_t)cap, "conv_mfma_kernel<%s,%d,%d,%d>", tn, a.taps, r.BM, r.BN); break;
diff --git a/diffusion-models-made-easy_amd/csrc/kernels_generic.hip b/diffusion-models-made-easy_amd/csrc/kernels_generic.hip
--- a/diffusion-models-made-easy_amd/csrc/kernels_generic.hip
+++ b/diffusion-models-made-easy_amd/csrc/kernels_generic.hip
@@ -885,6 +885,39 @@
     return DMME_OK;
 }
 
+template <typename T>
+__global__ void __launch_bounds__(256) up_fold_weights_kernel(const UpFoldJob* __restrict__ jobs, UpFoldJob one, char* __restrict__ packed) {
+    const UpFoldJob jb = jobs ? jobs[blockIdx.x] : one;
+    const int row = blockIdx.y;
+    if (row >= 4 * jb.Cout) return;
+    const int ph = row / jb.Cout, co = row - ph * jb.Cout, py = ph >> 1, px = ph & 1;
+    const T* w = (const T*)(packed + jb.w) + (int64_t)co * 9 * jb.Cin;
+    T* d = (T*)(packed + jb.dst) + (int64_t)row * 4 * jb.Cin;
+    for (int c = threadIdx.x; c < jb.Cin; c += 256)
+#pragma unroll
+        for (int tap = 0; tap < 4; ++tap) {
+            const int ta = tap >> 1, tc = tap & 1;
+            const int r0 = py == 0 ? (ta == 0 ? 0 : 1) : (ta == 0 ? 0 : 2), r1 = py == 0 ? (ta == 0 ? 0 : 2) : (ta == 0 ? 1 : 2);
+            const int s0 = px == 0 ? (tc == 0 ? 0 : 1) : (tc == 0 ? 0 : 2), s1 = px == 0 ? (tc == 0 ? 0 : 2) : (tc == 0 ? 1 : 2);
+            float acc = 0.f;
+            for (int r = r0; r <= r1; ++r)
+                for (int q = s0; q <= s1; ++q) acc += (float)w[(int64_t)(r * 3 + q) * jb.Cin + c];
+            d[(int64_t)tap * jb.Cin + c] = from_f<T>(acc);
+        }
+}
+int launch_up_fold_weights(int dtype, const UpFoldJob* jobs_dev, int n_jobs, int max_rows, void* packed, hipStream_t s, const UpFoldJob* one) {
+    if (n_jobs == 0) return DMME_OK;
+    DMME_REQUIRE((jobs_dev != nullptr) != (one != nullptr) && (!one || n_jobs == 1), DMME_ERR_INVALID, "up_fold_weights: a device table, or one job by value");
+    DMME_REQUIRE(is16(dtype) && max_rows >= 4 && max_rows <= 65535, DMME_ERR_UNSUPPORTED, "up_fold_weights: 16-bit plans, at most 65535 filter rows (got %d)", max_rows);
+    const UpFoldJob j1 = one ? *one : UpFoldJob{};
+    if (dtype == DMME_F16)
+        hipLaunchKernelGGL(up_fold_weights_kernel<f16>, dim3((unsigned)n_jobs, (unsigned)max_rows), dim3(256), 0, s, jobs_dev, j1, (char*)packed);
+    else
+        hipLaunchKernelGGL(up_fold_weights_kernel<bf16>, dim3((unsigned)n_jobs, (unsigned)max_rows), dim3(256), 0, s, jobs_dev, j1, (char*)packed);
+    DMME_CHECK_LAUNCH();
+    return DMME_OK;
+}
+
 template <int DEPTH>
 __global__ void __launch_bounds__(256) l2_stream_kernel(const uint4* __restrict__ buf, int nvec, int iters, unsigned* __restrict__ sink) {
     unsigned acc = 0;
diff --git a/diffusion-models-made-easy_amd/csrc/plan.h b/diffusion-models-made-easy_amd/csrc/plan.h
--- a/diffusion-models-made-easy_amd/csrc/plan.h
+++ b/diffusion-models-made-easy_amd/csrc/plan.h
@@ -123,6 +123,7 @@
     int at_fold_qkv = -1;
     int folded_into = -1;
     int64_t fold_M = -1, fold_c = -1, fold_wpv = -1, fold_b2 = -1;
+    int64_t up_fold_w = -1;
     int mix = 0, route_f32 = 0;
     int mix2 = 0;
     int cast_src = -1, cast_dst = -1;
@@ -214,6 +215,9 @@
     std::vector<AttnFoldJob> fold_jobs;
     DevTable<AttnFoldJob> fold_jobs_dev;
     int fold_maxC = 0, n_launches_nograd = 0;
+    std::vector<UpFoldJob> up_jobs;
+    DevTable<UpFoldJob> up_jobs_dev;
+    int up_max_rows = 0;
     mutable const void* fold_packed = nullptr;
     int pred = DMME_PRED_EPS, pred_T = 0;
     const float* pred_ab = nullptr;
@@ -237,6 +241,7 @@
 int run_level(const dmme_plan* P, const LvlRun& R, const char* pk, char* ws, int nt, const float* drop_masks, hipStream_t s, bool keep_ctx = true);
 void assign_lvl_nograd(dmme_plan* P);
 void assign_attn_fold(dmme_plan* P);
+void assign_up_fold(dmme_plan* P);
 int lvl_check(const dmme_plan* P, const char* where, hipStream_t stream = nullptr, bool have_stream = false);
 void build_unpack_items(const dmme_plan* P, std::vector<PackItem>& items);
 void plan_backward(dmme_plan* P);
diff --git a/diffusion-models-made-easy_amd/csrc/plan.hip b/diffusion-models-made-easy_amd/csrc/plan.hip
--- a/diffusion-models-made-easy_amd/csrc/plan.hip
+++ b/diffusion-models-made-easy_amd/csrc/plan.hip
@@ -997,6 +997,35 @@
     P->packed_bytes = cur;
 }
 
+void assign_up_fold(dmme_plan* P) {
+    if (getenv("DMME_NO_UP_FOLD") || getenv("DMME_NO_ATTN_FOLD") || debug_route("no_attn_fold") || debug_route("no_up_fold") || !is16(P->dtype) || P->x3 || P->mix) return;
+    int64_t cur = P->packed_bytes;
+    const int64_t es = (int64_t)dtype_size(P->dtype);
+    for (Op& o : P->ops) {
+        if (o.kind != OP_CONV || o.up != 1 || o.taps != 9 || o.stride != 1 || o.lvl >= 0 || o.src1 < 0 || o.src2 >= 0 || o.dst < 0 || o.gn >= 0 || o.pro_silu ||
+            o.out_silu || o.dmask_off >= 0 || o.tproj_col >= 0 || o.res1 >= 0 || o.res2 >= 0 || o.rseg >= 0 || o.fused_away || o.folded_into >= 0 || o.gd_n > 0 ||
+            o.use_act || o.mix || o.route_f32 || P->tensors[o.src1].f32 || P->tensors[o.dst].f32 || P->params[o.w].pack_code >= 0)
+            continue;
+        ConvArgs a{};
+        fill_conv(P, o, (const char*)4096, (const float*)4096, (float*)4096, (char*)4096, nullptr, 1, a, true);
+        const ConvRoute r9 = conv_route(P->dtype, a);
+        a.fold_up = 1;
+        const ConvRoute r4 = conv_route(P->dtype, a);
+        const Tensor& td = P->tensors[o.dst];
+        if (!r4.fold || (td.stats_off >= 0 && (r4.stat_tiles != td.stats_tiles || r4.stat_px != r9.stat_px))) continue;
+        o.up_fold_w = cur;
+        cur = align_up(cur + (int64_t)4 * a.Cout * 4 * a.C1 * es, 256);
+        UpFoldJob jb{};
+        jb.w = P->params[o.w].packed_off;
+        jb.dst = o.up_fold_w;
+        jb.Cout = a.Cout;
+        jb.Cin = a.C1;
+        P->up_jobs.push_back(jb);
+        if (4 * a.Cout > P->up_max_rows) P->up_max_rows = 4 * a.Cout;
+    }
+    P->packed_bytes = cur;
+}
+
 int run_gn(const dmme_plan* P, const Op& o, const char* pk, char* ws, int nt, const float* drop_masks, hipStream_t s) {
     if (o.gn_direct || o.gn_in_consumer) return DMME_OK;
     const float* tsh = o.gn_mod_col >= 0 ? (const float*)(ws + P->ws_tproj) + o.gn_mod_col : nullptr;
@@ -1068,6 +1097,10 @@
         case OP_CONV: {
             ConvArgs a{};
             fill_conv(P, o, pk, x, y, ws, drop_masks, nt, a, true);
+            if (fold && o.up_fold_w >= 0) {
+                a.w = pk + o.up_fold_w;
+                a.fold_up = 1;
+            }
             return launch_conv(conv_dt(P, o), a, s);
         }
         case OP_CAST: {
@@ -1277,6 +1310,7 @@
     DMME_TRY(P->col_jobs_dev.upload(P->col_jobs));
     DMME_TRY(P->bias_jobs_dev.upload(P->bias_jobs));
     if (!P->fold_jobs.empty()) DMME_TRY(P->fold_jobs_dev.upload(P->fold_jobs));
+    if (!P->up_jobs.empty()) DMME_TRY(P->up_jobs_dev.upload(P->up_jobs));
     std::vector<dmme_plan::WgGroup*> all_groups{&P->wg[0], &P->wg[1], &P->wg[2]};
     for (auto& B_ : P->gb)
         for (int k = 0; k < 3; ++k) all_groups.push_back(&B_.wg[k]);
@@ -1335,6 +1369,7 @@
     assign_attn_proj(P);
     assign_lvl_nograd(P);
     assign_attn_fold(P);
+    assign_up_fold(P);
     P->n_launches = count_launches(P);
     P->n_launches_nograd = count_launches(P, true);
     plan_backward(P);
@@ -1371,6 +1406,7 @@
 DMME_API int dmme_unet_plan_num_launches(const dmme_plan* plan) { return plan ? plan->n_launches : 0; }
 DMME_API int dmme_unet_plan_num_launches_nograd(const dmme_plan* plan) { return plan ? plan->n_launches_nograd : 0; }
 DMME_API int dmme_unet_plan_num_folded(const dmme_plan* plan) { return plan ? (int)plan->fold_jobs.size() : 0; }
+DMME_API int dmme_unet_plan_num_up_folded(const dmme_plan* plan) { return plan ? (int)plan->up_jobs.size() : 0; }
 
 DMME_API int dmme_unet_pack_params(const dmme_plan* plan, const float* ref_flat, void* packed, void* stream) {
     DMME_REQUIRE(plan && ref_flat && packed, DMME_ERR_INVALID, "pack_params: null argument");
@@ -1382,8 +1418,9 @@
 DMME_API int dmme_unet_pack_folded(const dmme_plan* plan, void* packed, void* stream) {
     DMME_REQUIRE(plan && packed, DMME_ERR_INVALID, "pack_folded: null argument");
     DMME_REQUIRE(plan->items_dev, DMME_ERR_INVALID, "pack_folded: plan was created without a device");
-    if (plan->fold_jobs.empty()) return DMME_OK;
-    const int rc = launch_attn_fold_weights(plan->dtype, plan->fold_jobs_dev.get(), (int)plan->fold_jobs.size(), plan->fold_maxC, packed, (hipStream_t)stream);
+    if (plan->fold_jobs.empty() && plan->up_jobs.empty()) return DMME_OK;
+    int rc = launch_attn_fold_weights(plan->dtype, plan->fold_jobs_dev.get(), (int)plan->fold_jobs.size(), plan->fold_maxC, packed, (hipStream_t)stream);
+    if (rc == DMME_OK) rc = launch_up_fold_weights(plan->dtype, plan->up_jobs_dev.get(), (int)plan->up_jobs.size(), plan->up_max_rows, packed, (hipStream_t)stream);
     if (rc == DMME_OK) plan->fold_packed = packed;
     return rc;
 }
@@ -2042,6 +2079,37 @@
     return launch_attn_fold(dtype, x, N, S, C, parts ? &gni : nullptr, scale, shift, M, c, wpv, bias2, res, dst, gn_part, S / 32, gn_cg, (hipStream_t)stream, g_stamps);
 }
 
+DMME_API int dmme_up_fold_weights(int dtype, const void* w, int Cout, int Cin, void* folded, void* stream) {
+    DMME_REQUIRE(w && folded && Cout > 0 && Cin > 0, DMME_ERR_INVALID, "up_fold_weights: bad argument");
+    UpFoldJob jb{};
+    jb.w = (int64_t)(intptr_t)w;
+    jb.dst = (int64_t)(intptr_t)folded;
+    jb.Cout = Cout;
+    jb.Cin = Cin;
+    return launch_up_fold_weights(dtype, nullptr, 1, 4 * Cout, nullptr, (hipStream_t)stream, &jb);
+}
+DMME_API int dmme_conv2d_up_folded(int dtype, const void* src, int N, int Hin, int Win, int Cin, const void* folded, const float* bias, int Cout, void* dst,
+                                   float* gn_part, int gn_cg, int* gn_tiles, void* stream) {
+    DMME_REQUIRE(src && folded && bias && dst && N > 0 && Hin > 0 && Win > 0 && Cin > 0 && Cout > 0, DMME_ERR_INVALID, "conv2d_up_folded: bad argument");
+    DMME_REQUIRE(dtype == DMME_BF16 || dtype == DMME_F16, DMME_ERR_UNSUPPORTED, "conv2d_up_folded: 16-bit tensors only (dtype %d)", dtype);
+    ConvArgs a{};
+    a.src1 = src; a.w = folded; a.bias = bias; a.dst = dst;
+    a.N = N; a.Hin = Hin; a.Win = Win; a.C1 = Cin; a.Cout = Cout;
+    a.up = 1; a.stride = 1; a.taps = 9; a.Hout = 2 * Hin; a.Wout = 2 * Win;
+    a.f16 = dtype == DMME_F16;
+    a.fold_up = 1;
+    a.stamps = g_stamps;
+    const ConvRoute r = conv_route(dtype, a);
+    DMME_REQUIRE(r.fold, DMME_ERR_UNSUPPORTED, "conv2d_up_folded: no folded kernel takes %d -> %d channels on %d x %d x %d source maps", Cin, Cout, N, Hin, Win);
+    if (gn_tiles) *gn_tiles = r.stat_tiles;
+    if (gn_part) {
+        a.gn_part = gn_part;
+        a.gn_cg = gn_cg;
+        a.gn_tiles = r.stat_tiles;
+    }
+    return launch_conv(r, dtype, a, (hipStream_t)stream);
+}
+
 DMME_API int dmme_attention_heads(int dtype, const void* qkv, int N, int S, int C, int heads, void* out, int force_generic, void* stream) {
     DMME_REQUIRE(qkv && out && N > 0 && S > 0 && C > 0 && heads > 0 && C % heads == 0, DMME_ERR_INVALID, "attention_heads: bad argument");
     if (dtype == DMME_BF16X3) {
diff --git a/include/dmme_hip.h b/include/dmme_hip.h
--- a/include/dmme_hip.h
+++ b/include/dmme_hip.h
@@ -67,6 +67,7 @@
 DMME_API int dmme_unet_plan_num_launches(const dmme_plan* plan);
 DMME_API int dmme_unet_plan_num_launches_nograd(const dmme_plan* plan);
 DMME_API int dmme_unet_plan_num_folded(const dmme_plan* plan);
+DMME_API int dmme_unet_plan_num_up_folded(const dmme_plan* plan);
 
 DMME_API int dmme_unet_pack_params(const dmme_plan* plan, const float* ref_flat, void* packed, void* stream);
 DMME_API int dmme_unet_pack_folded(const dmme_plan* plan, void* packed, void* stream);
@@ -326,6 +327,10 @@
                                   const float* gamma, const float* beta, float eps, float* scale, float* shift, const void* M, const float* c,
                                   const void* wpv, const float* bias2, const void* res, void* dst, float* gn_part, int gn_cg, void* stream);
 
+DMME_API int dmme_up_fold_weights(int dtype, const void* w, int Cout, int Cin, void* folded, void* stream);
+DMME_API int dmme_conv2d_up_folded(int dtype, const void* src, int N, int Hin, int Win, int Cin, const void* folded, const float* bias, int Cout,
+                                   void* dst, float* gn_part, int gn_cg, int* gn_tiles, void* stream);
+
 DMME_API int dmme_attention_heads(int dtype, const void* qkv, int N, int S, int C, int heads, void* out, int force_generic, void* stream);
 
 DMME_API int dmme_nchw_to_nhwc(int dtype, const float* src, int N, int C, int HW, void* dst, void* stream);
```

Result: no change. 478.7 denoising steps/s (one step = UNet forward + DDPM update on a batch of 128), summed over GPUs, median of 6 (+0.3%).
